# Florescence/UNet-Medical-Image-Contour-Segmentation

Measured on NVIDIA B200. Metric: unet512_train_images_per_sec, higher is better.
Workload: dtype bf16

## Files before the change

include/unetb200.h:

```cpp
#ifndef UNETB200_H_
#define UNETB200_H_

#include <stddef.h>
#include <stdint.h>

#ifdef __cplusplus
extern "C" {
#endif

#define UNETB200_F32 0
#define UNETB200_BF16 1

#define UNETB200_OK 0
#define UNETB200_E_INVALID (-1)
#define UNETB200_E_CUDA (-2)
#define UNETB200_E_NOMEM (-3)

#define UNETB200_ALGO_AUTO 0
#define UNETB200_ALGO_SIMT 1
#define UNETB200_ALGO_TC 2
#define UNETB200_ALGO_PREFER_TC 3

int unetb200_version(void);
const char* unetb200_last_error(void);
int unetb200_device_info(int* sm_count, int* cc_major, int* cc_minor);

typedef struct unetb200_gconv {
  int32_t dtype;
  int32_t algo;
  int32_t B, Hm, Wm;
  int32_t Cin;
  int32_t ntaps;
  int32_t tap_dy[9], tap_dx[9];
  int32_t in_scale;
  int32_t in_off_y, in_off_x;
  int32_t Hin, Win;
  int64_t ld_in;
  int32_t N;
  int32_t nquad;
  int32_t out_scale;
  int32_t out_off_y, out_off_x;
  int32_t Hout, Wout;
  int64_t ld_out;
} unetb200_gconv_t;

int64_t unetb200_gconv_stats_workspace(const unetb200_gconv_t* d);
int unetb200_gconv_fprop(const unetb200_gconv_t* d, const void* x, const void* wp,
                         const float* bias, void* y, double* stats, float* stats_ws, int* algo_used,
                         void* stream);

int unetb200_gconv_fprop_affine_relu_supported(const unetb200_gconv_t* d, const void* x, const void* wp,
                                               const void* z);
int unetb200_gconv_fprop_affine_relu(const unetb200_gconv_t* d, const void* x, const void* wp,
                                     const float* scale_shift, void* z, void* stream);

int unetb200_gconv_fprop_affine_relu_pool_supported(const unetb200_gconv_t* d, const void* x, const void* wp,
                                                    const void* z, const void* pooled, int64_t ld_pooled);
int unetb200_gconv_fprop_affine_relu_pool(const unetb200_gconv_t* d, const void* x, const void* wp,
                                          const float* scale_shift, void* z, void* pooled, int64_t ld_pooled,
                                          void* stream);

int unetb200_gconv_fprop_affine_relu_outconv_supported(const unetb200_gconv_t* d, const void* x, const void* wp,
                                                       int ncls);
int unetb200_gconv_fprop_affine_relu_outconv(const unetb200_gconv_t* d, const void* x, const void* wp,
                                             const float* scale_shift, const float* oc_w, const float* oc_b,
                                             void* logits, int ncls, void* stream);

int unetb200_gconv_dgrad_bnbwd_supported(const unetb200_gconv_t* d, const void* g, const void* wp, const void* gx);
int unetb200_gconv_dgrad_bnbwd(const unetb200_gconv_t* d, const void* g, const void* wp, void* gx, const void* yprev,
                               int64_t ld_yprev, const float* coefs, double* sums, float* ws, void* stream);

int unetb200_gconv_wgrad_plan(const unetb200_gconv_t* d, int* splits, int* algo_used);
int unetb200_gconv_wgrad(const unetb200_gconv_t* d, const void* x, const void* gy, float* partials,
                         int splits, void* stream);
int unetb200_wgrad_reduce(const float* partials, int splits, int ntaps, int Cin, int N, int Cq,
                          float* dst, int64_t st, int64_t sc, int64_t sq, int64_t sn, int accumulate,
                          void* stream);

typedef struct unetb200_reduce_job {
  const float* partials;
  float* dst;
  int64_t st, sc, sq, sn;
  int32_t splits, ntaps, Cin, N, Cq, accumulate;
} unetb200_reduce_job_t;
int unetb200_wgrad_reduce_multi(const unetb200_reduce_job_t* jobs, int njobs, void* stream);

int unetb200_pack_weights(const float* src, void* dst, int dst_dtype, int64_t n0, int64_t n1,
                          int64_t n2, int64_t s0, int64_t s1, int64_t s2, int64_t off, void* stream);
typedef struct unetb200_pack_job {
  const float* src;
  void* dst;
  int64_t n0, n1, n2;
  int64_t s0, s1, s2, off;
} unetb200_pack_job_t;
int unetb200_pack_weights_multi(const unetb200_pack_job_t* jobs, int njobs, int dst_dtype, void* stream);

int unetb200_split_tf32(const float* x, int64_t ld_x, float* out, int64_t npix, int C, int pattern,
                        void* stream);

int unetb200_bn_finalize(const double* stats, int64_t count, const float* gamma, const float* beta,
                         float eps, float momentum, float* running_mean, float* running_var,
                         float* save_mean, float* save_invstd, float* scale, float* shift, int C,
                         void* stream);
int unetb200_bn_finalize_track(const double* stats, int64_t count, const float* gamma, const float* beta,
                               float eps, float momentum, float* running_mean, float* running_var,
                               float* save_mean, float* save_invstd, float* scale, float* shift,
                               int64_t* num_batches_tracked, int C, void* stream);
int unetb200_bn_eval_coeffs(const float* gamma, const float* beta, const float* running_mean,
                            const float* running_var, float eps, float* scale, float* shift,
                            float* save_mean, float* save_invstd, int C, void* stream);
int unetb200_bn_relu_apply(const void* y, int64_t ld_y, const float* scale, const float* shift,
                           void* z, int64_t ld_z, void* pooled, int64_t ld_p, int dtype, int B,
                           int H, int W, int C, void* stream);
int unetb200_maxpool2_fwd(const void* x, int64_t ld_x, void* p, int64_t ld_p, int dtype, int B,
                          int H, int W, int C, void* stream);
int unetb200_maxpool2_bwd(const void* x, int64_t ld_x, const void* gp, int64_t ld_gp, void* gx,
                          int64_t ld_gx, int accumulate, int dtype, int B, int H, int W, int C,
                          void* stream);
int unetb200_maxpool2_bwd_bnreduce(const void* x, int64_t ld_x, const void* gp, int64_t ld_gp, void* gx,
                                   int64_t ld_gx, const void* y, int64_t ld_y, const float* scale,
                                   const float* shift, const float* mean, const float* invstd, double* sums,
                                   int dtype, int B, int H, int W, int C, void* stream);
int unetb200_bn_relu_bwd_reduce(const void* gz, int64_t ld_gz, const void* y, int64_t ld_y,
                                const float* scale, const float* shift, const float* mean,
                                const float* invstd, double* sums, int dtype, int B, int H, int W,
                                int C, void* stream);
int unetb200_bn_bwd_finalize(const double* sums, int64_t count, int training, float* dgamma,
                             float* dbeta, float* coef, int C, void* stream);
int unetb200_bn_relu_bwd_apply(const void* gz, int64_t ld_gz, const void* y, int64_t ld_y,
                               const float* scale, const float* shift, const float* mean,
                               const float* invstd, const float* coef, void* gy, int64_t ld_gy,
                               int dtype, int B, int H, int W, int C, void* stream);

#define UNETB200_IPC_HANDLE_BYTES 64
#define UNETB200_BUS_ID_BYTES 32
typedef struct unetb200_bn_peer_group_s unetb200_bn_peer_group_t;
int unetb200_bn_peer_group_create(int rank, int world, int max_channels, void* ipc_handle, char* bus_id,
                                  unetb200_bn_peer_group_t** out);
int unetb200_bn_peer_group_open(unetb200_bn_peer_group_t* g, const void* ipc_handles, const char* bus_ids);
int unetb200_bn_peer_group_destroy(unetb200_bn_peer_group_t* g);
int unetb200_bn_peer_group_status(const unetb200_bn_peer_group_t* g, int64_t* missing_rank, int64_t* epoch);
int unetb200_bn_sync_finalize(unetb200_bn_peer_group_t* g, const double* stats, int64_t count,
                              const float* gamma, const float* beta, float eps, float momentum,
                              float* running_mean, float* running_var, float* save_mean,
                              float* save_invstd, float* scale, float* shift,
                              int64_t* num_batches_tracked, int C, void* stream);
int unetb200_bn_sync_bwd_finalize(unetb200_bn_peer_group_t* g, const double* sums, int64_t count,
                                  float* dgamma, float* dbeta, float* coef, int C, void* stream);

int unetb200_upsample2x_fwd(const void* x, int64_t ld_x, void* y, int64_t ld_y, int dtype, int B,
                            int h, int w, int C, int Hout, int Wout, int off_y, int off_x,
                            void* stream);
int unetb200_upsample2x_bwd(const void* gy, int64_t ld_gy, void* gx, int64_t ld_gx, int dtype,
                            int B, int h, int w, int C, int Hout, int Wout, int off_y, int off_x,
                            void* stream);

int unetb200_gather_nhwc(const void* src, int src_dtype, int64_t sn, int64_t sc, int64_t sh,
                         int64_t sw, void* dst, int dst_dtype, int64_t ld_dst, int B, int C, int H,
                         int W, void* stream);
int unetb200_copy_channels(const void* src, int src_dtype, int64_t ld_src, void* dst, int dst_dtype,
                           int64_t ld_dst, int64_t npix, int C, void* stream);
int unetb200_zero_channels(void* dst, int dtype, int64_t ld_dst, int64_t npix, int C, void* stream);
int unetb200_channel_sum(const void* g, int dtype, int64_t ld, int64_t npix, int C, double* acc,
                         float* out, void* stream);
int unetb200_f64_to_f32(const double* src, float* dst, int n, void* stream);
int unetb200_add_channels(void* a, int64_t ld_a, const void* b, int64_t ld_b, int dtype,
                          int64_t npix, int C, void* stream);

int unetb200_outconv_fwd(const void* x, int64_t ld_x, const float* w, const float* bias,
                         void* logits, int dtype, int64_t npix, int C, int ncls, void* stream);
int64_t unetb200_outconv_bwd_workspace(int64_t npix, int C, int ncls);
int unetb200_outconv_bwd(const void* x, int64_t ld_x, const float* w, const void* glogits,
                         void* gx, int64_t ld_gx, float* dw, float* dbias, float* workspace,
                         int dtype, int64_t npix, int C, int ncls, void* stream);
int unetb200_outconv_bwd_bnbwd_supported(const void* x, int64_t ld_x, const void* gx, int64_t ld_gx,
                                         const void* yprev, int64_t ld_yprev, int dtype, int C, int ncls);
int unetb200_outconv_bwd_bnbwd(const void* x, int64_t ld_x, const float* w, const void* glogits, void* gx,
                               int64_t ld_gx, float* dw, float* dbias, float* workspace, const void* yprev,
                               int64_t ld_yprev, const float* coefs, double* sums, int dtype, int64_t npix, int C,
                               int ncls, void* stream);

int unetb200_sa_forward(const void* x, int64_t ld_x, const float* w, float* stats, float* gate, void* out,
                        int64_t ld_out, int dtype, int B, int H, int W, int C, void* stream);
int64_t unetb200_sa_backward_workspace(int B, int H, int W);
int unetb200_sa_backward(const void* g, int64_t ld_g, const void* x, int64_t ld_x, const float* w,
// ... 43 lines not shown
```

unet-medical-image-contour-segmentation_b200/csrc/common.cuh:

```cuda
#pragma once
#include <cuda_bf16.h>
#include <cuda_runtime.h>
#include <stdint.h>
#include <stdio.h>

#include <string>

#include "../../include/unetb200.h"

namespace ub {

void set_error(const char* fmt, ...);
int cuda_fail(cudaError_t e, const char* what);

#define UB_CHECK_ARG(cond, ...)                \
  do {                                         \
    if (!(cond)) {                             \
      ub::set_error(__VA_ARGS__);              \
      return UNETB200_E_INVALID;               \
    }                                          \
  } while (0)

#define UB_LAUNCH_CHECK(what)                              \
  do {                                                     \
// ... 13 lines not shown
  static __device__ __forceinline__ float round(float v) { return v; }
};
template <>
struct Elem<__nv_bfloat16> {
  static __device__ __forceinline__ float ld(const __nv_bfloat16* p) { return __bfloat162float(*p); }
  static __device__ __forceinline__ void st(__nv_bfloat16* p, float v) { *p = __float2bfloat16_rn(v); }
  static __device__ __forceinline__ float round(float v) { return __bfloat162float(__float2bfloat16_rn(v)); }
};

__device__ __forceinline__ void load8(const float* p, float v[8]) {
  float4 a = *reinterpret_cast<const float4*>(p);
  float4 b = *reinterpret_cast<const float4*>(p + 4);
  v[0] = a.x; v[1] = a.y; v[2] = a.z; v[3] = a.w; v[4] = b.x; v[5] = b.y; v[6] = b.z; v[7] = b.w;
}
__device__ __forceinline__ void load8(const __nv_bfloat16* p, float v[8]) {
  uint4 r = *reinterpret_cast<const uint4*>(p);
  const uint32_t w[4] = {r.x, r.y, r.z, r.w};
#pragma unroll
  for (int i = 0; i < 4; ++i) {
    v[2 * i] = __uint_as_float(w[i] << 16);
    v[2 * i + 1] = __uint_as_float(w[i] & 0xffff0000u);
  }
}
__device__ __forceinline__ uint32_t pack_bf16x2(float lo, float hi) {
  __nv_bfloat162 t = __floats2bfloat162_rn(lo, hi);
  return *reinterpret_cast<uint32_t*>(&t);
}
__device__ __forceinline__ void store8(float* p, const float v[8]) {
  *reinterpret_cast<float4*>(p) = make_float4(v[0], v[1], v[2], v[3]);
  *reinterpret_cast<float4*>(p + 4) = make_float4(v[4], v[5], v[6], v[7]);
}
__device__ __forceinline__ void store8(__nv_bfloat16* p, const float v[8]) {
  uint4 r;
  r.x = pack_bf16x2(v[0], v[1]);
  r.y = pack_bf16x2(v[2], v[3]);
  r.z = pack_bf16x2(v[4], v[5]);
  r.w = pack_bf16x2(v[6], v[7]);
  *reinterpret_cast<uint4*>(p) = r;
}

__device__ __forceinline__ float warp_sum(float v) {
#pragma unroll
  for (int o = 16; o > 0; o >>= 1) v += __shfl_xor_sync(0xffffffffu, v, o);
  return v;
}
__device__ __forceinline__ double warp_sum(double v) {
#pragma unroll
  for (int o = 16; o > 0; o >>= 1) v += __shfl_xor_sync(0xffffffffu, v, o);
  return v;
}

inline bool aligned16(const void* p) { return (reinterpret_cast<uintptr_t>(p) & 15) == 0; }

}
```

unet-medical-image-contour-segmentation_b200/csrc/conv_simt.cu:

```cuda
#include <cstdlib>

#include "gconv.cuh"

namespace ub {

constexpr int FBM = 128, FBN = 64, FBK = 16;
constexpr int WBK = 64, WBN = 64, WBM = 16;

int gconv_validate(const unetb200_gconv_t* d, GconvDev* o) {
  UB_CHECK_ARG(d != nullptr, "gconv: null descriptor");
  UB_CHECK_ARG(d->dtype == UNETB200_F32 || d->dtype == UNETB200_BF16, "gconv: dtype %d", d->dtype);
  UB_CHECK_ARG(d->B > 0 && d->Hm > 0 && d->Wm > 0 && d->Cin > 0, "gconv: bad M grid / Cin");
  UB_CHECK_ARG(d->ntaps >= 1 && d->ntaps <= 9, "gconv: ntaps %d", d->ntaps);
  UB_CHECK_ARG(d->in_scale == 1 || d->in_scale == 2, "gconv: in_scale %d", d->in_scale);
  UB_CHECK_ARG(d->out_scale == 1 || d->out_scale == 2, "gconv: out_scale %d", d->out_scale);
  UB_CHECK_ARG(d->nquad == 1 || d->nquad == 4, "gconv: nquad %d", d->nquad);
  UB_CHECK_ARG(d->N > 0 && d->N % d->nquad == 0, "gconv: N %d not divisible by nquad %d", d->N, d->nquad);
  UB_CHECK_ARG(d->nquad == 1 || d->out_scale == 2, "gconv: nquad 4 needs out_scale 2");
  UB_CHECK_ARG(d->Hin > 0 && d->Win > 0 && d->Hout > 0 && d->Wout > 0, "gconv: bad grids");
  UB_CHECK_ARG(d->ld_in >= d->Cin && d->ld_out >= d->N / d->nquad, "gconv: pixel stride smaller than channels");
  UB_CHECK_ARG(d->out_off_y >= 0 && d->out_off_x >= 0 &&
                   (d->Hm - 1) * d->out_scale + (d->nquad == 4 ? 1 : 0) + d->out_off_y < d->Hout &&
                   (d->Wm - 1) * d->out_scale + (d->nquad == 4 ? 1 : 0) + d->out_off_x < d->Wout,
               "gconv: output does not fit the destination grid");
// ... 587 lines not shown

static bool simt_vec_ok(const unetb200_gconv_t* d, const void* x, const void* wp, const void* y) {
  const size_t esz = d->dtype == UNETB200_BF16 ? 2 : 4;
  const int Cq = d->N / d->nquad;
  return d->Cin % 16 == 0 && Cq % 4 == 0 && d->ld_in % 8 == 0 && d->ld_out % 4 == 0 &&
         (reinterpret_cast<uintptr_t>(x) % (8 * esz)) == 0 && (!wp || (reinterpret_cast<uintptr_t>(wp) % 16) == 0) &&
         (reinterpret_cast<uintptr_t>(y) % (4 * esz)) == 0;
}

static int simt_fbn(int N) { return N <= 16 ? 16 : (N <= 32 ? 32 : 64); }
static int simt_fbm(int N) { return 8 * 256 / (simt_fbn(N) / 4); }
static int simt_wbk(int N) { return 4 * 256 / (simt_fbn(N) / 4); }

static int simt_wgrad_splits(const GconvDev& g) {
  const int wbn = simt_fbn(g.N), wbk = simt_wbk(g.N);
  long long tiles = (long long)((g.K + wbk - 1) / wbk) * ((g.N + wbn - 1) / wbn);
  long long want = ((long long)sm_count() * 6 + tiles - 1) / tiles;
  long long max_by_m = (g.M + 255) / 256;
  if (want > max_by_m) want = max_by_m;
  if (want > 1024) want = 1024;
  if (want < 1) want = 1;
  return (int)want;
}

}

using namespace ub;
typedef __nv_bfloat16 bf16;

extern "C" {

int64_t unetb200_gconv_stats_workspace(const unetb200_gconv_t* d) {
  GconvDev g;
  if (gconv_validate(d, &g)) return -1;
  long long simt_tiles = (g.M + FBM - 1) / FBM;
  long long tiles = simt_tiles;
  long long ft = first_fprop_tiles(d);
  if (ft > tiles) tiles = ft;
  long long n = tiles * 2 * g.N;
  long long n2 = tc2_stats_workspace(d);
  if (n2 > n) n = n2;
  long long n3 = tc3_stats_workspace(d);
  if (n3 > n) n = n3;
  const long long n4 = narrow_tc_stats_rows(d) * 2 * g.N;
  if (n4 > n) n = n4;
  const long long n5 = halo_stats_rows(d) * 2 * g.N;
  if (n5 > n) n = n5;
  const long long n6 = first_narrow_rows(d) * 2 * g.N;
  if (n6 > n) n = n6;
  const long long n7 = fprop_narrow_f32_rows(d) * 2 * g.N;
  return n > n7 ? n : n7;
}

int unetb200_gconv_fprop(const unetb200_gconv_t* d, const void* x, const void* wp, const float* bias, void* y,
                         double* stats, float* stats_ws, int* algo_used, void* stream) {
  GconvDev g;
  int rc = gconv_validate(d, &g);
  if (rc) return rc;
  UB_CHECK_ARG(x && wp && y, "gconv_fprop: null pointer");
  UB_CHECK_ARG(!stats || (stats_ws && d->nquad == 1), "gconv_fprop: stats need a workspace and nquad == 1");
  if (!stats) stats_ws = nullptr;
  cudaStream_t s = (cudaStream_t)stream;
  int algo = d->algo;
  if (algo != UNETB200_ALGO_SIMT && !stats && halo_t_fprop_supported(d, x, wp, y)) {
    if (algo_used) *algo_used = UNETB200_ALGO_TC;
    return halo_t_fprop(d, x, wp, bias, y, s);
  }
  if (algo != UNETB200_ALGO_SIMT && !stats && !bias && halo_t_dgrad_supported(d, x, wp, y)) {
    if (algo_used) *algo_used = UNETB200_ALGO_TC;
    return halo_t_dgrad(d, x, wp, y, s);
  }
  if (!bias && first_narrow_supported(d, y)) {
    if (algo_used) *algo_used = UNETB200_ALGO_SIMT;
    return first_narrow_fprop(d, x, wp, y, stats, stats_ws, nullptr, s);
  }
  if (algo != UNETB200_ALGO_SIMT && !bias && halo_fprop_supported(d, x, wp, y)) {
    if (algo_used) *algo_used = UNETB200_ALGO_TC;
    return halo_fprop(d, x, wp, y, stats, stats_ws, nullptr, s);
  }
  if (algo != UNETB200_ALGO_SIMT && !bias && narrow_tc_supported(d, x, wp, y)) {
    if (algo_used) *algo_used = UNETB200_ALGO_TC;
    return narrow_tc_fprop(d, x, wp, y, stats, stats_ws, nullptr, s);
  }
  if (algo == UNETB200_ALGO_AUTO || algo == UNETB200_ALGO_PREFER_TC) algo = tc_fprop_supported(d, x, wp, y) ? UNETB200_ALGO_TC : UNETB200_ALGO_SIMT;
  if (algo_used) *algo_used = algo;
  if (algo == UNETB200_ALGO_TC) {
    UB_CHECK_ARG(tc_fprop_supported(d, x, wp, y), "gconv_fprop: tcgen05 path requested but shape/alignment unsupported");
    if (tc3_fprop_supported(d, x, wp, bias, y)) return tc3_fprop(d, g, x, wp, y, stats, stats_ws, s);
    return tc2_fprop(d, g, x, wp, bias, y, stats, stats_ws, s);
  }
  UB_CHECK_ARG(algo == UNETB200_ALGO_SIMT, "gconv_fprop: unknown algo %d", algo);
  if (!bias && first_fprop_supported(d, y)) return first_fprop(d, g, x, wp, y, stats, stats_ws, s);
  if (!bias && fprop_narrow_f32_supported(d, x, wp, y)) return fprop_narrow_f32(d, x, wp, y, stats, stats_ws, s);
  const int fbn = simt_fbn(g.N), fbm = simt_fbm(g.N);
  dim3 grid((unsigned)((g.M + fbm - 1) / fbm), (unsigned)((g.N + fbn - 1) / fbn));
  const bool vec = simt_vec_ok(d, x, wp, y) && (g.K % 4 == 0);
#define UB_SIMT_F(T, V, BN) gconv_fprop_simt_kernel<T, V, BN><<<grid, 256, 0, s>>>(g, (const T*)x, (const T*)wp, bias, (T*)y, stats_ws)
#define UB_SIMT_FN(T, V) do { if (fbn == 16) UB_SIMT_F(T, V, 16); else if (fbn == 32) UB_SIMT_F(T, V, 32); else UB_SIMT_F(T, V, 64); } while (0)
  if (d->dtype == UNETB200_BF16) {
    if (vec) UB_SIMT_FN(bf16, true); else UB_SIMT_FN(bf16, false);
  } else {
    if (vec) UB_SIMT_FN(float, true); else UB_SIMT_FN(float, false);
  }
#undef UB_SIMT_FN
#undef UB_SIMT_F
  UB_LAUNCH_CHECK("gconv_fprop_simt");
  if (stats) return launch_stats_reduce(stats_ws, (g.M + fbm - 1) / fbm, 2 * g.N, stats, s);
  return 0;
}

int unetb200_gconv_fprop_affine_relu_supported(const unetb200_gconv_t* d, const void* x, const void* wp, const void* z) {
  GconvDev g;
  if (gconv_validate(d, &g)) return 0;
  static const bool off = getenv("UNETB200_NO_BN_FOLD") != nullptr;
  static const bool wide = getenv("UNETB200_TC3_MAXBN") && atoi(getenv("UNETB200_TC3_MAXBN")) >= 256;
  if (off || d->algo == UNETB200_ALGO_SIMT) return 0;
  if (first_tc_supported(d, z) && aligned16(wp)) return 1;
  if (first_narrow_supported(d, z)) return 1;
  if (halo_fprop_supported(d, x, wp, z)) return 1;
  if (narrow_tc_supported(d, x, wp, z)) return 1;
  if (d->N % 128 != 0 && d->N % 64 != 0) return 0;
  if (d->dtype == UNETB200_BF16 && d->N % 256 == 0 && wide) return 0;
  return tc_fprop_supported(d, x, wp, z) && tc3_fprop_supported(d, x, wp, nullptr, z);
}

int unetb200_gconv_fprop_affine_relu(const unetb200_gconv_t* d, const void* x, const void* wp, const float* scale_shift,
                                     void* z, void* stream) {
  GconvDev g;
  int rc = gconv_validate(d, &g);
  if (rc) return rc;
  UB_CHECK_ARG(x && wp && z && scale_shift, "gconv_fprop_affine_relu: null pointer");
  UB_CHECK_ARG(unetb200_gconv_fprop_affine_relu_supported(d, x, wp, z),
               "gconv_fprop_affine_relu: shape not covered by the fused kernel (query _supported first and run "
               "gconv_fprop + bn_relu_apply instead)");
  if (first_tc_supported(d, z) && aligned16(wp))
    return first_tc_fprop(d, x, wp, z, nullptr, nullptr, scale_shift, (cudaStream_t)stream);
  if (first_narrow_supported(d, z))
    return first_narrow_fprop(d, x, wp, z, nullptr, nullptr, scale_shift, (cudaStream_t)stream);
  if (halo_fprop_supported(d, x, wp, z))
    return halo_fprop(d, x, wp, z, nullptr, nullptr, scale_shift, (cudaStream_t)stream);
  if (narrow_tc_supported(d, x, wp, z))
    return narrow_tc_fprop(d, x, wp, z, nullptr, nullptr, scale_shift, (cudaStream_t)stream);
  return tc3_fprop(d, g, x, wp, z, nullptr, nullptr, (cudaStream_t)stream, scale_shift);
}

int unetb200_gconv_fprop_affine_relu_pool_supported(const unetb200_gconv_t* d, const void* x, const void* wp, const void* z,
                                                    const void* pooled, int64_t ld_pooled) {
  GconvDev g;
  if (gconv_validate(d, &g)) return 0;
  static const bool off = getenv("UNETB200_NO_POOL_FOLD") != nullptr;
  if (off || d->dtype != UNETB200_BF16 || !pooled || (ld_pooled & 1) || (reinterpret_cast<uintptr_t>(pooled) & 3)) return 0;
  if (!unetb200_gconv_fprop_affine_relu_supported(d, x, wp, z)) return 0;
  if ((first_tc_supported(d, z) && aligned16(wp)) || first_narrow_supported(d, z)) return 0;
  if (!halo_fprop_supported(d, x, wp, z) && narrow_tc_supported(d, x, wp, z)) return 0;
  return d->Hm >= 2 && d->Wm >= 2;
}

int unetb200_gconv_fprop_affine_relu_pool(const unetb200_gconv_t* d, const void* x, const void* wp, const float* scale_shift,
                                          void* z, void* pooled, int64_t ld_pooled, void* stream) {
  GconvDev g;
  int rc = gconv_validate(d, &g);
  if (rc) return rc;
  UB_CHECK_ARG(x && wp && z && scale_shift && pooled, "gconv_fprop_affine_relu_pool: null pointer");
  UB_CHECK_ARG(unetb200_gconv_fprop_affine_relu_pool_supported(d, x, wp, z, pooled, ld_pooled),
               "gconv_fprop_affine_relu_pool: shape not covered (query _supported first and run gconv_fprop_affine_relu + "
               "maxpool2_fwd instead)");
  if (halo_fprop_supported(d, x, wp, z))
    return halo_fprop(d, x, wp, z, nullptr, nullptr, scale_shift, (cudaStream_t)stream, nullptr, 0, nullptr, pooled,
                      (long long)ld_pooled);
  return tc3_fprop(d, g, x, wp, z, nullptr, nullptr, (cudaStream_t)stream, scale_shift, nullptr, 0, nullptr, nullptr, pooled,
                   (long long)ld_pooled);
}

int unetb200_gconv_dgrad_bnbwd_supported(const unetb200_gconv_t* d, const void* g, const void* wp, const void* gx) {
  GconvDev gd;
  if (gconv_validate(d, &gd)) return 0;
  static const bool off = getenv("UNETB200_NO_BNBWD_FUSE") != nullptr;
  if (off || d->algo == UNETB200_ALGO_SIMT) return 0;
  if (halo_bnbwd_supported(d, g, wp, gx)) return 1;
  return tc_fprop_supported(d, g, wp, gx) && tc3_fprop_supported(d, g, wp, nullptr, gx) && tc3_bnbwd_supported(d);
}

int unetb200_gconv_dgrad_bnbwd(const unetb200_gconv_t* d, const void* g, const void* wp, void* gx, const void* yprev,
                               int64_t ld_yprev, const float* coefs, double* sums, float* ws, void* stream) {
  GconvDev gd;
  int rc = gconv_validate(d, &gd);
  if (rc) return rc;
  UB_CHECK_ARG(g && wp && gx && yprev && coefs && sums && ws, "gconv_dgrad_bnbwd: null pointer");
  UB_CHECK_ARG(ld_yprev >= d->N, "gconv_dgrad_bnbwd: ld_yprev < N");
  UB_CHECK_ARG(unetb200_gconv_dgrad_bnbwd_supported(d, g, wp, gx),
               "gconv_dgrad_bnbwd: shape not covered by the fused kernel (query _supported first and run gconv_fprop + "
               "bn_relu_bwd_reduce instead)");
  if (halo_bnbwd_supported(d, g, wp, gx))
    return halo_fprop(d, g, wp, gx, sums, ws, nullptr, (cudaStream_t)stream, yprev, (long long)ld_yprev, coefs);
  return tc3_fprop(d, gd, g, wp, gx, sums, ws, (cudaStream_t)stream, nullptr, yprev, (long long)ld_yprev, coefs);
}

int unetb200_gconv_fprop_affine_relu_outconv_supported(const unetb200_gconv_t* d, const void* x, const void* wp,
                                                       int ncls) {
  GconvDev g;
  if (gconv_validate(d, &g)) return 0;
  static const bool off = getenv("UNETB200_NO_BN_FOLD") != nullptr || getenv("UNETB200_NO_OUTCONV_FOLD") != nullptr;
  if (off || d->algo == UNETB200_ALGO_SIMT || !aligned16(x) || !aligned16(wp)) return 0;
  return tc3_affine_outconv_supported(d, ncls);
}

int unetb200_gconv_fprop_affine_relu_outconv(const unetb200_gconv_t* d, const void* x, const void* wp,
                                             const float* scale_shift, const float* oc_w, const float* oc_b,
                                             void* logits, int ncls, void* stream) {
  GconvDev g;
  int rc = gconv_validate(d, &g);
  if (rc) return rc;
  UB_CHECK_ARG(x && wp && scale_shift && oc_w && logits, "gconv_fprop_affine_relu_outconv: null pointer");
  UB_CHECK_ARG(unetb200_gconv_fprop_affine_relu_outconv_supported(d, x, wp, ncls),
               "gconv_fprop_affine_relu_outconv: shape not covered (query _supported first)");
  Tc3OutConv oc = {oc_w, oc_b, logits, ncls};
  return tc3_fprop(d, g, x, wp, logits, nullptr, nullptr, (cudaStream_t)stream, scale_shift, nullptr, 0, nullptr, &oc);
}

int unetb200_gconv_wgrad_plan(const unetb200_gconv_t* d, int* splits, int* algo_used) {
  GconvDev g;
  int rc = gconv_validate(d, &g);
  if (rc) return rc;
  int algo = d->algo;
  if (first_narrow_supported(d, nullptr)) {
    if (algo_used) *algo_used = UNETB200_ALGO_SIMT;
    if (splits) *splits = first_narrow_wgrad_splits(d);
    return 0;
  }
  if (algo != UNETB200_ALGO_SIMT && halo_wgrad_supported(d, nullptr, nullptr)) {
    if (algo_used) *algo_used = UNETB200_ALGO_TC;
    if (splits) *splits = halo_wgrad_splits(d);
    return 0;
  }
  if (algo != UNETB200_ALGO_SIMT && halo_t_wgrad_supported(d, nullptr, nullptr)) {
    if (algo_used) *algo_used = UNETB200_ALGO_TC;
    if (splits) *splits = halo_t_wgrad_splits(d);
    return 0;
  }
  if (algo != UNETB200_ALGO_SIMT && narrow_wgrad_supported(d, nullptr, nullptr)) {
    if (algo_used) *algo_used = UNETB200_ALGO_TC;
    if (splits) *splits = narrow_wgrad_splits(d);
    return 0;
  }
  if (algo == UNETB200_ALGO_AUTO || algo == UNETB200_ALGO_PREFER_TC) algo = tc_wgrad_supported(d, nullptr, nullptr) ? UNETB200_ALGO_TC : UNETB200_ALGO_SIMT;
  if (algo == UNETB200_ALGO_TC)
    UB_CHECK_ARG(tc_wgrad_supported(d, nullptr, nullptr), "gconv_wgrad: tcgen05 path requested but shape unsupported");
// ... 191 lines not shown
```

unet-medical-image-contour-segmentation_b200/csrc/conv_tc3.cu:

```cuda
#include <cstring>

#include "tc_common.cuh"

namespace ub {

__device__ __forceinline__ uint32_t cluster_ctarank() {
  uint32_t r;
  asm volatile("mov.u32 %0, %%cluster_ctarank;" : "=r"(r));
  return r;
}
__device__ __forceinline__ void cluster_sync_all() {
  asm volatile("barrier.cluster.arrive.release.aligned;\n\tbarrier.cluster.wait.acquire.aligned;" ::: "memory");
}
__device__ __forceinline__ uint32_t mapa_u32(uint32_t saddr, uint32_t rank) {
  uint32_t r;
  asm volatile("mapa.shared::cluster.u32 %0, %1, %2;" : "=r"(r) : "r"(saddr), "r"(rank));
  return r;
}
__device__ __forceinline__ void mbar_arrive_cluster(uint32_t cluster_addr) {
  asm volatile("mbarrier.arrive.release.cluster.shared::cluster.b64 _, [%0];" ::"r"(cluster_addr) : "memory");
}
__device__ __forceinline__ void mbar_arrive_local(uint64_t* bar) {
  asm volatile("mbarrier.arrive.shared::cta.b64 _, [%0];" ::"r"(smem_u32(bar)) : "memory");
}
// ... 123 lines not shown
  long long ld_pool;
};

constexpr uint32_t kA3Stage = 44032;
constexpr int kEpi3Stage = 4096;
constexpr int kEpi3Warps = 8;
constexpr int kTc3Threads = 64 + 32 * kEpi3Warps;

constexpr int EPI_PLAIN = 0, EPI_AFFINE = 1, EPI_BNBWD = 2, EPI_AFFINE_OUT = 3;
template <typename T, int BLOCK_N, int SA, int SB, int ACC, int CG, int TPS, int EPI = EPI_PLAIN>
__global__ void __launch_bounds__(kTc3Threads, 1) tc3_conv_kernel(const __grid_constant__ Tc3Params p) {
  constexpr bool OUTC = EPI == EPI_AFFINE_OUT, AFFINE = EPI == EPI_AFFINE || OUTC, BNBWD = EPI == EPI_BNBWD;
  static_assert(!OUTC || (BLOCK_N == 64 && sizeof(T) == 2), "the OutConv epilogue is the bf16 N = 64 kernel");
  constexpr bool TF32 = sizeof(T) == 4;
  constexpr int EPR = 128 / sizeof(T);
  constexpr uint32_t kBTap = (BLOCK_N / CG) * 128;
  constexpr uint32_t kBStage = TPS * kBTap;
  static_assert(9 % TPS == 0, "taps per stage");
  constexpr int NCB = BLOCK_N / EPR;
  static_assert(2 * BLOCK_N * ACC <= 512, "TMEM columns");
  extern __shared__ uint8_t smem_raw[];
  uint8_t* smem = reinterpret_cast<uint8_t*>((reinterpret_cast<uintptr_t>(smem_raw) + 1023) & ~(uintptr_t)1023);
  uint8_t* a_ring = smem;
  uint8_t* b_ring = a_ring + SA * kA3Stage;
  uint8_t* epi = b_ring + SB * kBStage;
  uint8_t* yst = epi + kEpi3Warps * kEpi3Stage;
  uint64_t* bars = reinterpret_cast<uint64_t*>(yst + (BNBWD ? kEpi3Warps * kEpi3Stage : 0));
  uint64_t* a_full = bars;
  uint64_t* a_empty = a_full + SA;
  uint64_t* b_full = a_empty + SA;
  uint64_t* b_empty = b_full + SB;
  uint64_t* t_full = b_empty + SB;
  uint64_t* t_empty = t_full + ACC;
  uint64_t* y_full = t_empty + ACC;
  uint32_t* tmem_slot = reinterpret_cast<uint32_t*>(y_full + kEpi3Warps);

  const int warp = threadIdx.x >> 5, lane = threadIdx.x & 31;
  const uint32_t rank = CG == 2 ? cluster_ctarank() : 0u;
  const int group0 = blockIdx.x / CG, ngroups = gridDim.x / CG;
  if (warp == 0 && lane == 0) {
    tma_prefetch_desc(&p.a_map);
    tma_prefetch_desc(&p.b_map);
    tma_prefetch_desc(&p.o_map);
    for (int s = 0; s < SA; ++s) { mbar_init(&a_full[s], 1); mbar_init(&a_empty[s], 1); }
    for (int s = 0; s < SB; ++s) { mbar_init(&b_full[s], 1); mbar_init(&b_empty[s], 1); }
    for (int s = 0; s < ACC; ++s) { mbar_init(&t_full[s], 1); mbar_init(&t_empty[s], kEpi3Warps * CG); }
    if constexpr (BNBWD) {
      tma_prefetch_desc(&p.y_map);
      for (int s = 0; s < kEpi3Warps; ++s) mbar_init(&y_full[s], 1);
    }
    fence_barrier_init();
  }
  if (warp == 1) tmem_alloc_cg<CG>(tmem_slot, 512);
  if constexpr (OUTC) {
    float* ocs = reinterpret_cast<float*>(epi);
    for (int i = threadIdx.x; i < 64 * 8 + 8; i += blockDim.x) {
      const int c = i >> 3, k = i & 7;
      float v = 0.f;
      if (k < p.ncls) v = c < 64 ? __ldg(p.oc_w + k * 64 + c) : (p.oc_b ? __ldg(p.oc_b + k) : 0.f);
      ocs[i] = __bfloat162float(__float2bfloat16_rn(v));
    }
  }
  tc_fence_before();
  __syncthreads();
  if constexpr (CG == 2) cluster_sync_all();
  tc_fence_after();
  const uint32_t tmem_base = *tmem_slot;

  if (warp == 0) {
    uint32_t sa = 0, pa = 1, sb = 0, pb = 1;
    for (int gt = group0; gt < p.total_groups; gt += ngroups) {
      const int nb = gt / p.m_groups;
      int mt = (gt - nb * p.m_groups) * CG + (int)rank;
      const bool valid = mt < p.m_tiles;
      const int tj = mt % p.tiles_w;
      mt /= p.tiles_w;
      const int ti = mt % p.tiles_h;
      const int b = valid ? mt / p.tiles_h : p.B;
      const int i0 = ti * p.tile_h - 1, j0 = tj * p.tile_w - 1;
      const int n0 = nb * BLOCK_N + (int)rank * (BLOCK_N / CG);
      for (int c = 0; c < p.cchunks; ++c) {
        mbar_wait(&a_empty[sa], pa);
        if (elect_one()) {
          if (rank == 0) mbar_expect_tx(&a_full[sa], CG * p.a_box_bytes);
          tma_load_4d_cg<CG>(a_ring + sa * kA3Stage, &p.a_map, mapa_u32(smem_u32(&a_full[sa]), 0), c * EPR, j0, i0, b);
        }
        if (++sa == SA) { sa = 0; pa ^= 1; }
        for (int t = 0; t < 9; t += TPS) {
          mbar_wait(&b_empty[sb], pb);
          if (elect_one()) {
            if (rank == 0) mbar_expect_tx(&b_full[sb], CG * kBStage);
            const uint32_t bar = mapa_u32(smem_u32(&b_full[sb]), 0);
#pragma unroll
            for (int j = 0; j < TPS; ++j)
              tma_load_2d_cg<CG>(b_ring + sb * kBStage + j * kBTap, &p.b_map, bar, (t + j) * p.Cin + c * EPR, n0);
          }
          if (++sb == SB) { sb = 0; pb ^= 1; }
        }
      }
    }
  } else if (warp == 1) {
    if (rank == 0) {
      constexpr uint32_t idesc = make_idesc(TF32, false, false, 128 * CG, BLOCK_N);
      const uint64_t a_desc_t = make_desc(smem_u32(a_ring), 16, p.row_bytes);
      const uint64_t b_desc_t = make_desc(smem_u32(b_ring), 16, 1024);
      const uint32_t sub1 = p.sub1_off;
      uint32_t sa = 0, pa = 0, sb = 0, pb = 0, acc = 0, pacc = 1;
      for (int gt = group0; gt < p.total_groups; gt += ngroups) {
        mbar_wait(&t_empty[acc], pacc);
        tc_fence_after();
        const uint32_t d_tmem = tmem_base + acc * 2 * BLOCK_N;
        uint32_t accum = 0;
        for (int c = 0; c < p.cchunks; ++c) {
          mbar_wait(&a_full[sa], pa);
          const uint64_t a_desc0 = a_desc_t + sa * (kA3Stage >> 4);
          for (int t = 0; t < 9; t += TPS) {
            mbar_wait(&b_full[sb], pb);
            tc_fence_after();
            const uint64_t b_desc0 = b_desc_t + sb * (kBStage >> 4);
            if (elect_one()) {
#pragma unroll
              for (int j = 0; j < TPS; ++j) {
                const uint64_t a_desc1 = a_desc0 + p.tap_aoff[t + j];
                const uint64_t b_desc1 = b_desc0 + j * (kBTap >> 4);
#pragma unroll
                for (int kk = 0; kk < 4; ++kk) {
                  const uint32_t on = accum | (uint32_t)(j | kk);
                  umma_cg<CG, TF32>(d_tmem, a_desc1 + 2 * kk, b_desc1 + 2 * kk, idesc, on);
                  umma_cg<CG, TF32>(d_tmem + BLOCK_N, a_desc1 + sub1 + 2 * kk, b_desc1 + 2 * kk, idesc, on);
                }
              }
              umma_commit_cg<CG>(&b_empty[sb]);
              if (t + TPS == 9) umma_commit_cg<CG>(&a_empty[sa]);
            }
            __syncwarp();
            accum = 1;
            if (++sb == SB) { sb = 0; pb ^= 1; }
          }
          if (++sa == SA) { sa = 0; pa ^= 1; }
        }
        if (elect_one()) umma_commit_cg<CG>(&t_full[acc]);
        __syncwarp();
        if (++acc == ACC) { acc = 0; pacc ^= 1; }
      }
    }
  } else {
    const int quad = warp & 3;
    const int s = (warp - 2) >> 2;
    const int ew = s * 4 + quad;
    uint8_t* buf = epi + ew * kEpi3Stage;
    const uint32_t buf_s = smem_u32(buf);
    uint32_t acc = 0, pacc = 0;
    int cur_nb = -1;
    float st[NCB][TF32 ? 2 : 4];
#pragma unroll
    for (int i = 0; i < NCB; ++i)
#pragma unroll
      for (int j = 0; j < (TF32 ? 2 : 4); ++j) st[i][j] = 0.f;
    auto flush = [&](int nb) {
      if (!p.stats_ws || nb < 0) return;
      float* dst = p.stats_ws + (((long long)nb * gridDim.x + blockIdx.x) * kEpi3Warps + ew) * 2 * BLOCK_N;
#pragma unroll
      for (int cb = 0; cb < NCB; ++cb) {
        if constexpr (TF32) {
          dst[cb * 32 + lane] = st[cb][0];
          dst[BLOCK_N + cb * 32 + lane] = st[cb][1];
          st[cb][0] = st[cb][1] = 0.f;
        } else {
          dst[cb * 64 + 2 * lane] = st[cb][0];
          dst[BLOCK_N + cb * 64 + 2 * lane] = st[cb][1];
          dst[cb * 64 + 2 * lane + 1] = st[cb][2];
          dst[BLOCK_N + cb * 64 + 2 * lane + 1] = st[cb][3];
          st[cb][0] = st[cb][1] = st[cb][2] = st[cb][3] = 0.f;
        }
      }
    };
    const uint32_t t_empty_leader0 = mapa_u32(smem_u32(&t_empty[0]), 0);
    constexpr int CPL = TF32 ? 1 : 2;
    float bmu[BNBWD ? NCB : 1][CPL], bis[BNBWD ? NCB : 1][CPL], bsc[BNBWD ? NCB : 1][CPL], bsh[BNBWD ? NCB : 1][CPL];
    uint8_t* ybuf = yst + ew * kEpi3Stage;
    const uint32_t ybuf_s = smem_u32(ybuf);
    uint32_t yph = 0;
    auto y_fetch = [&](int gt2, int cb2) {
      const int nb2 = gt2 / p.m_groups;
      int mt2 = (gt2 - nb2 * p.m_groups) * CG + (int)rank;
      const bool valid2 = mt2 < p.m_tiles;
      const int tj2 = mt2 % p.tiles_w;
      mt2 /= p.tiles_w;
      const int ti2 = mt2 % p.tiles_h;
      const int b2 = valid2 ? mt2 / p.tiles_h : p.B;
      mbar_expect_tx(&y_full[ew], kEpi3Stage);
      tma_load_4d(ybuf, &p.y_map, &y_full[ew], nb2 * BLOCK_N + cb2 * EPR, tj2 * p.tile_w + s * p.sub1_dj,
                  ti2 * p.tile_h + s * p.sub1_di + 4 * quad, b2);
    };
    if constexpr (BNBWD) {
      if (lane == 0 && group0 < p.total_groups) y_fetch(group0, 0);
    }
    for (int gt = group0; gt < p.total_groups; gt += ngroups) {
      const int nb = gt / p.m_groups;
      int mt = (gt - nb * p.m_groups) * CG + (int)rank;
      const bool valid = mt < p.m_tiles;
      const int tj = mt % p.tiles_w;
      mt /= p.tiles_w;
      const int ti = mt % p.tiles_h;
      const int b = mt / p.tiles_h;
      const int n0 = nb * BLOCK_N;
      if (nb != cur_nb) {
        flush(cur_nb);
        cur_nb = nb;
        if constexpr (BNBWD) {
#pragma unroll
          for (int cb = 0; cb < NCB; ++cb)
#pragma unroll
            for (int k = 0; k < CPL; ++k) {
              const int ch = n0 + cb * EPR + CPL * lane + k;
              bmu[cb][k] = __ldg(p.bnc + ch);
              bis[cb][k] = __ldg(p.bnc + p.N + ch);
              bsc[cb][k] = __ldg(p.bnc + 2 * p.N + ch);
              bsh[cb][k] = __ldg(p.bnc + 3 * p.N + ch);
            }
        }
      }
      const int pi0 = ti * p.tile_h + s * p.sub1_di + 4 * quad;
      const int pj0 = tj * p.tile_w + s * p.sub1_dj;
      const uint32_t valid_rows =
          __ballot_sync(0xffffffffu, valid && (pi0 + (lane >> 3) < p.Hm) && (pj0 + (lane & 7) < p.Wm));
      mbar_wait(&t_full[acc], pacc);
      tc_fence_after();
      if (valid_rows != 0u) {
#pragma unroll
        for (int cb = 0; cb < NCB; ++cb) {
          const uint32_t taddr = tmem_base + ((uint32_t)(quad * 32) << 16) + acc * 2 * BLOCK_N + s * BLOCK_N + cb * EPR;
          uint32_t v[EPR];
#pragma unroll
          for (int h = 0; h < EPR / 32; ++h) tmem_ld32_issue(taddr + h * 32, v + h * 32);
          if (lane == 0) tma_store_wait_read_all();
          tmem_ld_fence();
          __syncwarp();
          if constexpr (AFFINE) {
            const float4* sc4 = reinterpret_cast<const float4*>(p.affine + n0 + cb * EPR);
            const float4* sh4 = reinterpret_cast<const float4*>(p.affine + p.N + n0 + cb * EPR);
#pragma unroll
            for (int k4 = 0; k4 < EPR / 4; ++k4) {
              const float4 a = __ldg(sc4 + k4), c = __ldg(sh4 + k4);
              v[4 * k4 + 0] = __float_as_uint(fmaxf(fmaf(__uint_as_float(v[4 * k4 + 0]), a.x, c.x), 0.f));
              v[4 * k4 + 1] = __float_as_uint(fmaxf(fmaf(__uint_as_float(v[4 * k4 + 1]), a.y, c.y), 0.f));
              v[4 * k4 + 2] = __float_as_uint(fmaxf(fmaf(__uint_as_float(v[4 * k4 + 2]), a.z, c.z), 0.f));
              v[4 * k4 + 3] = __float_as_uint(fmaxf(fmaf(__uint_as_float(v[4 * k4 + 3]), a.w, c.w), 0.f));
            }
          }
          if constexpr (OUTC) {
            const float* ocs = reinterpret_cast<const float*>(epi);
            float lg[8];
#pragma unroll
            for (int k = 0; k < 8; ++k) lg[k] = 0.f;
#pragma unroll
            for (int c = 0; c < 64; ++c) {
              const float z = __bfloat162float(__float2bfloat16_rn(__uint_as_float(v[c])));
              const float4 w0 = *reinterpret_cast<const float4*>(ocs + c * 8);
              lg[0] = fmaf(z, w0.x, lg[0]); lg[1] = fmaf(z, w0.y, lg[1]);
              lg[2] = fmaf(z, w0.z, lg[2]); lg[3] = fmaf(z, w0.w, lg[3]);
// ... 98 lines not shown
            for (int r = 0; r < 32; ++r)
              u[r] = lds_u32(buf_s + r * 128 + ((((lane >> 2) ^ (r & 7)) << 4) | ((lane & 3) << 2)));
            if (valid_rows == 0xffffffffu) {
#pragma unroll
              for (int r = 0; r < 32; ++r) {
                if constexpr (TF32) {
                  const float a = __uint_as_float(u[r]);
                  s0 += a; q0 = fmaf(a, a, q0);
                } else {
                  const float a = __uint_as_float(u[r] << 16), c2 = __uint_as_float(u[r] & 0xffff0000u);
                  s0 += a; q0 = fmaf(a, a, q0); s1 += c2; q1 = fmaf(c2, c2, q1);
                }
              }
            } else {
#pragma unroll
              for (int r = 0; r < 32; ++r) {
                const float m = ((valid_rows >> r) & 1u) ? 1.f : 0.f;
                if constexpr (TF32) {
                  const float a = __uint_as_float(u[r]) * m;
                  s0 += a; q0 = fmaf(a, a, q0);
                } else {
                  const float a = __uint_as_float(u[r] << 16) * m, c2 = __uint_as_float(u[r] & 0xffff0000u) * m;
                  s0 += a; q0 = fmaf(a, a, q0); s1 += c2; q1 = fmaf(c2, c2, q1);
                }
              }
            }
            st[cb][0] += s0; st[cb][1] += q0;
            if constexpr (!TF32) { st[cb][2] += s1; st[cb][3] += q1; }
          }
        }
      }
      if constexpr (BNBWD) {
        if (valid_rows == 0u) {
#pragma unroll 1
          for (int cb = 0; cb < NCB; ++cb) {
            mbar_wait(&y_full[ew], yph);
            yph ^= 1;
            __syncwarp();
            if (lane == 0) {
              if (cb + 1 < NCB) y_fetch(gt, cb + 1);
              else if (gt + ngroups < p.total_groups) y_fetch(gt + ngroups, 0);
            }
          }
        }
      }
      tc_fence_before();
      __syncwarp();
      if (lane == 0) {
        if constexpr (CG == 2) mbar_arrive_cluster(t_empty_leader0 + acc * 8);
        else mbar_arrive_local(&t_empty[acc]);
      }
      if (++acc == ACC) { acc = 0; pacc ^= 1; }
    }
    flush(cur_nb);
    if (lane == 0) tma_store_wait_all();
  }
  tc_fence_before();
  __syncthreads();
  if constexpr (CG == 2) cluster_sync_all();
  if (warp == 1) {
    __syncwarp();
    tmem_dealloc_cg<CG>(tmem_base, 512);
  }
}

struct Tc3Plan {
  int BN, CG, tile_w, tile_h, box_w, box_h;
  int m_tiles, m_groups, n_blocks, grid;
};

static int tc3_cluster_size() {
  static const int cg = getenv("UNETB200_TC3_CG1") ? 1 : 2;
  return cg;
}

static bool tc3_plan(const unetb200_gconv_t* d, Tc3Plan* pl) {
  const int esz = d->dtype == UNETB200_BF16 ? 2 : 4;
  const int epr = 128 / esz;
  if (d->dtype != UNETB200_BF16 && d->dtype != UNETB200_F32) return false;
  if (d->nquad != 1 || d->in_scale != 1 || d->out_scale != 1 || d->ntaps != 9) return false;
  if (d->in_off_y || d->in_off_x) return false;
  if (d->Cin % epr || d->N % 64) return false;
  if ((d->ld_in * esz) % 16 || (d->ld_out * esz) % 16) return false;
  bool seen[9] = {false};
  for (int t = 0; t < 9; ++t) {
    const int dy = d->tap_dy[t], dx = d->tap_dx[t];
    if (dy < -1 || dy > 1 || dx < -1 || dx > 1) return false;
    if (seen[(dy + 1) * 3 + dx + 1]) return false;
    seen[(dy + 1) * 3 + dx + 1] = true;
  }
  pl->CG = tc3_cluster_size();
  static const int max_bn = getenv("UNETB200_TC3_MAXBN") ? atoi(getenv("UNETB200_TC3_MAXBN")) : 128;
  pl->BN = (d->dtype == UNETB200_BF16 && d->N % 256 == 0 && max_bn >= 256) ? 256 : (d->N % 128 == 0 ? 128 : 64);
  if (d->Wm > 8) { pl->tile_w = 16; pl->tile_h = 16; }
  else { pl->tile_w = 8; pl->tile_h = 32; }
  pl->box_w = pl->tile_w + 2;
  pl->box_h = pl->tile_h + 2;
  const int tiles_w = (d->Wm + pl->tile_w - 1) / pl->tile_w, tiles_h = (d->Hm + pl->tile_h - 1) / pl->tile_h;
  pl->m_tiles = d->B * tiles_w * tiles_h;
  pl->m_groups = (pl->m_tiles + pl->CG - 1) / pl->CG;
  pl->n_blocks = d->N / pl->BN;
  const long long total = (long long)pl->m_groups * pl->n_blocks;
  const int slots = sm_count() / pl->CG;
  pl->grid = (int)(total < slots ? total : slots) * pl->CG;
  return true;
}

int tc3_fprop_supported(const unetb200_gconv_t* d, const void* x, const void* wp, const float* bias, const void* y) {
  static const bool off = getenv("UNETB200_NO_TC3") != nullptr;
  if (off || bias) return 0;
  if (d->dtype == UNETB200_F32 && d->algo != UNETB200_ALGO_TC && d->algo != UNETB200_ALGO_PREFER_TC) return 0;
  Tc3Plan pl;
  if (!tc3_plan(d, &pl)) return 0;
  if (!aligned16(x) || !aligned16(wp) || !aligned16(y)) return 0;
  return 1;
}

long long tc3_stats_workspace(const unetb200_gconv_t* d) {
  Tc3Plan pl;
  if (!tc3_plan(d, &pl)) return 0;
  return (long long)pl.n_blocks * pl.grid * kEpi3Warps * 2 * pl.BN;
}

template <typename T, int BN, int SA, int SB, int ACC, int CG, int TPS, int EPI = EPI_PLAIN>
static int tc3_launch(const Tc3Params& P, int grid, cudaStream_t s) {
  constexpr int smem = SA * kA3Stage + SB * TPS * (BN / CG) * 128 + (EPI == EPI_BNBWD ? 2 : 1) * kEpi3Warps * kEpi3Stage + 1024 + 256;
  static_assert(smem <= 227 * 1024, "shared memory budget");
  if (int rc = set_max_dynamic_smem(reinterpret_cast<const void*>(&tc3_conv_kernel<T, BN, SA, SB, ACC, CG, TPS, EPI>), smem,
                                    "tc3_conv smem attribute"))
    return rc;
  cudaLaunchConfig_t cfg = {};
  cfg.gridDim = dim3((unsigned)grid);
  cfg.blockDim = dim3(kTc3Threads);
  cfg.dynamicSmemBytes = smem;
  cfg.stream = s;
  cudaLaunchAttribute at[1];
  at[0].id = cudaLaunchAttributeClusterDimension;
  at[0].val.clusterDim.x = CG;
  at[0].val.clusterDim.y = 1;
  at[0].val.clusterDim.z = 1;
  cfg.attrs = at;
  cfg.numAttrs = 1;
  cudaError_t e = cudaLaunchKernelEx(&cfg, tc3_conv_kernel<T, BN, SA, SB, ACC, CG, TPS, EPI>, P);
  if (e != cudaSuccess) return cuda_fail(e, "tc3_conv launch");
  return 0;
}

__global__ void __launch_bounds__(1024) tc3_stats_reduce_kernel(const float* __restrict__ ws, int rows, int BN, int N, double* __restrict__ stats) {
  __shared__ double red[32][33];
  const int lane = threadIdx.x & 31, ry = threadIdx.x >> 5;
  const int nb = blockIdx.y;
  const int col = blockIdx.x * 32 + lane;
  double acc = 0.0;
  if (col < 2 * BN) {
    const float* base = ws + (long long)nb * rows * 2 * BN + col;
    int r = ry;
    for (; r + 96 < rows; r += 128) {
      const float a = base[(long long)r * 2 * BN], b = base[(long long)(r + 32) * 2 * BN],
                  c = base[(long long)(r + 64) * 2 * BN], d = base[(long long)(r + 96) * 2 * BN];
      acc += (double)a; acc += (double)b; acc += (double)c; acc += (double)d;
    }
    for (; r < rows; r += 32) acc += (double)base[(long long)r * 2 * BN];
  }
  red[ry][lane] = acc;
  __syncthreads();
  if (ry == 0 && col < 2 * BN) {
    double s = 0.0;
#pragma unroll
    for (int i = 0; i < 32; ++i) s += red[i][lane];
    const int which = col / BN, c = col - which * BN;
    stats[which * N + nb * BN + c] += s;
  }
}

int tc3_bnbwd_supported(const unetb200_gconv_t* d) {
  Tc3Plan pl;
  if (!tc3_plan(d, &pl)) return 0;
  return pl.CG == 2 && pl.BN != 256;
}

int tc3_affine_outconv_supported(const unetb200_gconv_t* d, int ncls) {
  Tc3Plan pl;
  if (!tc3_plan(d, &pl)) return 0;
  return d->dtype == UNETB200_BF16 && pl.CG == 2 && pl.BN == 64 && d->N == 64 && ncls >= 1 && ncls <= 8;
}

int tc3_fprop(const unetb200_gconv_t* d, const GconvDev& g, const void* x, const void* wp, void* y, double* stats,
              float* stats_ws, cudaStream_t stream, const float* affine, const void* yprev, long long ld_yprev,
              const float* bnc, const Tc3OutConv* oc, void* pooled, long long ld_pool) {
  Tc3Plan pl;
  if (pooled && (!affine || oc || d->dtype != UNETB200_BF16 || (ld_pool & 1) || (reinterpret_cast<uintptr_t>(pooled) & 3))) {
    set_error("tc3_fprop: the pooled second output needs the bf16 affine epilogue and 4-byte aligned rows");
    return UNETB200_E_INVALID;
  }
  if (yprev && (affine || !stats || !stats_ws || !bnc || !aligned16(yprev) ||
                (ld_yprev * (d->dtype == UNETB200_BF16 ? 2 : 4)) % 16)) {
    set_error("tc3_fprop: the BatchNorm-backward epilogue needs sums, a workspace, coefficients and 16-byte aligned yprev rows");
    return UNETB200_E_INVALID;
  }
  if (affine && (stats || (reinterpret_cast<uintptr_t>(affine) & 15))) {
    set_error("tc3_fprop: the affine epilogue takes no statistics and needs 16-byte aligned coefficients");
    return UNETB200_E_INVALID;
  }
  if (!tc3_plan(d, &pl)) { set_error("tc3_fprop: unsupported shape"); return UNETB200_E_INVALID; }
  const int esz = d->dtype == UNETB200_BF16 ? 2 : 4;
  Tc3Params P;
  memset(&P, 0, sizeof(P));
  int rc = encode_act_box(&P.a_map, d->dtype, x, d->Cin, d->Win, d->Hin, d->B, d->ld_in, (long long)d->Win * d->ld_in,
                          (long long)d->Hin * d->Win * d->ld_in, pl.box_w, pl.box_h, false);
  if (rc) return rc;
  const char* obase = (const char*)y + ((long long)d->out_off_y * d->Wout + d->out_off_x) * d->ld_out * (long long)esz;
  rc = encode_act_box(&P.o_map, d->dtype, obase, d->N, d->Wm, d->Hm, d->B, d->ld_out, (long long)d->Wout * d->ld_out,
                      (long long)d->Hout * d->Wout * d->ld_out, 8, 4, false);
  if (rc) return rc;
  rc = encode_weights(&P.b_map, d->dtype, wp, g.K, d->N, pl.BN / pl.CG);
  if (rc) return rc;
  for (int t = 0; t < 9; ++t)
    P.tap_aoff[t] = (uint32_t)(((d->tap_dy[t] + 1) * pl.box_w + (d->tap_dx[t] + 1)) * 128) >> 4;
  P.a_box_bytes = (uint32_t)(pl.box_w * pl.box_h * 128);
  P.row_bytes = (uint32_t)pl.box_w * 128;
  if (pl.tile_w == 16) { P.sub1_di = 0; P.sub1_dj = 8; P.sub1_off = (8 * 128) >> 4; }
  else { P.sub1_di = 16; P.sub1_dj = 0; P.sub1_off = (uint32_t)(16 * pl.box_w * 128) >> 4; }
  P.cchunks = d->Cin / (128 / esz);
  P.Cin = d->Cin;
  P.tile_w = pl.tile_w; P.tile_h = pl.tile_h;
  P.tiles_w = (d->Wm + pl.tile_w - 1) / pl.tile_w;
  P.tiles_h = (d->Hm + pl.tile_h - 1) / pl.tile_h;
  P.m_tiles = pl.m_tiles; P.m_groups = pl.m_groups;
  P.total_groups = pl.m_groups * pl.n_blocks;
  P.Hm = d->Hm; P.Wm = d->Wm; P.B = d->B;
  P.stats_ws = stats ? stats_ws : nullptr;
  P.affine = affine;
  P.N = d->N;
  P.bnc = bnc;
  P.pooled = pooled; P.ld_pool = ld_pool;
  if (yprev) {
    rc = encode_act_box(&P.y_map, d->dtype, yprev, d->N, d->Wm, d->Hm, d->B, ld_yprev, (long long)d->Wm * ld_yprev,
                        (long long)d->Hm * d->Wm * ld_yprev, 8, 4, false);
    if (rc) return rc;
  }
  if (oc) {
    if (!affine || !tc3_affine_outconv_supported(d, oc->ncls) || !oc->w || !oc->logits) {
      set_error("tc3_fprop: the OutConv epilogue needs the folded BatchNorm coefficients, bf16, N = 64 and n_classes <= 8");
      return UNETB200_E_INVALID;
    }
    P.oc_w = oc->w; P.oc_b = oc->b; P.logits = oc->logits; P.ncls = oc->ncls;
    return tc3_launch<__nv_bfloat16, 64, 3, 3, 2, 2, 3, EPI_AFFINE_OUT>(P, pl.grid, stream);
  }
  if (affine) {
    if (pl.BN == 256) { set_error("tc3_fprop: affine epilogue supports N blocks of 64 / 128"); return UNETB200_E_INVALID; }
    if (d->dtype == UNETB200_BF16) {
      if (pl.CG == 2) return pl.BN == 128 ? tc3_launch<__nv_bfloat16, 128, 2, 3, 2, 2, 3, EPI_AFFINE>(P, pl.grid, stream)
                                          : tc3_launch<__nv_bfloat16, 64, 3, 3, 2, 2, 3, EPI_AFFINE>(P, pl.grid, stream);
      return pl.BN == 128 ? tc3_launch<__nv_bfloat16, 128, 2, 6, 2, 1, 1, EPI_AFFINE>(P, pl.grid, stream)
                          : tc3_launch<__nv_bfloat16, 64, 3, 6, 2, 1, 1, EPI_AFFINE>(P, pl.grid, stream);
    }
    if (pl.CG == 2) return pl.BN == 128 ? tc3_launch<float, 128, 2, 3, 2, 2, 3, EPI_AFFINE>(P, pl.grid, stream)
                                        : tc3_launch<float, 64, 3, 3, 2, 2, 3, EPI_AFFINE>(P, pl.grid, stream);
    return pl.BN == 128 ? tc3_launch<float, 128, 2, 6, 2, 1, 1, EPI_AFFINE>(P, pl.grid, stream)
                        : tc3_launch<float, 64, 3, 6, 2, 1, 1, EPI_AFFINE>(P, pl.grid, stream);
  }
  if (stats) {
    cudaError_t e = cudaMemsetAsync(stats_ws, 0, sizeof(float) * (size_t)tc3_stats_workspace(d), stream);
    if (e != cudaSuccess) return cuda_fail(e, "tc3 stats workspace memset");
  }
  if (yprev) {
    if (pl.CG != 2 || pl.BN == 256) { set_error("tc3_fprop: BatchNorm-backward epilogue: CTA pairs, N blocks of 64 / 128"); return UNETB200_E_INVALID; }
    static const int cfg64 = getenv("UNETB200_BNBWD64_CFG") ? atoi(getenv("UNETB200_BNBWD64_CFG")) : 1;
    if (d->dtype == UNETB200_BF16)
      rc = pl.BN == 128 ? tc3_launch<__nv_bfloat16, 128, 2, 3, 2, 2, 3, EPI_BNBWD>(P, pl.grid, stream)
           : cfg64 == 1 ? tc3_launch<__nv_bfloat16, 64, 3, 2, 2, 2, 3, EPI_BNBWD>(P, pl.grid, stream)
                        : tc3_launch<__nv_bfloat16, 64, 2, 3, 2, 2, 3, EPI_BNBWD>(P, pl.grid, stream);
    else
      rc = pl.BN == 128 ? tc3_launch<float, 128, 2, 3, 2, 2, 3, EPI_BNBWD>(P, pl.grid, stream)
                        : tc3_launch<float, 64, 3, 2, 2, 2, 3, EPI_BNBWD>(P, pl.grid, stream);
  } else if (d->dtype == UNETB200_BF16) {
    if (pl.CG == 2) {
      if (pl.BN == 256) rc = tc3_launch<__nv_bfloat16, 256, 2, 2, 1, 2, 3>(P, pl.grid, stream);
      else if (pl.BN == 128) rc = tc3_launch<__nv_bfloat16, 128, 2, 3, 2, 2, 3>(P, pl.grid, stream);
      else rc = tc3_launch<__nv_bfloat16, 64, 3, 3, 2, 2, 3>(P, pl.grid, stream);
    } else {
      if (pl.BN == 256) rc = tc3_launch<__nv_bfloat16, 256, 2, 3, 1, 1, 1>(P, pl.grid, stream);
      else if (pl.BN == 128) rc = tc3_launch<__nv_bfloat16, 128, 2, 6, 2, 1, 1>(P, pl.grid, stream);
      else rc = tc3_launch<__nv_bfloat16, 64, 3, 6, 2, 1, 1>(P, pl.grid, stream);
    }
  } else {
    if (pl.CG == 2) {
      if (pl.BN == 128) rc = tc3_launch<float, 128, 2, 3, 2, 2, 3>(P, pl.grid, stream);
      else rc = tc3_launch<float, 64, 3, 3, 2, 2, 3>(P, pl.grid, stream);
    } else {
      if (pl.BN == 128) rc = tc3_launch<float, 128, 2, 6, 2, 1, 1>(P, pl.grid, stream);
      else rc = tc3_launch<float, 64, 3, 6, 2, 1, 1>(P, pl.grid, stream);
    }
  }
  if (rc) return rc;
  if (stats) {
    const int rows = pl.grid * kEpi3Warps;
    tc3_stats_reduce_kernel<<<dim3((2 * pl.BN + 31) / 32, pl.n_blocks), 1024, 0, stream>>>(stats_ws, rows, pl.BN, d->N, stats);
    cudaError_t e = cudaGetLastError();
    if (e != cudaSuccess) return cuda_fail(e, "tc3_stats_reduce");
  }
  return 0;
}


struct alignas(64) Tc3WParams {
  CUtensorMap a_map;
  CUtensorMap o_map;
  int g_dx[3], g_dy0, g_tap[3][3];
  int Cin, nunits;
  int tiles_w, tiles_h;
  int ptiles, ptiles_per_split;
  int N, K;
  float* partials;
};

template <int STAGES>
__global__ void __launch_bounds__(192, 1) tc3_wgrad_kernel(const __grid_constant__ Tc3WParams p) {
  constexpr int EPR = 64, BLOCK_N = 128;
  constexpr uint32_t kGSub = 64 * 128;
  constexpr uint32_t kABox = 10 * 8 * 128;
  constexpr uint32_t kStage = 2 * kABox + kGSub;
  constexpr int UMMA_K = 16, MMAS = 64 / UMMA_K;
  extern __shared__ uint8_t smem_raw[];
  uint8_t* smem = reinterpret_cast<uint8_t*>((reinterpret_cast<uintptr_t>(smem_raw) + 1023) & ~(uintptr_t)1023);
  uint64_t* full_bar = reinterpret_cast<uint64_t*>(smem + STAGES * kStage);
  uint64_t* empty_bar = full_bar + STAGES;
  uint64_t* tmem_full = empty_bar + STAGES;
  uint32_t* tmem_slot = reinterpret_cast<uint32_t*>(tmem_full + 1);

  const int warp = threadIdx.x >> 5, lane = threadIdx.x & 31;
  const uint32_t rank = cluster_ctarank();
  const int mt = blockIdx.x >> 1;
  const int n0 = blockIdx.y * BLOCK_N;
  const int split = blockIdx.z;
  const int pt_begin = split * p.ptiles_per_split;
  int pt_end = pt_begin + p.ptiles_per_split;
  if (pt_end > p.ptiles) pt_end = p.ptiles;
  const int num_k = pt_end - pt_begin;

  if (warp == 0 && lane == 0) {
    tma_prefetch_desc(&p.a_map);
    tma_prefetch_desc(&p.o_map);
    for (int s = 0; s < STAGES; ++s) { mbar_init(&full_bar[s], 1); mbar_init(&empty_bar[s], 1); }
    mbar_init(tmem_full, 1);
    fence_barrier_init();
  }
  if (warp == 1) tmem_alloc_cg<2>(tmem_slot, 512);
  tc_fence_before();
  __syncthreads();
  cluster_sync_all();
  tc_fence_after();
  const uint32_t tmem_base = *tmem_slot;

  if (warp == 0) {
    int pt = pt_begin;
    int tj = pt % p.tiles_w;
    int rest = pt / p.tiles_w;
    int ti = rest % p.tiles_h;
    int b = rest / p.tiles_h;
    int uc[2], ug[2];
#pragma unroll
    for (int h = 0; h < 2; ++h) {
      const int u = mt * 4 + (int)rank * 2 + h;
      uc[h] = u / 3;
      ug[h] = u - uc[h] * 3;
    }
    uint32_t s = 0, ph = 1;
    for (int kb = 0; kb < num_k; ++kb) {
      mbar_wait(&empty_bar[s], ph);
      if (elect_one()) {
        if (rank == 0) mbar_expect_tx(&full_bar[s], 2 * kStage);
        const uint32_t bar = mapa_u32(smem_u32(&full_bar[s]), 0);
        const int i0 = ti * 8, j0 = tj * 8;
        uint8_t* sa = smem + s * kStage;
#pragma unroll
        for (int h = 0; h < 2; ++h)
          tma_load_4d_cg<2>(sa + h * kABox, &p.a_map, bar, uc[h] * EPR, j0 + p.g_dx[ug[h]], i0 + p.g_dy0, b);
        tma_load_4d_cg<2>(sa + 2 * kABox, &p.o_map, bar, n0 + (int)rank * 64, j0, i0, b);
      }
      if (++s == STAGES) { s = 0; ph ^= 1; }
      if (++tj == p.tiles_w) { tj = 0; if (++ti == p.tiles_h) { ti = 0; ++b; } }
    }
  } else if (warp == 1) {
    if (rank == 0) {
      constexpr uint32_t idesc = make_idesc(false, true, true, 256, BLOCK_N);
      const uint64_t da_t = make_desc(smem_u32(smem), kABox, 1024, kLayoutSW128);
      const uint64_t db_t = make_desc(smem_u32(smem) + 2 * kABox, kGSub, 1024, kLayoutSW128);
      uint32_t s = 0, ph = 0;
      for (int kb = 0; kb < num_k; ++kb) {
        mbar_wait(&full_bar[s], ph);
        tc_fence_after();
        const uint64_t da0 = da_t + s * (kStage >> 4), db0 = db_t + s * (kStage >> 4);
        if (elect_one()) {
#pragma unroll
          for (int a = 0; a < 3; ++a) {
#pragma unroll
            for (int k = 0; k < MMAS; ++k)
              umma_cg<2, false>(tmem_base + a * BLOCK_N, da0 + ((a * 1024 + k * UMMA_K * 128) >> 4),
                                db0 + ((k * UMMA_K * 128) >> 4), idesc, (kb > 0 || k > 0) ? 1u : 0u);
          }
// ... 68 lines not shown
  w->mpairs = w->nunits / 4;
  w->ntiles = d->N / 128;
  w->tiles_w = (d->Wm + 7) / 8;
  w->tiles_h = (d->Hm + 7) / 8;
  w->ptiles = d->B * w->tiles_w * w->tiles_h;
  return true;
}

int tc3_wgrad_supported(const unetb200_gconv_t* d, const void* x, const void* gy) {
  Tc3WPlan w;
  if (!tc3_wgrad_plan(d, &w)) return 0;
  if ((x && !aligned16(x)) || (gy && !aligned16(gy))) return 0;
  return 1;
}

int tc3_wgrad_splits(const unetb200_gconv_t* d) {
  Tc3WPlan w;
  if (!tc3_wgrad_plan(d, &w)) return 1;
  const long long pairs = (long long)w.mpairs * w.ntiles;
  const long long max_by_k = (w.ptiles + 15) / 16;
  return pick_splits(pairs, sm_count() / 2, max_by_k);
}

int tc3_wgrad(const unetb200_gconv_t* d, const GconvDev& g, const void* x, const void* gy, float* partials, int splits,
              cudaStream_t stream) {
  Tc3WPlan w;
  if (!tc3_wgrad_plan(d, &w)) { set_error("tc3_wgrad: unsupported shape"); return UNETB200_E_INVALID; }
  Tc3WParams P;
  memset(&P, 0, sizeof(P));
  int rc = encode_act_box(&P.a_map, d->dtype, x, d->Cin, d->Win, d->Hin, d->B, d->ld_in, (long long)d->Win * d->ld_in,
                          (long long)d->Hin * d->Win * d->ld_in, 8, 10, true);
  if (rc) return rc;
  const char* obase = (const char*)gy + ((long long)d->out_off_y * d->Wout + d->out_off_x) * d->ld_out * 2LL;
  rc = encode_act_box(&P.o_map, d->dtype, obase, d->N, d->Wm, d->Hm, d->B, d->ld_out, (long long)d->Wout * d->ld_out,
                      (long long)d->Hout * d->Wout * d->ld_out, 8, 8, true);
  if (rc) return rc;
  for (int gi = 0; gi < 3; ++gi) {
    P.g_dx[gi] = w.g_dx[gi];
    for (int a = 0; a < 3; ++a) P.g_tap[gi][a] = w.g_tap[gi][a];
  }
  P.g_dy0 = w.g_dy0;
  P.Cin = d->Cin; P.nunits = w.nunits;
  P.tiles_w = w.tiles_w; P.tiles_h = w.tiles_h;
  P.ptiles = w.ptiles;
  P.ptiles_per_split = (w.ptiles + splits - 1) / splits;
  P.N = d->N; P.K = g.K;
  P.partials = partials;
  static const int st_env = getenv("UNETB200_TC3W_STAGES") ? atoi(getenv("UNETB200_TC3W_STAGES")) : 7;
  const bool deep = st_env >= 7;
  const int smem = (deep ? 7 : 5) * (2 * 10240 + 8192) + 1024 + 256;
  if (int rc = deep ? set_max_dynamic_smem(reinterpret_cast<const void*>(&tc3_wgrad_kernel<7>), smem, "tc3_wgrad smem attribute")
                    : set_max_dynamic_smem(reinterpret_cast<const void*>(&tc3_wgrad_kernel<5>), smem, "tc3_wgrad smem attribute"))
    return rc;
  cudaLaunchConfig_t cfg = {};
  cfg.gridDim = dim3((unsigned)w.mpairs * 2, (unsigned)w.ntiles, (unsigned)splits);
  cfg.blockDim = dim3(192);
  cfg.dynamicSmemBytes = smem;
  cfg.stream = stream;
  cudaLaunchAttribute at[1];
  at[0].id = cudaLaunchAttributeClusterDimension;
  at[0].val.clusterDim.x = 2;
  at[0].val.clusterDim.y = 1;
  at[0].val.clusterDim.z = 1;
  cfg.attrs = at;
  cfg.numAttrs = 1;
  cudaError_t e = deep ? cudaLaunchKernelEx(&cfg, tc3_wgrad_kernel<7>, P) : cudaLaunchKernelEx(&cfg, tc3_wgrad_kernel<5>, P);
  if (e != cudaSuccess) return cuda_fail(e, "tc3_wgrad launch");
  return 0;
}

}
```

unet-medical-image-contour-segmentation_b200/csrc/conv_tc4.cu:

```cuda
#include <cstring>

#include "tc_common.cuh"

namespace ub {

struct alignas(64) Tc4WParams {
  CUtensorMap a_map;
  CUtensorMap o_map;
  int tap[3][3];
  int Cin, N, K;
  int cchunks;
  int tiles_w, tiles_h;
  int ptiles, ptiles_per_split;
  float* partials;
};

constexpr uint32_t kT4Box = 10240;
constexpr uint32_t kT4Stage = 2 * kT4Box;
constexpr int kT4AccCols = 192;

template <int STAGES>
__global__ void __launch_bounds__(192, 1) tc4_wgrad_kernel(const __grid_constant__ Tc4WParams p) {
  constexpr int UMMA_K = 16, MMAS = 64 / UMMA_K;
  extern __shared__ uint8_t smem_raw[];
  uint8_t* smem = reinterpret_cast<uint8_t*>((reinterpret_cast<uintptr_t>(smem_raw) + 1023) & ~(uintptr_t)1023);
  uint64_t* full_bar = reinterpret_cast<uint64_t*>(smem + STAGES * kT4Stage);
  uint64_t* empty_bar = full_bar + STAGES;
  uint64_t* tmem_full = empty_bar + STAGES;
  uint32_t* tmem_slot = reinterpret_cast<uint32_t*>(tmem_full + 1);

  const int warp = threadIdx.x >> 5, lane = threadIdx.x & 31;
  const int c = blockIdx.x % p.cchunks;
  const int g = blockIdx.x / p.cchunks;
  const int split = blockIdx.z;
  const int pt_begin = split * p.ptiles_per_split;
  int pt_end = pt_begin + p.ptiles_per_split;
  if (pt_end > p.ptiles) pt_end = p.ptiles;
  const int num_k = pt_end - pt_begin;

  if (warp == 0 && lane == 0) {
    tma_prefetch_desc(&p.a_map);
    tma_prefetch_desc(&p.o_map);
    for (int s = 0; s < STAGES; ++s) { mbar_init(&full_bar[s], 1); mbar_init(&empty_bar[s], 1); }
    mbar_init(tmem_full, 1);
    fence_barrier_init();
  }
  if (warp == 1) tmem_alloc(tmem_slot, 512);
  tc_fence_before();
  __syncthreads();
  tc_fence_after();
  const uint32_t tmem_base = *tmem_slot;

  if (warp == 0) {
    int pt = pt_begin;
    int tj = pt % p.tiles_w;
    int rest = pt / p.tiles_w;
    int ti = rest % p.tiles_h;
    int b = rest / p.tiles_h;
    uint32_t s = 0, ph = 1;
    for (int kb = 0; kb < num_k; ++kb) {
      mbar_wait(&empty_bar[s], ph);
      if (elect_one()) {
        mbar_expect_tx(&full_bar[s], kT4Stage);
        const int i0 = ti * 8, j0 = tj * 8;
        uint8_t* sa = smem + s * kT4Stage;
        tma_load_4d(sa, &p.a_map, &full_bar[s], c * 64, j0, i0 - 1, b);
        tma_load_4d(sa + kT4Box, &p.o_map, &full_bar[s], g * 64, j0 - 1, i0, b);
      }
      if (++s == STAGES) { s = 0; ph ^= 1; }
      if (++tj == p.tiles_w) { tj = 0; if (++ti == p.tiles_h) { ti = 0; ++b; } }
    }
  } else if (warp == 1) {
    constexpr uint32_t idesc = make_idesc(false, true, true, 128, kT4AccCols);
    const uint64_t da_t = make_desc(smem_u32(smem), 1024, 1024, kLayoutSW128);
    const uint64_t db_t = make_desc(smem_u32(smem) + kT4Box, 128, 1280, kLayoutSW128);
    uint32_t s = 0, ph = 0;
    for (int kb = 0; kb < num_k; ++kb) {
      mbar_wait(&full_bar[s], ph);
      tc_fence_after();
      const uint64_t da0 = da_t + s * (kT4Stage >> 4), db0 = db_t + s * (kT4Stage >> 4);
      if (elect_one()) {
#pragma unroll
        for (int a = 0; a < 2; ++a) {
#pragma unroll
          for (int k = 0; k < MMAS; ++k)
            umma<false>(tmem_base + a * kT4AccCols, da0 + ((a * 2048 + k * 2 * 1024) >> 4), db0 + ((k * 2 * 1280) >> 4),
                        idesc, (kb > 0 || k > 0) ? 1u : 0u);
        }
        umma_commit(&empty_bar[s]);
      }
      __syncwarp();
      if (++s == STAGES) { s = 0; ph ^= 1; }
    }
    if (elect_one()) umma_commit(tmem_full);
    __syncwarp();
  } else {
    const int quad = warp & 3;
    const int row = quad * 32 + lane;
    mbar_wait(tmem_full, 0);
    tc_fence_after();
// ... 66 lines not shown
  w->tiles_w = (d->Wm + 7) / 8;
  w->tiles_h = (d->Hm + 7) / 8;
  w->ptiles = d->B * w->tiles_w * w->tiles_h;
  return true;
}

int tc4_wgrad_supported(const unetb200_gconv_t* d, const void* x, const void* gy) {
  Tc4WPlan w;
  if (!tc4_wgrad_plan(d, &w)) return 0;
  if ((x && !aligned16(x)) || (gy && !aligned16(gy))) return 0;
  return 1;
}

int tc4_wgrad_preferred(const unetb200_gconv_t* d) {
  if (!tc4_wgrad_supported(d, nullptr, nullptr)) return 0;
  if (tc4_mode() == 2) return 1;
  return tc3_wgrad_supported(d, nullptr, nullptr) ? 0 : 1;
}

int tc4_wgrad_splits(const unetb200_gconv_t* d) {
  Tc4WPlan w;
  if (!tc4_wgrad_plan(d, &w)) return 1;
  const long long tiles = (long long)w.cchunks * w.ngroups;
  const long long max_by_k = (w.ptiles + 15) / 16;
  return pick_splits(tiles, sm_count(), max_by_k);
}

int tc4_wgrad(const unetb200_gconv_t* d, const GconvDev& g, const void* x, const void* gy, float* partials, int splits,
              cudaStream_t stream) {
  Tc4WPlan w;
  if (!tc4_wgrad_plan(d, &w)) { set_error("tc4_wgrad: unsupported shape"); return UNETB200_E_INVALID; }
  Tc4WParams P;
  memset(&P, 0, sizeof(P));
  int rc = encode_act_box(&P.a_map, d->dtype, x, d->Cin, d->Win, d->Hin, d->B, d->ld_in, (long long)d->Win * d->ld_in,
                          (long long)d->Hin * d->Win * d->ld_in, 8, 10, true);
  if (rc) return rc;
  const char* obase = (const char*)gy + ((long long)d->out_off_y * d->Wout + d->out_off_x) * d->ld_out * 2LL;
  rc = encode_act_box(&P.o_map, d->dtype, obase, d->N, d->Wm, d->Hm, d->B, d->ld_out, (long long)d->Wout * d->ld_out,
                      (long long)d->Hout * d->Wout * d->ld_out, 10, 8, true);
  if (rc) return rc;
  for (int a = 0; a < 3; ++a)
    for (int b = 0; b < 3; ++b) P.tap[a][b] = w.tap[a][b];
  P.Cin = d->Cin; P.N = d->N; P.K = g.K;
  P.cchunks = w.cchunks;
  P.tiles_w = w.tiles_w; P.tiles_h = w.tiles_h;
  P.ptiles = w.ptiles;
  P.ptiles_per_split = (w.ptiles + splits - 1) / splits;
  P.partials = partials;
  constexpr int ST = 10;
  constexpr int smem = ST * (int)kT4Stage + 1024 + 256;
  static_assert(smem <= 227 * 1024, "shared memory budget");
  if (int e = set_max_dynamic_smem(reinterpret_cast<const void*>(&tc4_wgrad_kernel<ST>), smem, "tc4_wgrad")) return e;
  dim3 grid((unsigned)(w.cchunks * w.ngroups), 1, (unsigned)splits);
  tc4_wgrad_kernel<ST><<<grid, 192, smem, stream>>>(P);
  cudaError_t e = cudaGetLastError();
  if (e != cudaSuccess) return cuda_fail(e, "tc4_wgrad launch");
  return 0;
}

}
```

unet-medical-image-contour-segmentation_b200/csrc/core.cu:

```cuda
#include <stdarg.h>

#include <mutex>
#include <set>
#include <utility>

#include "common.cuh"

namespace ub {

static thread_local char g_err[1024] = "";

void set_error(const char* fmt, ...) {
  va_list ap;
  va_start(ap, fmt);
  vsnprintf(g_err, sizeof(g_err), fmt, ap);
  va_end(ap);
}

int cuda_fail(cudaError_t e, const char* what) {
  set_error("%s: %s (%s)", what, cudaGetErrorString(e), cudaGetErrorName(e));
  return e == cudaErrorMemoryAllocation ? UNETB200_E_NOMEM : UNETB200_E_CUDA;
}

int sm_count() {
  static int cached[64] = {0};
  int dev = 0;
  if (cudaGetDevice(&dev) != cudaSuccess || dev < 0 || dev >= 64) return 148;
  if (cached[dev] == 0) {
    int n = 0;
    if (cudaDeviceGetAttribute(&n, cudaDevAttrMultiProcessorCount, dev) != cudaSuccess || n <= 0) n = 148;
    cached[dev] = n;
  }
  return cached[dev];
}

int set_max_dynamic_smem(const void* func, int bytes, const char* what) {
  static std::mutex mu;
  static std::set<std::pair<int, const void*>> done;
  int dev = 0;
  cudaError_t e = cudaGetDevice(&dev);
  if (e != cudaSuccess) return cuda_fail(e, "cudaGetDevice");
  std::lock_guard<std::mutex> lock(mu);
  if (done.count({dev, func})) return 0;
  e = cudaFuncSetAttribute(func, cudaFuncAttributeMaxDynamicSharedMemorySize, bytes);
  if (e != cudaSuccess) return cuda_fail(e, what);
  done.insert({dev, func});
  return 0;
}

}

extern "C" {

int unetb200_version(void) { return 100; }

const char* unetb200_last_error(void) { return ub::g_err; }

int unetb200_device_info(int* sm_count, int* cc_major, int* cc_minor) {
  int dev = 0;
  cudaError_t e = cudaGetDevice(&dev);
  if (e != cudaSuccess) return ub::cuda_fail(e, "cudaGetDevice");
  cudaDeviceProp p;
  e = cudaGetDeviceProperties(&p, dev);
  if (e != cudaSuccess) return ub::cuda_fail(e, "cudaGetDeviceProperties");
  if (sm_count) *sm_count = p.multiProcessorCount;
  if (cc_major) *cc_major = p.major;
  if (cc_minor) *cc_minor = p.minor;
  return UNETB200_OK;
}
}
```

unet-medical-image-contour-segmentation_b200/csrc/elementwise.cu:

```cuda
#include "common.cuh"

namespace ub {

template <typename T, int V>
__device__ __forceinline__ void ldv(const T* p, float v[V]) {
  if constexpr (V == 8) {
    load8(p, v);
  } else {
#pragma unroll
    for (int i = 0; i < V; ++i) v[i] = Elem<T>::ld(p + i);
  }
}
template <typename T, int V>
__device__ __forceinline__ void stv(T* p, const float v[V]) {
  if constexpr (V == 8) {
    store8(p, v);
  } else {
#pragma unroll
    for (int i = 0; i < V; ++i) Elem<T>::st(p + i, v[i]);
  }
}
template <int V>
__device__ __forceinline__ void ldf(const float* p, float v[V]) {
#pragma unroll
  for (int i = 0; i < V; ++i) v[i] = __ldg(p + i);
}

static inline int grid_for(int64_t work, int threads, int per_sm = 8) {
  int64_t b = (work + threads - 1) / threads;
  int64_t cap = (int64_t)sm_count() * per_sm;
  if (b > cap) b = cap;
  if (b < 1) b = 1;
  return (int)b;
}

struct CsGeom {
  int CVB, gy;
  unsigned gx;
};
static CsGeom cs_geom(int CV, int64_t items, int per_thread, int max_cvb = 256) {
  CsGeom g;
  g.CVB = CV < max_cvb ? CV : max_cvb;
  const int lanes = 256 / g.CVB;
  g.gy = (CV + g.CVB - 1) / g.CVB;
  int64_t gx = (items + (int64_t)lanes * per_thread - 1) / ((int64_t)lanes * per_thread);
  int64_t cap = (int64_t)sm_count() * 8 / g.gy;
  if (cap < 1) cap = 1;
  if (gx > cap) gx = cap;
  if (gx < 1) gx = 1;
  g.gx = (unsigned)gx;
  return g;
}

template <typename T>
static bool vec_ok(int C, std::initializer_list<int64_t> lds, std::initializer_list<const void*> ptrs) {
  if (C % 8) return false;
  for (int64_t l : lds)
    if (l % 8) return false;
  for (const void* p : ptrs)
    if (p && (reinterpret_cast<uintptr_t>(p) % (8 * sizeof(T)))) return false;
  return true;
}

__global__ void bn_finalize_kernel(const double* __restrict__ stats, double inv_count, double unbias,
                                   const float* __restrict__ gamma, const float* __restrict__ beta,
                                   float eps, float momentum, float* running_mean, float* running_var,
                                   float* save_mean, float* save_invstd, float* scale, float* shift, int C,
                                   long long* num_batches_tracked) {
  int c = blockIdx.x * blockDim.x + threadIdx.x;
  if (c == 0 && num_batches_tracked) *num_batches_tracked += 1;
  if (c >= C) return;
  double mean = stats[c] * inv_count;
  double var = stats[C + c] * inv_count - mean * mean;
  if (var < 0) var = 0;
  float invstd = (float)(1.0 / sqrt(var + (double)eps));
  float g = gamma ? gamma[c] : 1.f, b = beta ? beta[c] : 0.f;
  float sc = g * invstd;
  save_mean[c] = (float)mean;
  save_invstd[c] = invstd;
  scale[c] = sc;
  shift[c] = b - (float)mean * sc;
  if (running_mean) running_mean[c] = (1.f - momentum) * running_mean[c] + momentum * (float)mean;
  if (running_var) running_var[c] = (1.f - momentum) * running_var[c] + momentum * (float)(var * unbias);
}

__global__ void bn_eval_coeffs_kernel(const float* __restrict__ gamma, const float* __restrict__ beta,
                                      const float* __restrict__ rm, const float* __restrict__ rv, float eps,
                                      float* scale, float* shift, float* save_mean, float* save_invstd, int C) {
  int c = blockIdx.x * blockDim.x + threadIdx.x;
  if (c >= C) return;
  float invstd = 1.0f / sqrtf(rv[c] + eps);
  float g = gamma ? gamma[c] : 1.f, b = beta ? beta[c] : 0.f;
  float sc = g * invstd;
  scale[c] = sc;
  shift[c] = b - rm[c] * sc;
  if (save_mean) save_mean[c] = rm[c];
  if (save_invstd) save_invstd[c] = invstd;
}

struct CsThread {
  int cv, lane, lanes;
  bool active;
};
__device__ __forceinline__ CsThread cs_thread(int CV, int CVB) {
  CsThread t;
  t.lanes = blockDim.x / CVB;
  t.lane = threadIdx.x / CVB;
  t.cv = blockIdx.y * CVB + threadIdx.x % CVB;
  t.active = t.cv < CV && t.lane < t.lanes;
  return t;
}

template <typename T, int V>
__global__ void __launch_bounds__(256)
bn_relu_apply_kernel(const T* __restrict__ y, int64_t ld_y, const float* __restrict__ scale,
                     const float* __restrict__ shift, T* __restrict__ z, int64_t ld_z, int64_t npix, int CV,
                     int CVB) {
  const CsThread t = cs_thread(CV, CVB);
  if (!t.active) return;
  const int c = t.cv * V;
  float sc[V], sh[V];
  ldf<V>(scale + c, sc);
  ldf<V>(shift + c, sh);
  const int64_t stride = (int64_t)gridDim.x * t.lanes;
  int64_t p = (int64_t)blockIdx.x * t.lanes + t.lane;
  for (; p + 3 * stride < npix; p += 4 * stride) {
    float v[4][V];
#pragma unroll
    for (int u = 0; u < 4; ++u) ldv<T, V>(y + (p + u * stride) * ld_y + c, v[u]);
#pragma unroll
    for (int u = 0; u < 4; ++u) {
#pragma unroll
      for (int i = 0; i < V; ++i) v[u][i] = fmaxf(fmaf(v[u][i], sc[i], sh[i]), 0.f);
      stv<T, V>(z + (p + u * stride) * ld_z + c, v[u]);
    }
  }
  for (; p < npix; p += stride) {
    float v[V];
    ldv<T, V>(y + p * ld_y + c, v);
#pragma unroll
    for (int i = 0; i < V; ++i) v[i] = fmaxf(fmaf(v[i], sc[i], sh[i]), 0.f);
    stv<T, V>(z + p * ld_z + c, v);
  }
}

__device__ __forceinline__ float pool_max(float m, float v) { return (v > m || v != v) ? v : m; }

template <typename T, int V>
__global__ void __launch_bounds__(256)
bn_relu_apply_pool_kernel(const T* __restrict__ y, int64_t ld_y, const float* __restrict__ scale,
                          const float* __restrict__ shift, T* __restrict__ z, int64_t ld_z, T* __restrict__ pooled,
                          int64_t ld_p, int B, int H, int W, int CV, int CVB) {
  const CsThread t = cs_thread(CV, CVB);
  if (!t.active) return;
  const int c = t.cv * V;
  float sc[V], sh[V];
  ldf<V>(scale + c, sc);
  ldf<V>(shift + c, sh);
  const int Hc = (H + 1) >> 1, Wc = (W + 1) >> 1, Hp = H >> 1, Wp = W >> 1;
  const int64_t nwin = (int64_t)B * Hc * Wc;
  const int64_t stride = (int64_t)gridDim.x * t.lanes;
  for (int64_t wdx = (int64_t)blockIdx.x * t.lanes + t.lane; wdx < nwin; wdx += stride) {
    const int j = (int)(wdx % Wc);
    int64_t r = wdx / Wc;
    const int i = (int)(r % Hc);
    const int n = (int)(r / Hc);
    const bool full = (2 * i + 1 < H) && (2 * j + 1 < W);
    float v[4][V], m[V];
    if (full) {
      const int64_t p00 = ((int64_t)n * H + 2 * i) * W + 2 * j;
      ldv<T, V>(y + p00 * ld_y + c, v[0]);
      ldv<T, V>(y + (p00 + 1) * ld_y + c, v[1]);
      ldv<T, V>(y + (p00 + W) * ld_y + c, v[2]);
      ldv<T, V>(y + (p00 + W + 1) * ld_y + c, v[3]);
#pragma unroll
      for (int k = 0; k < V; ++k) m[k] = -INFINITY;
#pragma unroll
      for (int q = 0; q < 4; ++q)
#pragma unroll
        for (int k = 0; k < V; ++k) {
          v[q][k] = Elem<T>::round(fmaxf(fmaf(v[q][k], sc[k], sh[k]), 0.f));
          m[k] = pool_max(m[k], v[q][k]);
        }
      stv<T, V>(z + p00 * ld_z + c, v[0]);
      stv<T, V>(z + (p00 + 1) * ld_z + c, v[1]);
      stv<T, V>(z + (p00 + W) * ld_z + c, v[2]);
      stv<T, V>(z + (p00 + W + 1) * ld_z + c, v[3]);
      stv<T, V>(pooled + (((int64_t)n * Hp + i) * Wp + j) * ld_p + c, m);
    } else {
      for (int q = 0; q < 4; ++q) {
        const int h = 2 * i + (q >> 1), w = 2 * j + (q & 1);
        if (h < H && w < W) {
          const int64_t p = ((int64_t)n * H + h) * W + w;
          ldv<T, V>(y + p * ld_y + c, v[0]);
#pragma unroll
          for (int k = 0; k < V; ++k) v[0][k] = fmaxf(fmaf(v[0][k], sc[k], sh[k]), 0.f);
          stv<T, V>(z + p * ld_z + c, v[0]);
        }
      }
    }
  }
}

template <typename T, int V>
__global__ void maxpool2_fwd_kernel(const T* __restrict__ x, int64_t ld_x, T* __restrict__ p, int64_t ld_p, int B,
                                    int H, int W, int CV) {
  const int Hp = H >> 1, Wp = W >> 1;
  const int64_t total = (int64_t)B * Hp * Wp * CV;
  for (int64_t idx = blockIdx.x * (int64_t)blockDim.x + threadIdx.x; idx < total;
       idx += (int64_t)gridDim.x * blockDim.x) {
    int cv = (int)(idx % CV);
    int64_t r = idx / CV;
    int j = (int)(r % Wp);
    r /= Wp;
    int i = (int)(r % Hp);
    int n = (int)(r / Hp);
    int c = cv * V;
    float m[V];
#pragma unroll
    for (int k = 0; k < V; ++k) m[k] = -INFINITY;
#pragma unroll
    for (int a = 0; a < 2; ++a)
#pragma unroll
      for (int b = 0; b < 2; ++b) {
        float v[V];
        ldv<T, V>(x + (((int64_t)n * H + 2 * i + a) * W + 2 * j + b) * ld_x + c, v);
#pragma unroll
        for (int k = 0; k < V; ++k) m[k] = pool_max(m[k], v[k]);
      }
    stv<T, V>(p + (((int64_t)n * Hp + i) * Wp + j) * ld_p + c, m);
  }
}

template <typename T, int V, bool ACC>
__global__ void maxpool2_bwd_kernel(const T* __restrict__ x, int64_t ld_x, const T* __restrict__ gp, int64_t ld_gp,
                                    T* __restrict__ gx, int64_t ld_gx, int B, int H, int W, int CV) {
  const int Hc = (H + 1) >> 1, Wc = (W + 1) >> 1, Hp = H >> 1, Wp = W >> 1;
  const int64_t total = (int64_t)B * Hc * Wc * CV;
  for (int64_t idx = blockIdx.x * (int64_t)blockDim.x + threadIdx.x; idx < total;
       idx += (int64_t)gridDim.x * blockDim.x) {
    int cv = (int)(idx % CV);
    int64_t r = idx / CV;
    int j = (int)(r % Wc);
    r /= Wc;
    int i = (int)(r % Hc);
    int n = (int)(r / Hc);
    int c = cv * V;
    const bool full = (i < Hp && j < Wp);
    float g[V], m[V];
    int arg[V];
#pragma unroll
    for (int k = 0; k < V; ++k) { m[k] = -INFINITY; arg[k] = 0; g[k] = 0.f; }
    if (full) {
      ldv<T, V>(gp + (((int64_t)n * Hp + i) * Wp + j) * ld_gp + c, g);
#pragma unroll
      for (int q = 0; q < 4; ++q) {
        float v[V];
        ldv<T, V>(x + (((int64_t)n * H + 2 * i + (q >> 1)) * W + 2 * j + (q & 1)) * ld_x + c, v);
#pragma unroll
        for (int k = 0; k < V; ++k)
          if (v[k] > m[k] || v[k] != v[k]) { m[k] = v[k]; arg[k] = q; }
      }
    }
#pragma unroll
    for (int q = 0; q < 4; ++q) {
      int h = 2 * i + (q >> 1), w = 2 * j + (q & 1);
      if (h < H && w < W) {
        T* dst = gx + (((int64_t)n * H + h) * W + w) * ld_gx + c;
        float o[V];
        if (ACC) ldv<T, V>(dst, o);
#pragma unroll
        for (int k = 0; k < V; ++k) {
          float t = (full && arg[k] == q) ? g[k] : 0.f;
          o[k] = ACC ? o[k] + t : t;
        }
        stv<T, V>(dst, o);
      }
    }
  }
}

template <typename T, int V>
__global__ void __launch_bounds__(256)
bn_relu_bwd_reduce_kernel(const T* __restrict__ gz, int64_t ld_gz, const T* __restrict__ y, int64_t ld_y,
                          const float* __restrict__ scale, const float* __restrict__ shift,
                          const float* __restrict__ mean, const float* __restrict__ invstd,
                          double* __restrict__ sums, int64_t npix, int C, int CV, int CVB) {
  constexpr int RED = (V == 8) ? 512 : 256;
  __shared__ float red[2][RED];
  const CsThread t = cs_thread(CV, CVB);
  const int cvl = threadIdx.x % CVB;
  float s0[V], s1[V];
#pragma unroll
  for (int k = 0; k < V; ++k) s0[k] = s1[k] = 0.f;
  if (t.active) {
    const int c = t.cv * V;
    float sc[V], sh[V], mu[V], is[V];
    ldf<V>(scale + c, sc);
    ldf<V>(shift + c, sh);
    ldf<V>(mean + c, mu);
    ldf<V>(invstd + c, is);
    const int64_t stride = (int64_t)gridDim.x * t.lanes;
    int64_t p = (int64_t)blockIdx.x * t.lanes + t.lane;
    for (; p + stride < npix; p += 2 * stride) {
      float g[2][V], v[2][V];
#pragma unroll
      for (int u = 0; u < 2; ++u) {
        ldv<T, V>(gz + (p + u * stride) * ld_gz + c, g[u]);
        ldv<T, V>(y + (p + u * stride) * ld_y + c, v[u]);
      }
#pragma unroll
      for (int u = 0; u < 2; ++u)
#pragma unroll
        for (int k = 0; k < V; ++k) {
          float gg = (fmaf(v[u][k], sc[k], sh[k]) > 0.f) ? g[u][k] : 0.f;
          s0[k] += gg;
          s1[k] += gg * ((v[u][k] - mu[k]) * is[k]);
        }
    }
    for (; p < npix; p += stride) {
      float g[V], v[V];
      ldv<T, V>(gz + p * ld_gz + c, g);
      ldv<T, V>(y + p * ld_y + c, v);
#pragma unroll
      for (int k = 0; k < V; ++k) {
        float gg = (fmaf(v[k], sc[k], sh[k]) > 0.f) ? g[k] : 0.f;
        s0[k] += gg;
        s1[k] += gg * ((v[k] - mu[k]) * is[k]);
      }
    }
  }
  const int lanes = t.lanes, lane = t.lane;
  const int row = CVB * V;
  const int chunk = RED / row;
  float fa[2] = {0.f, 0.f}, fb[2] = {0.f, 0.f};
  for (int base = 0; base < lanes; base += chunk) {
    __syncthreads();
    if (t.active && lane >= base && lane < base + chunk) {
#pragma unroll
      for (int k = 0; k < V; ++k) {
        red[0][(lane - base) * row + cvl * V + k] = s0[k];
        red[1][(lane - base) * row + cvl * V + k] = s1[k];
      }
    }
    __syncthreads();
    const int nl = lanes - base < chunk ? lanes - base : chunk;
#pragma unroll
    for (int u = 0; u < 2; ++u) {
      const int e = threadIdx.x + u * blockDim.x;
      if (e < row)
        for (int l = 0; l < nl; ++l) { fa[u] += red[0][l * row + e]; fb[u] += red[1][l * row + e]; }
    }
  }
#pragma unroll
  for (int u = 0; u < 2; ++u) {
    const int e = threadIdx.x + u * blockDim.x;
    const int ch = blockIdx.y * CVB * V + e;
    if (e < row && ch < C) {
      atomicAdd(sums + ch, (double)fa[u]);
      atomicAdd(sums + C + ch, (double)fb[u]);
    }
  }
}

__global__ void bn_bwd_finalize_kernel(const double* __restrict__ sums, double inv_count, int training,
                                       float* dgamma, float* dbeta, float* coef, int C) {
  int c = blockIdx.x * blockDim.x + threadIdx.x;
  if (c >= C) return;
  double sg = sums[c], sgx = sums[C + c];
  if (dbeta) dbeta[c] = (float)sg;
  if (dgamma) dgamma[c] = (float)sgx;
  coef[c] = training ? (float)(sg * inv_count) : 0.f;
  coef[C + c] = training ? (float)(sgx * inv_count) : 0.f;
}


template <typename T, int V>
__global__ void __launch_bounds__(256)
maxpool2_bwd_bnreduce_kernel(const T* __restrict__ x, int64_t ld_x, const T* __restrict__ gp, int64_t ld_gp,
                             T* __restrict__ gx, int64_t ld_gx, const T* __restrict__ y, int64_t ld_y,
                             const float* __restrict__ scale, const float* __restrict__ shift,
                             const float* __restrict__ mean, const float* __restrict__ invstd,
                             double* __restrict__ sums, int B, int H, int W, int C, int CV, int CVB) {
  constexpr int RED = (V == 8) ? 512 : 256;
  __shared__ float red[2][RED];
  const CsThread t = cs_thread(CV, CVB);
  const int cvl = threadIdx.x % CVB;
  float s0[V], s1[V];
#pragma unroll
  for (int k = 0; k < V; ++k) s0[k] = s1[k] = 0.f;
  if (t.active) {
    const int c = t.cv * V;
    float sc[V], sh[V], mu[V], is[V];
    ldf<V>(scale + c, sc);
    ldf<V>(shift + c, sh);
    ldf<V>(mean + c, mu);
    ldf<V>(invstd + c, is);
    const int Hc = (H + 1) >> 1, Wc = (W + 1) >> 1, Hp = H >> 1, Wp = W >> 1;
    const int64_t nwin = (int64_t)B * Hc * Wc;
    const int64_t stride = (int64_t)gridDim.x * t.lanes;
    for (int64_t wdx = (int64_t)blockIdx.x * t.lanes + t.lane; wdx < nwin; wdx += stride) {
      const int j = (int)(wdx % Wc);
      int64_t r = wdx / Wc;
      const int i = (int)(r % Hc);
      const int n = (int)(r / Hc);
      const bool full = (i < Hp && j < Wp);
      float g[V], m[V];
      int arg[V];
#pragma unroll
      for (int k = 0; k < V; ++k) { m[k] = -INFINITY; arg[k] = 0; g[k] = 0.f; }
      if (full) {
        ldv<T, V>(gp + (((int64_t)n * Hp + i) * Wp + j) * ld_gp + c, g);
#pragma unroll
        for (int q = 0; q < 4; ++q) {
          float v[V];
          ldv<T, V>(x + (((int64_t)n * H + 2 * i + (q >> 1)) * W + 2 * j + (q & 1)) * ld_x + c, v);
#pragma unroll
          for (int k = 0; k < V; ++k)
            if (v[k] > m[k] || v[k] != v[k]) { m[k] = v[k]; arg[k] = q; }
        }
      }
#pragma unroll
      for (int q = 0; q < 4; ++q) {
        const int h = 2 * i + (q >> 1), w = 2 * j + (q & 1);
        if (h < H && w < W) {
          const int64_t pix = ((int64_t)n * H + h) * W + w;
          float o[V], yv[V];
          ldv<T, V>(gx + pix * ld_gx + c, o);
          ldv<T, V>(y + pix * ld_y + c, yv);
#pragma unroll
          for (int k = 0; k < V; ++k) o[k] += (full && arg[k] == q) ? g[k] : 0.f;
          stv<T, V>(gx + pix * ld_gx + c, o);
#pragma unroll
          for (int k = 0; k < V; ++k) {
            const float gg = (fmaf(yv[k], sc[k], sh[k]) > 0.f) ? Elem<T>::round(o[k]) : 0.f;
            s0[k] += gg;
            s1[k] += gg * ((yv[k] - mu[k]) * is[k]);
          }
        }
      }
    }
  }
  const int lanes = t.lanes, lane = t.lane;
  const int row = CVB * V;
  const int chunk = RED / row;
  float fa[2] = {0.f, 0.f}, fb[2] = {0.f, 0.f};
  for (int base = 0; base < lanes; base += chunk) {
    __syncthreads();
    if (t.active && lane >= base && lane < base + chunk) {
#pragma unroll
      for (int k = 0; k < V; ++k) {
        red[0][(lane - base) * row + cvl * V + k] = s0[k];
        red[1][(lane - base) * row + cvl * V + k] = s1[k];
      }
    }
    __syncthreads();
    const int nl = lanes - base < chunk ? lanes - base : chunk;
#pragma unroll
    for (int u = 0; u < 2; ++u) {
      const int e = threadIdx.x + u * blockDim.x;
      if (e < row)
        for (int l = 0; l < nl; ++l) { fa[u] += red[0][l * row + e]; fb[u] += red[1][l * row + e]; }
    }
  }
#pragma unroll
  for (int u = 0; u < 2; ++u) {
    const int e = threadIdx.x + u * blockDim.x;
    const int ch = blockIdx.y * CVB * V + e;
    if (e < row && ch < C) {
      atomicAdd(sums + ch, (double)fa[u]);
      atomicAdd(sums + C + ch, (double)fb[u]);
    }
  }
}

template <typename T, int V>
__global__ void __launch_bounds__(256)
bn_relu_bwd_apply_kernel(const T* __restrict__ gz, int64_t ld_gz, const T* __restrict__ y, int64_t ld_y,
                         const float* __restrict__ scale, const float* __restrict__ shift,
                         const float* __restrict__ mean, const float* __restrict__ invstd,
                         const float* __restrict__ coef, T* __restrict__ gy, int64_t ld_gy, int64_t npix, int C,
                         int CV, int CVB) {
  const CsThread t = cs_thread(CV, CVB);
  if (!t.active) return;
  const int c = t.cv * V;
  float sc[V], sh[V], mu[V], A[V], B0[V];
  {
    float is[V], c0[V], c1[V];
    ldf<V>(scale + c, sc);
    ldf<V>(shift + c, sh);
    ldf<V>(mean + c, mu);
    ldf<V>(invstd + c, is);
    ldf<V>(coef + c, c0);
    ldf<V>(coef + C + c, c1);
#pragma unroll
    for (int k = 0; k < V; ++k) { A[k] = -sc[k] * c1[k] * is[k]; B0[k] = -sc[k] * c0[k]; }
  }
  const int64_t stride = (int64_t)gridDim.x * t.lanes;
  int64_t p = (int64_t)blockIdx.x * t.lanes + t.lane;
  for (; p + stride < npix; p += 2 * stride) {
    float g[2][V], v[2][V];
#pragma unroll
    for (int u = 0; u < 2; ++u) {
      ldv<T, V>(gz + (p + u * stride) * ld_gz + c, g[u]);
      ldv<T, V>(y + (p + u * stride) * ld_y + c, v[u]);
    }
#pragma unroll
    for (int u = 0; u < 2; ++u) {
#pragma unroll
      for (int k = 0; k < V; ++k) {
        float gg = (fmaf(v[u][k], sc[k], sh[k]) > 0.f) ? g[u][k] : 0.f;
        g[u][k] = fmaf(sc[k], gg, fmaf(A[k], v[u][k] - mu[k], B0[k]));
      }
      stv<T, V>(gy + (p + u * stride) * ld_gy + c, g[u]);
    }
  }
  for (; p < npix; p += stride) {
    float g[V], v[V];
    ldv<T, V>(gz + p * ld_gz + c, g);
    ldv<T, V>(y + p * ld_y + c, v);
#pragma unroll
    for (int k = 0; k < V; ++k) {
      float gg = (fmaf(v[k], sc[k], sh[k]) > 0.f) ? g[k] : 0.f;
      g[k] = fmaf(sc[k], gg, fmaf(A[k], v[k] - mu[k], B0[k]));
    }
    stv<T, V>(gy + p * ld_gy + c, g);
  }
}

struct Lerp { int i0, i1; float w0, w1; };
__device__ __forceinline__ Lerp lerp_coords(int o, int in_size, float s) {
  float src = s * (float)o;
  int i0 = (int)src;
  if (i0 > in_size - 1) i0 = in_size - 1;
  int i1 = i0 + (i0 < in_size - 1 ? 1 : 0);
  float l1 = src - (float)i0;
  return {i0, i1, 1.f - l1, l1};
}

template <typename T, int V>
__global__ void upsample2x_fwd_kernel(const T* __restrict__ x, int64_t ld_x, T* __restrict__ y, int64_t ld_y, int B,
                                      int h, int w, int CV, int Hout, int Wout, int off_y, int off_x, float sy,
                                      float sx) {
  const int H2 = 2 * h, W2 = 2 * w;
  const int64_t total = (int64_t)B * H2 * W2 * CV;
  for (int64_t idx = blockIdx.x * (int64_t)blockDim.x + threadIdx.x; idx < total;
       idx += (int64_t)gridDim.x * blockDim.x) {
// ... 202 lines not shown
  int i = blockIdx.x * blockDim.x + threadIdx.x;
  if (i < n) o[i] = (float)a[i];
}

}

using namespace ub;
typedef __nv_bfloat16 bf16;

#define UB_DTYPE_OK(dt) UB_CHECK_ARG((dt) == UNETB200_F32 || (dt) == UNETB200_BF16, "unsupported dtype %d", (int)(dt))

__device__ __forceinline__ float tf32_hi(float x) {
  const uint32_t u = __float_as_uint(x);
  return __uint_as_float((u + 0x1000u) & 0xffffe000u);
}

template <int V>
__global__ void __launch_bounds__(256) split_tf32_kernel(const float* __restrict__ x, int64_t ld_x, float* __restrict__ out,
                                                         int64_t npix, int CV, int pattern) {
  const int64_t total = npix * CV;
  const int C = CV * V;
  for (int64_t i = blockIdx.x * (int64_t)blockDim.x + threadIdx.x; i < total; i += (int64_t)gridDim.x * blockDim.x) {
    const int64_t p = i / CV;
    const int c = (int)(i - p * CV) * V;
    float v[V], hi[V], lo[V];
    if (V == 4) {
      const float4 t = *reinterpret_cast<const float4*>(x + p * ld_x + c);
      v[0] = t.x; v[1 % V] = t.y; v[2 % V] = t.z; v[3 % V] = t.w;
    } else {
      v[0] = x[p * ld_x + c];
    }
#pragma unroll
    for (int k = 0; k < V; ++k) { hi[k] = tf32_hi(v[k]); lo[k] = v[k] - hi[k]; }
    float* o = out + p * 3 * C + c;
    const float* g1 = pattern == 0 ? lo : hi;
    const float* g2 = pattern == 0 ? hi : lo;
    if (V == 4) {
      *reinterpret_cast<float4*>(o) = make_float4(hi[0], hi[1 % V], hi[2 % V], hi[3 % V]);
      *reinterpret_cast<float4*>(o + C) = make_float4(g1[0], g1[1 % V], g1[2 % V], g1[3 % V]);
      *reinterpret_cast<float4*>(o + 2 * C) = make_float4(g2[0], g2[1 % V], g2[2 % V], g2[3 % V]);
    } else {
      o[0] = hi[0]; o[C] = g1[0]; o[2 * C] = g2[0];
    }
  }
}

extern "C" {

int unetb200_bn_finalize_track(const double* stats, int64_t count, const float* gamma, const float* beta, float eps,
                               float momentum, float* running_mean, float* running_var, float* save_mean,
                               float* save_invstd, float* scale, float* shift, int64_t* num_batches_tracked, int C,
                               void* stream) {
  UB_CHECK_ARG(C > 0 && count > 0, "bn_finalize: C=%d count=%lld", C, (long long)count);
  double unbias = count > 1 ? (double)count / (double)(count - 1) : 1.0;
  bn_finalize_kernel<<<(C + 127) / 128, 128, 0, (cudaStream_t)stream>>>(
      stats, 1.0 / (double)count, unbias, gamma, beta, eps, momentum, running_mean, running_var, save_mean,
      save_invstd, scale, shift, C, reinterpret_cast<long long*>(num_batches_tracked));
  UB_LAUNCH_CHECK("bn_finalize");
  return 0;
}

int unetb200_bn_finalize(const double* stats, int64_t count, const float* gamma, const float* beta, float eps,
                         float momentum, float* running_mean, float* running_var, float* save_mean,
                         float* save_invstd, float* scale, float* shift, int C, void* stream) {
  return unetb200_bn_finalize_track(stats, count, gamma, beta, eps, momentum, running_mean, running_var, save_mean,
                                    save_invstd, scale, shift, nullptr, C, stream);
}

int unetb200_bn_eval_coeffs(const float* gamma, const float* beta, const float* running_mean,
                            const float* running_var, float eps, float* scale, float* shift, float* save_mean,
                            float* save_invstd, int C, void* stream) {
  UB_CHECK_ARG(C > 0, "bn_eval_coeffs: C=%d", C);
  bn_eval_coeffs_kernel<<<(C + 127) / 128, 128, 0, (cudaStream_t)stream>>>(gamma, beta, running_mean, running_var,
                                                                          eps, scale, shift, save_mean,
                                                                          save_invstd, C);
  UB_LAUNCH_CHECK("bn_eval_coeffs");
  return 0;
}

int unetb200_bn_relu_apply(const void* y, int64_t ld_y, const float* scale, const float* shift, void* z,
                           int64_t ld_z, void* pooled, int64_t ld_p, int dtype, int B, int H, int W, int C,
                           void* stream) {
  UB_DTYPE_OK(dtype);
  UB_CHECK_ARG(B > 0 && H > 0 && W > 0 && C > 0 && ld_y >= C && ld_z >= C, "bn_relu_apply: bad shape");
  cudaStream_t s = (cudaStream_t)stream;
  const int64_t npix = (int64_t)B * H * W;
#define GO(T, V)                                                                                              \
  do {                                                                                                        \
    int CV = C / V;                                                                                           \
    if (pooled) {                                                                                             \
      CsGeom g_ = cs_geom(CV, (int64_t)B * ((H + 1) / 2) * ((W + 1) / 2), 2);                                 \
      bn_relu_apply_pool_kernel<T, V><<<dim3(g_.gx, g_.gy), 256, 0, s>>>(                                     \
          (const T*)y, ld_y, scale, shift, (T*)z, ld_z, (T*)pooled, ld_p, B, H, W, CV, g_.CVB);               \
    } else {                                                                                                  \
      CsGeom g_ = cs_geom(CV, npix, 8);                                                                       \
      bn_relu_apply_kernel<T, V><<<dim3(g_.gx, g_.gy), 256, 0, s>>>((const T*)y, ld_y, scale, shift, (T*)z,   \
                                                                   ld_z, npix, CV, g_.CVB);                   \
    }                                                                                                         \
  } while (0)
  if (dtype == UNETB200_BF16) {
    if (vec_ok<bf16>(C, {ld_y, ld_z, pooled ? ld_p : 0}, {y, z, pooled})) GO(bf16, 8); else GO(bf16, 1);
  } else {
    if (vec_ok<float>(C, {ld_y, ld_z, pooled ? ld_p : 0}, {y, z, pooled})) GO(float, 8); else GO(float, 1);
  }
#undef GO
  UB_LAUNCH_CHECK("bn_relu_apply");
  return 0;
}

int unetb200_maxpool2_fwd(const void* x, int64_t ld_x, void* p, int64_t ld_p, int dtype, int B, int H, int W,
                          int C, void* stream) {
  UB_DTYPE_OK(dtype);
  UB_CHECK_ARG(B > 0 && H >= 2 && W >= 2 && C > 0, "maxpool2_fwd: bad shape %d %d %d %d", B, H, W, C);
  cudaStream_t s = (cudaStream_t)stream;
#define GO(T, V)                                                                                         \
  do {                                                                                                   \
    int CV = C / V;                                                                                      \
    int64_t work = (int64_t)B * (H / 2) * (W / 2) * CV;                                                  \
    maxpool2_fwd_kernel<T, V><<<grid_for(work, 256, 16), 256, 0, s>>>((const T*)x, ld_x, (T*)p, ld_p, B, \
                                                                      H, W, CV);                         \
  } while (0)
  if (dtype == UNETB200_BF16) {
    if (vec_ok<bf16>(C, {ld_x, ld_p}, {x, p})) GO(bf16, 8); else GO(bf16, 1);
  } else {
    if (vec_ok<float>(C, {ld_x, ld_p}, {x, p})) GO(float, 8); else GO(float, 1);
  }
#undef GO
  UB_LAUNCH_CHECK("maxpool2_fwd");
  return 0;
}

int unetb200_maxpool2_bwd(const void* x, int64_t ld_x, const void* gp, int64_t ld_gp, void* gx, int64_t ld_gx,
                          int accumulate, int dtype, int B, int H, int W, int C, void* stream) {
  UB_DTYPE_OK(dtype);
  UB_CHECK_ARG(B > 0 && H >= 2 && W >= 2 && C > 0, "maxpool2_bwd: bad shape");
  cudaStream_t s = (cudaStream_t)stream;
#define GO(T, V)                                                                                              \
  do {                                                                                                        \
    int CV = C / V;                                                                                           \
    int64_t work = (int64_t)B * ((H + 1) / 2) * ((W + 1) / 2) * CV;                                           \
    if (accumulate)                                                                                           \
      maxpool2_bwd_kernel<T, V, true><<<grid_for(work, 256, 16), 256, 0, s>>>(                                \
          (const T*)x, ld_x, (const T*)gp, ld_gp, (T*)gx, ld_gx, B, H, W, CV);                                \
    else                                                                                                      \
      maxpool2_bwd_kernel<T, V, false><<<grid_for(work, 256, 16), 256, 0, s>>>(                               \
          (const T*)x, ld_x, (const T*)gp, ld_gp, (T*)gx, ld_gx, B, H, W, CV);                                \
  } while (0)
  if (dtype == UNETB200_BF16) {
    if (vec_ok<bf16>(C, {ld_x, ld_gp, ld_gx}, {x, gp, gx})) GO(bf16, 8); else GO(bf16, 1);
  } else {
    if (vec_ok<float>(C, {ld_x, ld_gp, ld_gx}, {x, gp, gx})) GO(float, 8); else GO(float, 1);
  }
#undef GO
  UB_LAUNCH_CHECK("maxpool2_bwd");
  return 0;
}

int unetb200_maxpool2_bwd_bnreduce(const void* x, int64_t ld_x, const void* gp, int64_t ld_gp, void* gx, int64_t ld_gx,
                                   const void* y, int64_t ld_y, const float* scale, const float* shift, const float* mean,
                                   const float* invstd, double* sums, int dtype, int B, int H, int W, int C, void* stream) {
  UB_DTYPE_OK(dtype);
  UB_CHECK_ARG(B > 0 && H >= 2 && W >= 2 && C > 0 && x && gp && gx && y && scale && shift && mean && invstd && sums,
               "maxpool2_bwd_bnreduce: bad args");
  cudaStream_t s = (cudaStream_t)stream;
  const int64_t nwin = (int64_t)B * ((H + 1) / 2) * ((W + 1) / 2);
#define GO(T, V)                                                                                              \
  do {                                                                                                        \
    const int CV = (C + V - 1) / V;                                                                           \
    CsGeom g_ = cs_geom(CV, nwin, 2, V == 8 ? 64 : 256);                                                      \
    maxpool2_bwd_bnreduce_kernel<T, V><<<dim3(g_.gx, g_.gy), 256, 0, s>>>(                                    \
        (const T*)x, ld_x, (const T*)gp, ld_gp, (T*)gx, ld_gx, (const T*)y, ld_y, scale, shift, mean, invstd, \
        sums, B, H, W, C, CV, g_.CVB);                                                                        \
  } while (0)
  if (dtype == UNETB200_BF16) {
    if (vec_ok<bf16>(C, {ld_x, ld_gp, ld_gx, ld_y}, {x, gp, gx, y})) GO(bf16, 8); else GO(bf16, 1);
  } else {
    if (vec_ok<float>(C, {ld_x, ld_gp, ld_gx, ld_y}, {x, gp, gx, y})) GO(float, 8); else GO(float, 1);
  }
#undef GO
  UB_LAUNCH_CHECK("maxpool2_bwd_bnreduce");
  return 0;
}

int unetb200_bn_relu_bwd_reduce(const void* gz, int64_t ld_gz, const void* y, int64_t ld_y, const float* scale,
                                const float* shift, const float* mean, const float* invstd, double* sums,
                                int dtype, int B, int H, int W, int C, void* stream) {
  UB_DTYPE_OK(dtype);
  UB_CHECK_ARG(B > 0 && H > 0 && W > 0 && C > 0, "bn_relu_bwd_reduce: bad shape");
  cudaStream_t s = (cudaStream_t)stream;
  const int64_t npix = (int64_t)B * H * W;
#define GO(T, V)                                                                                              \
  do {                                                                                                        \
    int CV = C / V;                                                                                           \
    CsGeom g_ = cs_geom(CV, npix, 8, V == 8 ? 64 : 256);      \
    bn_relu_bwd_reduce_kernel<T, V><<<dim3(g_.gx, g_.gy), 256, 0, s>>>(                                       \
        (const T*)gz, ld_gz, (const T*)y, ld_y, scale, shift, mean, invstd, sums, npix, C, CV, g_.CVB);       \
  } while (0)
  if (dtype == UNETB200_BF16) {
    if (vec_ok<bf16>(C, {ld_gz, ld_y}, {gz, y})) GO(bf16, 8); else GO(bf16, 1);
  } else {
    if (vec_ok<float>(C, {ld_gz, ld_y}, {gz, y})) GO(float, 8); else GO(float, 1);
  }
#undef GO
  UB_LAUNCH_CHECK("bn_relu_bwd_reduce");
  return 0;
}

int unetb200_bn_bwd_finalize(const double* sums, int64_t count, int training, float* dgamma, float* dbeta,
                             float* coef, int C, void* stream) {
  UB_CHECK_ARG(C > 0 && count > 0, "bn_bwd_finalize: bad shape");
  bn_bwd_finalize_kernel<<<(C + 127) / 128, 128, 0, (cudaStream_t)stream>>>(sums, 1.0 / (double)count, training,
                                                                            dgamma, dbeta, coef, C);
  UB_LAUNCH_CHECK("bn_bwd_finalize");
  return 0;
}

int unetb200_bn_relu_bwd_apply(const void* gz, int64_t ld_gz, const void* y, int64_t ld_y, const float* scale,
                               const float* shift, const float* mean, const float* invstd, const float* coef,
                               void* gy, int64_t ld_gy, int dtype, int B, int H, int W, int C, void* stream) {
  UB_DTYPE_OK(dtype);
  UB_CHECK_ARG(B > 0 && H > 0 && W > 0 && C > 0, "bn_relu_bwd_apply: bad shape");
  cudaStream_t s = (cudaStream_t)stream;
  const int64_t npix = (int64_t)B * H * W;
#define GO(T, V)                                                                                             \
  do {                                                                                                       \
    int CV = C / V;                                                                                          \
    CsGeom g_ = cs_geom(CV, npix, 8);                                                                        \
    bn_relu_bwd_apply_kernel<T, V><<<dim3(g_.gx, g_.gy), 256, 0, s>>>(                                       \
        (const T*)gz, ld_gz, (const T*)y, ld_y, scale, shift, mean, invstd, coef, (T*)gy, ld_gy, npix, C, CV,  \
        g_.CVB);                                                                                             \
  } while (0)
  if (dtype == UNETB200_BF16) {
    if (vec_ok<bf16>(C, {ld_gz, ld_y, ld_gy}, {gz, y, gy})) GO(bf16, 8); else GO(bf16, 1);
  } else {
    if (vec_ok<float>(C, {ld_gz, ld_y, ld_gy}, {gz, y, gy})) GO(float, 8); else GO(float, 1);
  }
#undef GO
  UB_LAUNCH_CHECK("bn_relu_bwd_apply");
  return 0;
}

static inline float ac_scale(int in, int out) { return out > 1 ? (float)(in - 1) / (float)(out - 1) : 0.f; }

int unetb200_upsample2x_fwd(const void* x, int64_t ld_x, void* y, int64_t ld_y, int dtype, int B, int h, int w,
                            int C, int Hout, int Wout, int off_y, int off_x, void* stream) {
  UB_DTYPE_OK(dtype);
  UB_CHECK_ARG(B > 0 && h > 0 && w > 0 && C > 0 && off_y >= 0 && off_x >= 0 && 2 * h + off_y <= Hout &&
                   2 * w + off_x <= Wout,
               "upsample2x_fwd: bad shape");
  cudaStream_t s = (cudaStream_t)stream;
  float sy = ac_scale(h, 2 * h), sx = ac_scale(w, 2 * w);
#define GO(T, V)                                                                                           \
  do {                                                                                                     \
    int CV = C / V;                                                                                        \
    int64_t work = (int64_t)B * 4 * h * w * CV;                                                            \
    upsample2x_fwd_kernel<T, V><<<grid_for(work, 256, 16), 256, 0, s>>>(                                   \
        (const T*)x, ld_x, (T*)y, ld_y, B, h, w, CV, Hout, Wout, off_y, off_x, sy, sx);                    \
  } while (0)
  if (dtype == UNETB200_BF16) {
    if (vec_ok<bf16>(C, {ld_x, ld_y}, {x, y})) GO(bf16, 8); else GO(bf16, 1);
  } else {
    if (vec_ok<float>(C, {ld_x, ld_y}, {x, y})) GO(float, 8); else GO(float, 1);
  }
#undef GO
  UB_LAUNCH_CHECK("upsample2x_fwd");
  return 0;
}

int unetb200_upsample2x_bwd(const void* gy, int64_t ld_gy, void* gx, int64_t ld_gx, int dtype, int B, int h,
                            int w, int C, int Hout, int Wout, int off_y, int off_x, void* stream) {
  UB_DTYPE_OK(dtype);
  UB_CHECK_ARG(B > 0 && h > 0 && w > 0 && C > 0 && off_y >= 0 && off_x >= 0 && 2 * h + off_y <= Hout &&
                   2 * w + off_x <= Wout,
               "upsample2x_bwd: bad shape");
  cudaStream_t s = (cudaStream_t)stream;
  float sy = ac_scale(h, 2 * h), sx = ac_scale(w, 2 * w);
#define GO(T, V)                                                                                           \
  do {                                                                                                     \
    int CV = C / V;                                                                                        \
    int64_t work = (int64_t)B * h * w * CV;                                                                \
    upsample2x_bwd_kernel<T, V><<<grid_for(work, 128, 16), 128, 0, s>>>(                                   \
        (const T*)gy, ld_gy, (T*)gx, ld_gx, B, h, w, CV, Hout, Wout, off_y, off_x, sy, sx);                \
  } while (0)
  if (dtype == UNETB200_BF16) {
    if (vec_ok<bf16>(C, {ld_gy, ld_gx}, {gy, gx})) GO(bf16, 8); else GO(bf16, 1);
  } else {
    if (vec_ok<float>(C, {ld_gy, ld_gx}, {gy, gx})) GO(float, 8); else GO(float, 1);
  }
#undef GO
  UB_LAUNCH_CHECK("upsample2x_bwd");
  return 0;
}
// ... 152 lines not shown
```

unet-medical-image-contour-segmentation_b200/csrc/gconv.cuh:

```cuda
#pragma once
#include "common.cuh"

namespace ub {

struct GconvDev {
  int B, Hm, Wm, Cin, ntaps;
  int tap_dy[9], tap_dx[9];
  int in_scale, in_off_y, in_off_x, Hin, Win;
  long long ld_in;
  int N, nquad, Cq, out_scale, out_off_y, out_off_x, Hout, Wout;
  long long ld_out;
  long long M;
  int K;
};

int gconv_validate(const unetb200_gconv_t* d, GconvDev* out);

inline int pick_splits(long long tiles, int slots, long long smax) {
  if (tiles < 1) tiles = 1;
  if (smax < 1) smax = 1;
  long long lim = (4LL * slots + tiles - 1) / tiles;
  if (lim > smax) lim = smax;
  if (lim > 512) lim = 512;
  if (lim < 1) lim = 1;
  double best = -1.0;
  long long pick = 1;
  for (long long s = 1; s <= lim; ++s) {
    const long long ctas = tiles * s;
    const long long waves = (ctas + slots - 1) / slots;
    const double eff = (double)ctas / (double)(waves * slots);
    if (eff > best + 1e-9 || (eff > best - 0.005 && ctas <= 2LL * slots)) { best = eff > best ? eff : best; pick = s; }
  }
  return (int)pick;
}

int tc_fprop_supported(const unetb200_gconv_t* d, const void* x, const void* wp, const void* y);
int tc_wgrad_supported(const unetb200_gconv_t* d, const void* x, const void* gy);
int launch_stats_reduce(const float* ws, long long ntiles, int C2, double* stats, cudaStream_t s);

int tc2_fprop_supported(const unetb200_gconv_t* d, const void* x, const void* wp, const void* y);
long long tc2_stats_workspace(const unetb200_gconv_t* d);
int tc2_fprop(const unetb200_gconv_t* d, const GconvDev& g, const void* x, const void* wp, const float* bias, void* y,
              double* stats, float* stats_ws, cudaStream_t stream);

int tc2_wgrad_supported(const unetb200_gconv_t* d, const void* x, const void* gy);
int tc2_wgrad_splits(const unetb200_gconv_t* d);
int tc2_wgrad(const unetb200_gconv_t* d, const GconvDev& g, const void* x, const void* gy, float* partials, int splits,
              cudaStream_t stream);

int tc3_fprop_supported(const unetb200_gconv_t* d, const void* x, const void* wp, const float* bias, const void* y);
long long tc3_stats_workspace(const unetb200_gconv_t* d);
struct Tc3OutConv {
  const float* w;
  const float* b;
  void* logits;
  int ncls;
};
int tc3_affine_outconv_supported(const unetb200_gconv_t* d, int ncls);
int tc3_fprop(const unetb200_gconv_t* d, const GconvDev& g, const void* x, const void* wp, void* y, double* stats,
              float* stats_ws, cudaStream_t stream, const float* affine = nullptr, const void* yprev = nullptr,
              long long ld_yprev = 0, const float* bnc = nullptr, const Tc3OutConv* oc = nullptr, void* pooled = nullptr,
              long long ld_pool = 0);
int tc3_bnbwd_supported(const unetb200_gconv_t* d);

int tc3_wgrad_supported(const unetb200_gconv_t* d, const void* x, const void* gy);
int tc3_wgrad_splits(const unetb200_gconv_t* d);
int tc3_wgrad(const unetb200_gconv_t* d, const GconvDev& g, const void* x, const void* gy, float* partials, int splits,
              cudaStream_t stream);

int tc4_wgrad_supported(const unetb200_gconv_t* d, const void* x, const void* gy);
int tc4_wgrad_preferred(const unetb200_gconv_t* d);
int tc4_wgrad_splits(const unetb200_gconv_t* d);
int tc4_wgrad(const unetb200_gconv_t* d, const GconvDev& g, const void* x, const void* gy, float* partials, int splits,
              cudaStream_t stream);

int first_tc_supported(const unetb200_gconv_t* d, const void* y);
long long first_tc_stats_rows(const unetb200_gconv_t* d);
int first_tc_fprop(const unetb200_gconv_t* d, const void* x, const void* wp, void* y, double* stats, float* stats_ws,
                   const float* affine, cudaStream_t s);

int narrow_tc_supported(const unetb200_gconv_t* d, const void* x, const void* wp, const void* y);
long long narrow_tc_stats_rows(const unetb200_gconv_t* d);
int narrow_tc_fprop(const unetb200_gconv_t* d, const void* x, const void* wp, void* y, double* stats, float* stats_ws,
                    const float* affine, cudaStream_t s);

int halo_fprop_supported(const unetb200_gconv_t* d, const void* x, const void* wp, const void* y);
long long halo_stats_rows(const unetb200_gconv_t* d);
int halo_fprop(const unetb200_gconv_t* d, const void* x, const void* wp, void* y, double* stats, float* stats_ws,
               const float* affine, cudaStream_t s, const void* yprev = nullptr, long long ld_yprev = 0,
               const float* bnc = nullptr, void* pooled = nullptr, long long ld_pool = 0);
int halo_bnbwd_supported(const unetb200_gconv_t* d, const void* g, const void* wp, const void* gx);
int halo_wgrad_supported(const unetb200_gconv_t* d, const void* x, const void* gy);
int halo_wgrad_splits(const unetb200_gconv_t* d);
int halo_wgrad(const unetb200_gconv_t* d, const void* x, const void* gy, float* partials, int splits, cudaStream_t s);
int first_narrow_supported(const unetb200_gconv_t* d, const void* y);
long long first_narrow_rows(const unetb200_gconv_t* d);
int first_narrow_fprop(const unetb200_gconv_t* d, const void* x, const void* wp, void* y, double* stats, float* stats_ws,
                       const float* affine, cudaStream_t s);
int first_narrow_wgrad_splits(const unetb200_gconv_t* d);
int first_narrow_wgrad(const unetb200_gconv_t* d, const void* x, const void* gy, float* partials, int splits, cudaStream_t s);
int fprop_narrow_f32_supported(const unetb200_gconv_t* d, const void* x, const void* wp, const void* y);
long long fprop_narrow_f32_rows(const unetb200_gconv_t* d);
int fprop_narrow_f32(const unetb200_gconv_t* d, const void* x, const void* wp, void* y, double* stats, float* stats_ws,
                     cudaStream_t s);
int wgrad_narrow_f32_supported(const unetb200_gconv_t* d, const void* x, const void* gy);
int wgrad_narrow_f32_splits(const unetb200_gconv_t* d);
int wgrad_narrow_f32(const unetb200_gconv_t* d, const void* x, const void* gy, float* partials, int splits, cudaStream_t s);
int halo_t_fprop_supported(const unetb200_gconv_t* d, const void* x, const void* wp, const void* y);
int halo_t_fprop(const unetb200_gconv_t* d, const void* x, const void* wp, const float* bias, void* y, cudaStream_t s);
int halo_t_dgrad_supported(const unetb200_gconv_t* d, const void* g, const void* wp, const void* gx);
int halo_t_dgrad(const unetb200_gconv_t* d, const void* g, const void* wp, void* gx, cudaStream_t s);
int halo_t_wgrad_supported(const unetb200_gconv_t* d, const void* x, const void* gy);
int halo_t_wgrad_splits(const unetb200_gconv_t* d);
int halo_t_wgrad(const unetb200_gconv_t* d, const void* x, const void* gy, float* partials, int splits, cudaStream_t s);
int narrow_wgrad_supported(const unetb200_gconv_t* d, const void* x, const void* gy);
// ... 14 lines not shown
```

unet-medical-image-contour-segmentation_b200/unetb200/_lib.py:

```python
from __future__ import annotations

import ctypes as C
import os

_HERE = os.path.dirname(os.path.abspath(__file__))
LIB_PATH = os.path.join(_HERE, "libunetb200.so")

F32, BF16, I64, U8 = 0, 1, 2, 3
ALGO_AUTO, ALGO_SIMT, ALGO_TC, ALGO_PREFER_TC = 0, 1, 2, 3
E_INVALID, E_CUDA, E_NOMEM = -1, -2, -3

c_i64 = C.c_int64
c_p = C.c_void_p


class GConv(C.Structure):
    _fields_ = [
        ("dtype", C.c_int32), ("algo", C.c_int32),
        ("B", C.c_int32), ("Hm", C.c_int32), ("Wm", C.c_int32),
        ("Cin", C.c_int32), ("ntaps", C.c_int32),
        ("tap_dy", C.c_int32 * 9), ("tap_dx", C.c_int32 * 9),
        ("in_scale", C.c_int32), ("in_off_y", C.c_int32), ("in_off_x", C.c_int32),
        ("Hin", C.c_int32), ("Win", C.c_int32), ("ld_in", c_i64),
        ("N", C.c_int32), ("nquad", C.c_int32), ("out_scale", C.c_int32),
        ("out_off_y", C.c_int32), ("out_off_x", C.c_int32),
        ("Hout", C.c_int32), ("Wout", C.c_int32), ("ld_out", c_i64),
    ]


class PackJob(C.Structure):
    _fields_ = [("src", c_p), ("dst", c_p), ("n0", c_i64), ("n1", c_i64), ("n2", c_i64),
                ("s0", c_i64), ("s1", c_i64), ("s2", c_i64), ("off", c_i64)]


class ReduceJob(C.Structure):
    _fields_ = [("partials", c_p), ("dst", c_p), ("st", c_i64), ("sc", c_i64), ("sq", c_i64), ("sn", c_i64),
                ("splits", C.c_int32), ("ntaps", C.c_int32), ("Cin", C.c_int32), ("N", C.c_int32), ("Cq", C.c_int32),
                ("accumulate", C.c_int32)]


PROTOTYPES = {
    "unetb200_version": (C.c_int, []),
    "unetb200_last_error": (C.c_char_p, []),
    "unetb200_device_info": (C.c_int, [C.POINTER(C.c_int)] * 3),
    "unetb200_gconv_stats_workspace": (c_i64, [C.POINTER(GConv)]),
    "unetb200_gconv_fprop": (C.c_int, [C.POINTER(GConv), c_p, c_p, c_p, c_p, c_p, c_p, C.POINTER(C.c_int), c_p]),
    "unetb200_gconv_fprop_affine_relu_supported": (C.c_int, [C.POINTER(GConv), c_p, c_p, c_p]),
    "unetb200_gconv_fprop_affine_relu": (C.c_int, [C.POINTER(GConv), c_p, c_p, c_p, c_p, c_p]),
    "unetb200_gconv_fprop_affine_relu_pool_supported": (C.c_int, [C.POINTER(GConv), c_p, c_p, c_p, c_p, C.c_int64]),
    "unetb200_gconv_fprop_affine_relu_pool": (C.c_int, [C.POINTER(GConv), c_p, c_p, c_p, c_p, c_p, C.c_int64, c_p]),
    "unetb200_gconv_fprop_affine_relu_outconv_supported": (C.c_int, [C.POINTER(GConv), c_p, c_p, C.c_int]),
    "unetb200_gconv_fprop_affine_relu_outconv": (C.c_int, [C.POINTER(GConv), c_p, c_p, c_p, c_p, c_p, c_p, C.c_int, c_p]),
    "unetb200_wgrad_reduce_multi": (C.c_int, [C.POINTER(ReduceJob), C.c_int, c_p]),
    "unetb200_gconv_dgrad_bnbwd_supported": (C.c_int, [C.POINTER(GConv), c_p, c_p, c_p]),
    "unetb200_gconv_dgrad_bnbwd": (C.c_int, [C.POINTER(GConv), c_p, c_p, c_p, c_p, C.c_int64, c_p, c_p, c_p, c_p]),
    "unetb200_gconv_wgrad_plan": (C.c_int, [C.POINTER(GConv), C.POINTER(C.c_int), C.POINTER(C.c_int)]),
    "unetb200_gconv_wgrad": (C.c_int, [C.POINTER(GConv), c_p, c_p, c_p, C.c_int, c_p]),
    "unetb200_wgrad_reduce": (C.c_int, [c_p, C.c_int, C.c_int, C.c_int, C.c_int, C.c_int, c_p, c_i64, c_i64, c_i64, c_i64,
                                        C.c_int, c_p]),
    "unetb200_pack_weights": (C.c_int, [c_p, c_p, C.c_int, c_i64, c_i64, c_i64, c_i64, c_i64, c_i64, c_i64, c_p]),
    "unetb200_pack_weights_multi": (C.c_int, [C.POINTER(PackJob), C.c_int, C.c_int, c_p]),
    "unetb200_split_tf32": (C.c_int, [c_p, c_i64, c_p, c_i64, C.c_int, C.c_int, c_p]),
    "unetb200_bn_finalize": (C.c_int, [c_p, c_i64, c_p, c_p, C.c_float, C.c_float, c_p, c_p, c_p, c_p, c_p, c_p, C.c_int, c_p]),
    "unetb200_bn_finalize_track": (C.c_int, [c_p, c_i64, c_p, c_p, C.c_float, C.c_float, c_p, c_p, c_p, c_p, c_p, c_p, c_p,
                                             C.c_int, c_p]),
    "unetb200_bn_eval_coeffs": (C.c_int, [c_p, c_p, c_p, c_p, C.c_float, c_p, c_p, c_p, c_p, C.c_int, c_p]),
    "unetb200_bn_relu_apply": (C.c_int, [c_p, c_i64, c_p, c_p, c_p, c_i64, c_p, c_i64, C.c_int, C.c_int, C.c_int, C.c_int, C.c_int, c_p]),
    "unetb200_maxpool2_fwd": (C.c_int, [c_p, c_i64, c_p, c_i64, C.c_int, C.c_int, C.c_int, C.c_int, C.c_int, c_p]),
    "unetb200_maxpool2_bwd": (C.c_int, [c_p, c_i64, c_p, c_i64, c_p, c_i64, C.c_int, C.c_int, C.c_int, C.c_int, C.c_int, C.c_int, c_p]),
    "unetb200_bn_relu_bwd_reduce": (C.c_int, [c_p, c_i64, c_p, c_i64, c_p, c_p, c_p, c_p, c_p, C.c_int, C.c_int, C.c_int, C.c_int, C.c_int, c_p]),
    "unetb200_bn_bwd_finalize": (C.c_int, [c_p, c_i64, C.c_int, c_p, c_p, c_p, C.c_int, c_p]),
    "unetb200_bn_relu_bwd_apply": (C.c_int, [c_p, c_i64, c_p, c_i64, c_p, c_p, c_p, c_p, c_p, c_p, c_i64, C.c_int, C.c_int, C.c_int, C.c_int, C.c_int, c_p]),
    "unetb200_bn_peer_group_create": (C.c_int, [C.c_int, C.c_int, C.c_int, c_p, c_p, C.POINTER(c_p)]),
    "unetb200_bn_peer_group_open": (C.c_int, [c_p, c_p, c_p]),
    "unetb200_bn_peer_group_destroy": (C.c_int, [c_p]),
    "unetb200_bn_peer_group_status": (C.c_int, [c_p, C.POINTER(c_i64), C.POINTER(c_i64)]),
    "unetb200_bn_sync_finalize": (C.c_int, [c_p, c_p, c_i64, c_p, c_p, C.c_float, C.c_float, c_p, c_p, c_p, c_p, c_p, c_p,
                                            c_p, C.c_int, c_p]),
    "unetb200_bn_sync_bwd_finalize": (C.c_int, [c_p, c_p, c_i64, c_p, c_p, c_p, C.c_int, c_p]),
    "unetb200_upsample2x_fwd": (C.c_int, [c_p, c_i64, c_p, c_i64, C.c_int] + [C.c_int] * 8 + [c_p]),
    "unetb200_upsample2x_bwd": (C.c_int, [c_p, c_i64, c_p, c_i64, C.c_int] + [C.c_int] * 8 + [c_p]),
    "unetb200_gather_nhwc": (C.c_int, [c_p, C.c_int, c_i64, c_i64, c_i64, c_i64, c_p, C.c_int, c_i64, C.c_int, C.c_int, C.c_int, C.c_int, c_p]),
    "unetb200_copy_channels": (C.c_int, [c_p, C.c_int, c_i64, c_p, C.c_int, c_i64, c_i64, C.c_int, c_p]),
    "unetb200_zero_channels": (C.c_int, [c_p, C.c_int, c_i64, c_i64, C.c_int, c_p]),
    "unetb200_sa_forward": (C.c_int, [c_p, c_i64, c_p, c_p, c_p, c_p, c_i64, C.c_int, C.c_int, C.c_int, C.c_int, C.c_int, c_p]),
    "unetb200_sa_backward_workspace": (c_i64, [C.c_int, C.c_int, C.c_int]),
    "unetb200_sa_backward": (C.c_int, [c_p, c_i64, c_p, c_i64, c_p, c_p, c_p, c_p, c_i64, c_p, c_p, C.c_int, C.c_int, C.c_int,
                                       C.c_int, C.c_int, c_p]),
    "unetb200_maxpool2_bwd_bnreduce": (C.c_int, [c_p, c_i64, c_p, c_i64, c_p, c_i64, c_p, c_i64, c_p, c_p, c_p, c_p, c_p,
                                                 C.c_int, C.c_int, C.c_int, C.c_int, C.c_int, c_p]),
    "unetb200_f64_to_f32": (C.c_int, [c_p, c_p, C.c_int, c_p]),
    "unetb200_channel_sum": (C.c_int, [c_p, C.c_int, c_i64, c_i64, C.c_int, c_p, c_p, c_p]),
    "unetb200_add_channels": (C.c_int, [c_p, c_i64, c_p, c_i64, C.c_int, c_i64, C.c_int, c_p]),
    "unetb200_outconv_fwd": (C.c_int, [c_p, c_i64, c_p, c_p, c_p, C.c_int, c_i64, C.c_int, C.c_int, c_p]),
    "unetb200_outconv_bwd_workspace": (c_i64, [c_i64, C.c_int, C.c_int]),
    "unetb200_outconv_bwd": (C.c_int, [c_p, c_i64, c_p, c_p, c_p, c_i64, c_p, c_p, c_p, C.c_int, c_i64, C.c_int, C.c_int, c_p]),
    "unetb200_outconv_bwd_bnbwd_supported": (C.c_int, [c_p, c_i64, c_p, c_i64, c_p, c_i64, C.c_int, C.c_int, C.c_int]),
    "unetb200_outconv_bwd_bnbwd": (C.c_int, [c_p, c_i64, c_p, c_p, c_p, c_i64, c_p, c_p, c_p, c_p, c_i64, c_p, c_p, C.c_int,
                                             c_i64, C.c_int, C.c_int, c_p]),
    "unetb200_ce_dice_fwd": (C.c_int, [c_p, C.c_int, c_p, c_i64, C.c_int, C.c_float, c_p, c_p, c_p, c_p]),
    "unetb200_ce_dice_bwd": (C.c_int, [c_p, C.c_int, c_p, c_i64, C.c_int, c_p, c_p, c_p, c_p]),
    "unetb200_dice_fwd": (C.c_int, [c_p, c_p, c_i64, c_i64, C.c_float, c_p, c_p, c_p, c_p]),
    "unetb200_dice_bwd": (C.c_int, [c_p, c_p, c_i64, c_i64, C.c_float, c_p, c_p, c_p, c_p]),
    "unetb200_boundary_loss": (C.c_int, [c_p, C.c_int, c_i64, c_i64, c_i64, c_p, C.c_int, c_i64, c_i64, c_i64,
                                         C.c_int, C.c_int, C.c_int, C.c_int, C.c_float, C.c_float, c_p, c_p, c_p]),
    "unetb200_boundary_work_bytes": (c_i64, []),
    "unetb200_grad_sqnorm": (C.c_int, [c_p, c_p, C.c_int, c_p, c_p]),
    "unetb200_rmsprop_step": (C.c_int, [c_p, c_p, c_p, c_p, c_p, C.c_int, c_p, C.c_float, C.c_float, C.c_float, C.c_float,
                                        C.c_float, C.c_float, C.c_int, c_p]),
    "unetb200_eval_counts": (C.c_int, [c_p, C.c_int, c_i64, c_i64, c_i64, c_i64, c_p, C.c_int, C.c_int, C.c_int,
                                       C.c_int, C.c_int, C.c_int, C.c_int, c_p, C.c_int, c_p, C.c_float, c_p, c_p]),
    "unetb200_resize_argmax": (C.c_int, [c_p, C.c_int, c_i64, c_i64, c_i64, c_i64] + [C.c_int] * 6 + [c_p, C.c_int, c_p]),
    "unetb200_preprocess_image_u8": (C.c_int, [c_p, C.c_int, C.c_int, C.c_int, C.c_int, c_p, C.c_int, c_p, c_p, c_p]),
    "unetb200_preprocess_mask_u8": (C.c_int, [c_p, C.c_int, C.c_int, C.c_int, c_p, C.c_int, c_p, c_p, c_p]),
}

_lib = None


class UnetB200Error(RuntimeError):
    pass


def load():
    global _lib
# ... 28 lines not shown
```

unet-medical-image-contour-segmentation_b200/unetb200/functional.py:

```python
from __future__ import annotations

import os

import torch

from . import _lib, ops
from ._lib import ALGO_AUTO, ALGO_PREFER_TC, ALGO_SIMT


def compute_dtype(x):
    if torch.is_autocast_enabled("cuda") or x.dtype == torch.bfloat16:
        return torch.bfloat16
    return torch.float32


def conv_algo(dtype):
    if dtype == torch.bfloat16:
        return ALGO_AUTO
    mode = os.environ.get("UNET_B200_PRECISION", "").lower()
    if mode == "":
        mode = "tf32" if torch.backends.cudnn.allow_tf32 else "fp32"
    if mode in ("tf32", "tf32x3"):
        return ALGO_PREFER_TC
    if mode == "fp32":
# ... 269 lines not shown
    ent = _EVAL_COEFS.get(id(bn))
    if ent is not None and ent[0]() is bn and ent[1] == key and not torch.cuda.is_current_stream_capturing():
        return ent[2]
    gamma = _f32c(bn.weight) if bn.weight is not None else None
    beta = _f32c(bn.bias) if bn.bias is not None else None
    coefs = ops.bn_eval_coeffs(gamma, beta, bn.running_mean, bn.running_var, bn.eps, Cout)
    if len(_EVAL_COEFS) > 512:
        for k in [k for k, e in _EVAL_COEFS.items() if e[0]() is None]:
            del _EVAL_COEFS[k]
    if not torch.cuda.is_current_stream_capturing():
        _EVAL_COEFS[id(bn)] = (weakref.ref(bn), key, coefs)
    return coefs


def sync_peer(bn, training, device):
    if not training or not isinstance(bn, torch.nn.SyncBatchNorm):
        return None
    from . import ddp
    return ddp.bn_sync_group(bn, device)


def conv_bn_relu_fwd(x, w, bn, training, out=None, want_pool=False, fold=False, outconv=None, peer=None):
    B, Cin, H, W = x.shape
    Cout = w.shape[0]
    cd, dev = x.dtype, x.device
    wp = pack3x3_fprop(w, cd)
    if fold and not (training or bn.running_mean is None) and Cout % 2 == 0:
        if outconv is not None and out is None and not want_pool:
            ow, ob = outconv
            K = ow.shape[0]
            d = ops.make_gconv(ops._DT[cd], conv_algo(cd), B, H, W, Cin, ops.TAPS3, 1, (0, 0), H, W, ops.nhwc_ld(x),
                               Cout, 1, 1, (0, 0), H, W, Cout)
            if tuple(ow.shape[1:]) == (Cout, 1, 1) and ops.gconv_fprop_affine_relu_outconv_supported(d, x, wp, K):
                coefs = _eval_coefs(bn, Cout)
                logits = torch.empty((B, H, W, K), dtype=cd, device=dev)
                ops.gconv_fprop_affine_relu_outconv(d, x, wp, coefs, _f32c(ow).view(K, Cout),
                                                    _f32c(ob) if ob is not None else None, logits)
                return None, logits.permute(0, 3, 1, 2), None, coefs, True
        z = out if out is not None else ops.empty_nhwc(B, Cout, H, W, cd, dev)
        d = _gconv3x3(x, Cout, z, cd)
        if ops.gconv_fprop_affine_relu_supported(d, x, wp, z):
            coefs = _eval_coefs(bn, Cout)
            pooled = ops.empty_nhwc(B, Cout, H // 2, W // 2, cd, dev) if want_pool else None
            if pooled is not None and ops.gconv_fprop_affine_relu_pool_supported(d, x, wp, z, pooled):
                ops.gconv_fprop_affine_relu(d, x, wp, coefs, z, pooled)
            else:
                ops.gconv_fprop_affine_relu(d, x, wp, coefs, z)
                if pooled is not None:
                    ops.maxpool2_fwd(z, pooled)
            return None, z, pooled, coefs, False
    y = ops.empty_nhwc(B, Cout, H, W, cd, dev)
    use_batch = training or bn.running_mean is None
    stats = zeros_f64(2 * Cout, dev) if use_batch else None
    ops.gconv_fprop(_gconv3x3(x, Cout, y, cd), x, wp, None, y, stats)
    gamma = _f32c(bn.weight) if bn.weight is not None else None
    beta = _f32c(bn.bias) if bn.bias is not None else None
    if use_batch:
        if bn.momentum is None and bn.running_mean is not None and training:
            raise ValueError(f"unetb200: {type(bn).__name__}(momentum=None) (cumulative average) is not supported")
        update = training and bn.running_mean is not None and not _RECOMPUTE[0]
        args = (stats, B * H * W, gamma, beta, bn.eps, bn.momentum if update else 0.0,
                bn.running_mean if update else None, bn.running_var if update else None, Cout)
        nbt = bn.num_batches_tracked if update else None
        if peer is None:
            coefs = ops.bn_finalize(*args, num_batches_tracked=nbt)
        else:
            coefs = ops.bn_sync_finalize(peer, *args, num_batches_tracked=nbt)
        if update:
            torch._C._increment_version([bn.running_mean, bn.running_var])
    else:
        coefs = ops.bn_eval_coeffs(gamma, beta, bn.running_mean, bn.running_var, bn.eps, Cout)
    z = out if out is not None else ops.empty_nhwc(B, Cout, H, W, cd, dev)
    pooled = ops.empty_nhwc(B, Cout, H // 2, W // 2, cd, dev) if want_pool else None
    ops.bn_relu_apply(y, coefs, z, pooled)
    return y, z, pooled, coefs, False


def _grad_kept_as_is(param, dW):
    if getattr(param, "grad", None) is not None or torch.is_grad_enabled():
        return False
    if dW.stride() != param.stride() or param.dtype != torch.float32 or dW.dtype != torch.float32:
        return False
    if getattr(param, "_backward_hooks", None) or getattr(param, "_post_accumulate_grad_hooks", None):
        return False
    return True


def _sink_owns(param, dW):
    ent = _GRAD_SINK.get(id(param))
    return (ent is not None and ent[0]() is param and ent[2] and dW.data_ptr() == ent[1].data_ptr()
            and not torch.is_grad_enabled())


def _defer_mode(param, dW, kept, side):
    if side:
        return False
    if _sink_owns(param, dW):
        return "pass"
    return "call" if kept else False


def _vec_dst(param, Cc):
    if param is None:
        return None
    d = grad_dst(param)
    return d if d is not None and d.dim() == 1 and d.numel() == Cc and d.is_contiguous() else None


def conv_bn_relu_bwd(gz, x, y, w, coefs, batch_stats, need_gx, param=None, bn_params=(None, None), sums=None,
                     below=None, colsum=None, peer=None):
    param = w if param is None else param
    B, Cin, H, W = x.shape
    Cout = w.shape[0]
    cd = x.dtype
    gy, dgamma, dbeta = ops.bn_relu_bwd(gz, y, coefs, batch_stats, _vec_dst(bn_params[0], Cout),
                                        _vec_dst(bn_params[1], Cout), sums=sums, peer=peer)
    dW = grad_dst(param)
    if dW is None:
        dW = torch.empty_like(w, dtype=torch.float32)
    so, si, skh, skw = dW.stride()
    if skh != 3 * skw or dW.shape != (Cout, Cin, 3, 3):
        dW = torch.empty((Cout, Cin, 3, 3), dtype=torch.float32, device=x.device)
        so, si, skh, skw = dW.stride()
# ... 343 lines not shown
```

unet-medical-image-contour-segmentation_b200/unetb200/ops.py:

```python
from __future__ import annotations

import contextlib
import ctypes as C
import os

import torch

from . import _lib
from ._lib import ALGO_AUTO, ALGO_SIMT, ALGO_TC, BF16, F32, I64, GConv

_DT = {torch.float32: F32, torch.bfloat16: BF16}
_ESZ = {torch.float32: 4, torch.bfloat16: 2}

LAUNCHES = 0
_PROFILE = None


@contextlib.contextmanager
def profile():
    global _PROFILE
    prev, _PROFILE = _PROFILE, []
    try:
        yield _PROFILE
    finally:
# ... 268 lines not shown

def x3_active(d):
    return d.dtype == F32 and d.algo in (ALGO_TC, _lib.ALGO_PREFER_TC) and d.Cin >= 16 and x3_mode()


def x3_split(x):
    B, Cc, H, W = x.shape
    out = empty_nhwc(B, 3 * Cc, H, W, torch.float32, x.device)
    _run("split_tf32", lib().unetb200_split_tf32, _p(x), nhwc_ld(x), _p(out), B * H * W, Cc, 0, _stream(),
         nbytes=16.0 * x.numel())
    return out


def x3_split_rows(wp, rows, Cc):
    out = torch.empty((rows * 3 * Cc,), dtype=torch.float32, device=wp.device)
    _run("split_tf32_w", lib().unetb200_split_tf32, _p(wp), Cc, _p(out), rows, Cc, 1, _stream(), nbytes=16.0 * rows * Cc)
    return out


def _x3_desc(d, ld_in=None, ld_out=None, triple=True):
    d3 = GConv.from_buffer_copy(d)
    if triple:
        d3.Cin = 3 * d.Cin
    if ld_in is not None:
        d3.ld_in = ld_in
    if ld_out is not None:
        d3.ld_out = ld_out
    return d3


def gconv_fprop(d, x, wp, bias, y, stats, kind="fprop", x_split=None):
    used = C.c_int(0)
    ws = None
    flops, nbytes = gconv_flops(d), gconv_bytes(d, 2 if d.dtype == BF16 else 4)
    tag = _shape_tag(d)
    if x3_active(d):
        xs = x_split if x_split is not None else x3_split(x)
        wp = x3_split_rows(wp, d.N * d.ntaps, d.Cin)
        d = _x3_desc(d, ld_in=3 * d.Cin)
        x = xs
        kind = kind + "_x3"
    if stats is not None:
        n = lib().unetb200_gconv_stats_workspace(C.byref(d))
        if n < 0:
            _lib.check(-1, "gconv_stats_workspace")
        ws = torch.empty(n, dtype=torch.float32, device=x.device)
    _run(f"conv_{kind}", lib().unetb200_gconv_fprop, C.byref(d), _p(x), _p(wp), _p(bias), _p(y), _p(stats), _p(ws),
         C.byref(used), _stream(), kernels=2 if stats is not None else 1, flops=flops, nbytes=nbytes)
    if _PROFILE is not None:
        _PROFILE[-1][0] = f"conv_{kind}_{_ALGO_NAME.get(used.value, '?')}" + tag
    return used.value


def gconv_fprop_affine_relu_supported(d, x, wp, z):
    if x3_active(d):
        d = _x3_desc(d, ld_in=3 * d.Cin)
    return bool(lib().unetb200_gconv_fprop_affine_relu_supported(C.byref(d), _p(x), _p(wp), _p(z)))


def gconv_fprop_affine_relu_pool_supported(d, x, wp, z, pooled):
    return (not x3_active(d)) and bool(lib().unetb200_gconv_fprop_affine_relu_pool_supported(
        C.byref(d), _p(x), _p(wp), _p(z), _p(pooled), nhwc_ld(pooled)))


def gconv_fprop_affine_relu(d, x, wp, coefs, z, pooled=None):
    flops, nbytes = gconv_flops(d), gconv_bytes(d, 2 if d.dtype == BF16 else 4)
    tag = _shape_tag(d)
    if pooled is not None:
        _run("conv_fprop_bnfold", lib().unetb200_gconv_fprop_affine_relu_pool, C.byref(d), _p(x), _p(wp), _prow(coefs, 2),
             _p(z), _p(pooled), nhwc_ld(pooled), _stream(), flops=flops,
             nbytes=nbytes + float(pooled.numel()) * pooled.element_size())
        if _PROFILE is not None:
            _PROFILE[-1][0] = "conv_fprop_bnfold_tc" + tag
        return
    if x3_active(d):
        x = x3_split(x)
        wp = x3_split_rows(wp, d.N * d.ntaps, d.Cin)
        d = _x3_desc(d, ld_in=3 * d.Cin)
    _run("conv_fprop_bnfold", lib().unetb200_gconv_fprop_affine_relu, C.byref(d), _p(x), _p(wp), _prow(coefs, 2), _p(z),
         _stream(), flops=flops, nbytes=nbytes)
    if _PROFILE is not None:
        _PROFILE[-1][0] = "conv_fprop_bnfold_tc" + tag


def gconv_fprop_affine_relu_outconv_supported(d, x, wp, ncls):
    return (not x3_active(d)) and bool(lib().unetb200_gconv_fprop_affine_relu_outconv_supported(C.byref(d), _p(x), _p(wp), ncls))


def gconv_fprop_affine_relu_outconv(d, x, wp, coefs, oc_w, oc_b, logits):
    flops, tag = gconv_flops(d), _shape_tag(d)
    ncls = oc_w.shape[0]
    es = 2 if d.dtype == BF16 else 4
    _run("conv_fprop_bnfold", lib().unetb200_gconv_fprop_affine_relu_outconv, C.byref(d), _p(x), _p(wp), _prow(coefs, 2),
         _p(oc_w), _p(oc_b), _p(logits), ncls, _stream(), flops=flops,
         nbytes=float(es) * d.B * d.Hin * d.Win * d.Cin + float(es) * d.B * d.Hm * d.Wm * ncls)
    if _PROFILE is not None:
        _PROFILE[-1][0] = "conv_fprop_bnfold_tc" + tag


def gconv_dgrad_bnbwd_supported(d, g, wp, gx):
    return (not x3_active(d)) and bool(lib().unetb200_gconv_dgrad_bnbwd_supported(C.byref(d), _p(g), _p(wp), _p(gx)))


def gconv_dgrad_bnbwd(d, g, wp, gx, yprev, coefs_prev):
    flops, nbytes = gconv_flops(d), gconv_bytes(d, 2 if d.dtype == BF16 else 4)
    tag = _shape_tag(d)
    sums = torch.zeros((2, d.N), dtype=torch.float64, device=g.device)
    n = lib().unetb200_gconv_stats_workspace(C.byref(d))
    if n < 0:
        _lib.check(-1, "gconv_stats_workspace")
    ws = torch.empty(n, dtype=torch.float32, device=g.device)
    if not coefs_prev.is_contiguous():
        raise ValueError("unetb200: BatchNorm coefficients must be a contiguous [4, C] tensor")
    _run("conv_dgrad_tc" + tag, lib().unetb200_gconv_dgrad_bnbwd, C.byref(d), _p(g), _p(wp), _p(gx), _p(yprev),
         nhwc_ld(yprev), _p(coefs_prev), _p(sums), _p(ws), _stream(), kernels=2, flops=flops,
         nbytes=nbytes + float(yprev.numel()) * yprev.element_size())
    return sums


_REDUCE_JOBS = []
_REDUCE_PENDING = [None]
_CALL_JOBS = [None]
DEFER_REDUCE = _os.environ.get("UNETB200_DEFER_REDUCE", "1") != "0"


def graph_task():
    return torch._C._current_graph_task_id() if hasattr(torch._C, "_current_graph_task_id") else None


def _reduce_multi(jobs):
    if not jobs:
        return
    arr = (_lib.ReduceJob * len(jobs))()
    nbytes = 0.0
    for j, (partials, dst, st, sc, sq, sn, splits, ntaps, Cin, N, Cq) in enumerate(jobs):
        arr[j].partials, arr[j].dst = partials.data_ptr(), dst
        arr[j].st, arr[j].sc, arr[j].sq, arr[j].sn = st, sc, sq, sn
        arr[j].splits, arr[j].ntaps, arr[j].Cin, arr[j].N, arr[j].Cq, arr[j].accumulate = splits, ntaps, Cin, N, Cq, 0
        nbytes += 4.0 * ntaps * Cin * N * (splits + 1)
    n = len(jobs)
    _run("wgrad_reduce", lib().unetb200_wgrad_reduce_multi, arr, n, _stream(), nbytes=nbytes, kernels=(n + 31) // 32)


def flush_wgrad_reduce():
    _REDUCE_PENDING[0] = None
    try:
        _reduce_multi(_REDUCE_JOBS)
    finally:
        _REDUCE_JOBS.clear()


@contextlib.contextmanager
def reductions_at_return():
    prev, _CALL_JOBS[0] = _CALL_JOBS[0], []
    try:
        yield
        jobs = _CALL_JOBS[0]
    finally:
        _CALL_JOBS[0] = prev
    _reduce_multi(jobs)
# ... 108 lines not shown
    _run("bn_eval_coeffs", lib().unetb200_bn_eval_coeffs, _p(gamma), _p(beta), _p(running_mean), _p(running_var),
         eps, _prow(coefs, 2), _prow(coefs, 3), _prow(coefs, 0), _prow(coefs, 1), Cc, _stream())
    return coefs


def bn_relu_apply(y, coefs, z, pooled=None):
    B, Cc, H, W = y.shape
    es = y.element_size()
    _run("bn_relu_apply_pool" if pooled is not None else "bn_relu_apply", lib().unetb200_bn_relu_apply, _p(y),
         nhwc_ld(y), _prow(coefs, 2), _prow(coefs, 3), _p(z), nhwc_ld(z), _p(pooled),
         nhwc_ld(pooled) if pooled is not None else 0, dt(y), B, H, W, Cc, _stream(),
         nbytes=y.numel() * es * (2.25 if pooled is not None else 2.0))


def maxpool2_fwd(x, p):
    B, Cc, H, W = x.shape
    _run("maxpool2_fwd", lib().unetb200_maxpool2_fwd, _p(x), nhwc_ld(x), _p(p), nhwc_ld(p), dt(x), B, H, W, Cc,
         _stream(), nbytes=x.numel() * x.element_size() * 1.25)


def maxpool2_bwd(x, gp, gx, accumulate):
    B, Cc, H, W = x.shape
    _run("maxpool2_bwd", lib().unetb200_maxpool2_bwd, _p(x), nhwc_ld(x), _p(gp), nhwc_ld(gp), _p(gx), nhwc_ld(gx),
         1 if accumulate else 0, dt(x), B, H, W, Cc, _stream(),
         nbytes=x.numel() * x.element_size() * (3.25 if accumulate else 2.25))


POOL_BNBWD_FUSE = _os.environ.get("UNETB200_POOL_BNBWD_FUSE", "0") != "0" and _os.environ.get("UNETB200_NO_BNBWD_FUSE") is None


def maxpool2_bwd_bnreduce(x, gp, gx, y, coefs):
    B, Cc, H, W = x.shape
    sums = torch.zeros((2, Cc), dtype=torch.float64, device=x.device)
    _run("maxpool2_bwd", lib().unetb200_maxpool2_bwd_bnreduce, _p(x), nhwc_ld(x), _p(gp), nhwc_ld(gp), _p(gx), nhwc_ld(gx),
         _p(y), nhwc_ld(y), _prow(coefs, 2), _prow(coefs, 3), _prow(coefs, 0), _prow(coefs, 1), _p(sums), dt(x), B, H, W, Cc,
         _stream(), nbytes=x.numel() * x.element_size() * 4.25)
    return sums


def bn_relu_bwd(gz, y, coefs, training, dgamma=None, dbeta=None, sums=None, peer=None):
    B, Cc, H, W = y.shape
    dev = y.device
    es = y.element_size()
    L = lib()
    if sums is None:
        sums = torch.zeros((2, Cc), dtype=torch.float64, device=dev)
        _run("bn_relu_bwd_reduce", L.unetb200_bn_relu_bwd_reduce, _p(gz), nhwc_ld(gz), _p(y), nhwc_ld(y), _prow(coefs, 2),
             _prow(coefs, 3), _prow(coefs, 0), _prow(coefs, 1), _p(sums), dt(y), B, H, W, Cc, _stream(),
             nbytes=2.0 * y.numel() * es)
    if dgamma is None:
        dgamma = torch.empty(Cc, dtype=torch.float32, device=dev)
    if dbeta is None:
        dbeta = torch.empty(Cc, dtype=torch.float32, device=dev)
    coef = torch.empty((2, Cc), dtype=torch.float32, device=dev)
    if peer is not None:
        bn_sync_bwd_finalize(peer, sums, B * H * W, dgamma, dbeta, coef)
    else:
        _run("bn_bwd_finalize", L.unetb200_bn_bwd_finalize, _p(sums), B * H * W, 1 if training else 0, _p(dgamma),
             _p(dbeta), _p(coef), Cc, _stream())
    gy = empty_nhwc(B, Cc, H, W, y.dtype, dev)
    _run("bn_relu_bwd_apply", L.unetb200_bn_relu_bwd_apply, _p(gz), nhwc_ld(gz), _p(y), nhwc_ld(y), _prow(coefs, 2),
         _prow(coefs, 3), _prow(coefs, 0), _prow(coefs, 1), _p(coef), _p(gy), nhwc_ld(gy), dt(y), B, H, W, Cc, _stream(),
         nbytes=3.0 * y.numel() * es)
    return gy, dgamma, dbeta


def upsample2x_fwd(x, y, off):
    B, Cc, h, w = x.shape
    _run("upsample2x_fwd", lib().unetb200_upsample2x_fwd, _p(x), nhwc_ld(x), _p(y), nhwc_ld(y), dt(x), B, h, w, Cc,
         y.shape[2], y.shape[3], off[0], off[1], _stream(), nbytes=5.0 * x.numel() * x.element_size())


def upsample2x_bwd(gy, gx, off):
    B, Cc, h, w = gx.shape
    _run("upsample2x_bwd", lib().unetb200_upsample2x_bwd, _p(gy), nhwc_ld(gy), _p(gx), nhwc_ld(gx), dt(gx), B, h, w,
         Cc, gy.shape[2], gy.shape[3], off[0], off[1], _stream(), nbytes=5.0 * gx.numel() * gx.element_size())


def sa_forward(x, w, out):
    B, Cc, H, W = x.shape
    stats = torch.empty((B, H, W, 2), dtype=torch.float32, device=x.device)
    gate = torch.empty((B, H, W), dtype=torch.float32, device=x.device)
    _run("sa_forward", lib().unetb200_sa_forward, _p(x), nhwc_ld(x), _p(w), _p(stats), _p(gate), _p(out), nhwc_ld(out),
         dt(x), B, H, W, Cc, _stream(), kernels=3, nbytes=3.0 * x.numel() * x.element_size())
    return stats, gate


def sa_backward(g, x, w, stats, gate, dx, dw):
    B, Cc, H, W = x.shape
    ws = torch.empty(lib().unetb200_sa_backward_workspace(B, H, W), dtype=torch.float32, device=x.device)
    _run("sa_backward", lib().unetb200_sa_backward, _p(g), nhwc_ld(g), _p(x), nhwc_ld(x), _p(w), _p(stats), _p(gate),
         _p(dx), nhwc_ld(dx), _p(dw), _p(ws), dt(x), B, H, W, Cc, _stream(), kernels=5,
         nbytes=5.0 * x.numel() * x.element_size())


def outconv_fwd(x, w, bias, logits):
    B, Cc, H, W = x.shape
    K = w.shape[0]
    _run("outconv_fwd", lib().unetb200_outconv_fwd, _p(x), nhwc_ld(x), _p(w), _p(bias), _p(logits), dt(x), B * H * W,
         Cc, K, _stream(), nbytes=(x.numel() + logits.numel()) * x.element_size())


OUTCONV_FUSE = _os.environ.get("UNETB200_OUTCONV_FUSE", "0") != "0"


def outconv_bwd(x, w, glogits, gx, dw, dbias, below=None):
    B, Cc, H, W = x.shape
    K = w.shape[0]
    n = lib().unetb200_outconv_bwd_workspace(B * H * W, Cc, K)
    ws = torch.empty(n, dtype=torch.float32, device=x.device)
    if below is not None and gx is not None and OUTCONV_FUSE:
        yprev, coefs = below
        if coefs.is_contiguous() and lib().unetb200_outconv_bwd_bnbwd_supported(
# ... 11 lines not shown
```

Before: 707.8.

## Fold BatchNorm finalize into conv stats reduce and enable PDL launches

Folds the BatchNorm forward finalize (mean, invstd, scale/shift, running stats) into the tc3 stats-reduce kernel, so no separate finalize launch is needed. The conv epilogue now writes every stats workspace slot, which removes the workspace memset. The backward finalize is merged into the apply kernel. tc3 and reduce kernels launch with programmatic dependent launch (griddepcontrol) so consecutive kernels can overlap their prologues. Together these cut kernel launches and small serial gaps per BN layer, at the cost of more complex kernels and of correctness that depends on every workspace row being written.

```diff
diff --git a/include/unetb200.h b/include/unetb200.h
--- a/include/unetb200.h
+++ b/include/unetb200.h
@@ -48,6 +48,11 @@
 int unetb200_gconv_fprop(const unetb200_gconv_t* d, const void* x, const void* wp,
                          const float* bias, void* y, double* stats, float* stats_ws, int* algo_used,
                          void* stream);
+int unetb200_gconv_fprop_bn(const unetb200_gconv_t* d, const void* x, const void* wp, void* y, double* stats,
+                            float* stats_ws, int64_t count, const float* gamma, const float* beta, float eps,
+                            float momentum, float* running_mean, float* running_var, float* save_mean,
+                            float* save_invstd, float* scale, float* shift, int64_t* num_batches_tracked,
+                            int* algo_used, int* folded, void* stream);
 
 int unetb200_gconv_fprop_affine_relu_supported(const unetb200_gconv_t* d, const void* x, const void* wp,
                                                const void* z);
@@ -131,6 +136,11 @@
                                const float* scale, const float* shift, const float* mean,
                                const float* invstd, const float* coef, void* gy, int64_t ld_gy,
                                int dtype, int B, int H, int W, int C, void* stream);
+int unetb200_bn_relu_bwd_finalize_apply(const void* gz, int64_t ld_gz, const void* y, int64_t ld_y,
+                                        const float* scale, const float* shift, const float* mean,
+                                        const float* invstd, const double* sums, int training, float* dgamma,
+                                        float* dbeta, void* gy, int64_t ld_gy, int dtype, int B, int H, int W,
+                                        int C, void* stream);
 
 #define UNETB200_IPC_HANDLE_BYTES 64
 #define UNETB200_BUS_ID_BYTES 32
diff --git a/unet-medical-image-contour-segmentation_b200/csrc/common.cuh b/unet-medical-image-contour-segmentation_b200/csrc/common.cuh
--- a/unet-medical-image-contour-segmentation_b200/csrc/common.cuh
+++ b/unet-medical-image-contour-segmentation_b200/csrc/common.cuh
@@ -89,4 +89,78 @@
 
 inline bool aligned16(const void* p) { return (reinterpret_cast<uintptr_t>(p) & 15) == 0; }
 
+__device__ __forceinline__ void pdl_wait() { asm volatile("griddepcontrol.wait;" ::: "memory"); }
+__device__ __forceinline__ void pdl_launch_dependents() { asm volatile("griddepcontrol.launch_dependents;" ::: "memory"); }
+
+bool pdl_enabled();
+
+template <typename... P, typename... A>
+cudaError_t launch_pdl(void (*kernel)(P...), dim3 grid, dim3 block, size_t smem, cudaStream_t s, int cluster,
+                       A&&... args) {
+  cudaLaunchConfig_t cfg = {};
+  cfg.gridDim = grid;
+  cfg.blockDim = block;
+  cfg.dynamicSmemBytes = smem;
+  cfg.stream = s;
+  cudaLaunchAttribute at[2];
+  int n = 0;
+  at[n].id = cudaLaunchAttributeProgrammaticStreamSerialization;
+  at[n].val.programmaticStreamSerializationAllowed = pdl_enabled() ? 1 : 0;
+  ++n;
+  if (cluster > 1) {
+    at[n].id = cudaLaunchAttributeClusterDimension;
+    at[n].val.clusterDim.x = (unsigned)cluster;
+    at[n].val.clusterDim.y = 1;
+    at[n].val.clusterDim.z = 1;
+    ++n;
+  }
+  cfg.attrs = at;
+  cfg.numAttrs = n;
+  return cudaLaunchKernelEx(&cfg, kernel, static_cast<P>(args)...);
 }
+
+struct BnFinalize {
+  const float* gamma;
+  const float* beta;
+  float eps, momentum;
+  double inv_count, unbias;
+  float* running_mean;
+  float* running_var;
+  float* mean;
+  float* invstd;
+  float* scale;
+  float* shift;
+  long long* num_batches_tracked;
+  int C;
+};
+
+__device__ __forceinline__ void bn_finalize_channel(const BnFinalize& f, int c, double sum, double sumsq) {
+  double mean = sum * f.inv_count;
+  double var = sumsq * f.inv_count - mean * mean;
+  if (var < 0) var = 0;
+  float invstd = (float)(1.0 / sqrt(var + (double)f.eps));
+  float g = f.gamma ? f.gamma[c] : 1.f, b = f.beta ? f.beta[c] : 0.f;
+  float sc = g * invstd;
+  f.mean[c] = (float)mean;
+  f.invstd[c] = invstd;
+  f.scale[c] = sc;
+  f.shift[c] = b - (float)mean * sc;
+  if (f.running_mean) f.running_mean[c] = (1.f - f.momentum) * f.running_mean[c] + f.momentum * (float)mean;
+  if (f.running_var) f.running_var[c] = (1.f - f.momentum) * f.running_var[c] + f.momentum * (float)(var * f.unbias);
+}
+
+inline BnFinalize make_bn_finalize(int64_t count, const float* gamma, const float* beta, float eps, float momentum,
+                                   float* running_mean, float* running_var, float* mean, float* invstd, float* scale,
+                                   float* shift, int64_t* num_batches_tracked, int C) {
+  BnFinalize f;
+  f.gamma = gamma; f.beta = beta; f.eps = eps; f.momentum = momentum;
+  f.inv_count = 1.0 / (double)count;
+  f.unbias = count > 1 ? (double)count / (double)(count - 1) : 1.0;
+  f.running_mean = running_mean; f.running_var = running_var;
+  f.mean = mean; f.invstd = invstd; f.scale = scale; f.shift = shift;
+  f.num_batches_tracked = reinterpret_cast<long long*>(num_batches_tracked);
+  f.C = C;
+  return f;
+}
+
+}
diff --git a/unet-medical-image-contour-segmentation_b200/csrc/conv_simt.cu b/unet-medical-image-contour-segmentation_b200/csrc/conv_simt.cu
--- a/unet-medical-image-contour-segmentation_b200/csrc/conv_simt.cu
+++ b/unet-medical-image-contour-segmentation_b200/csrc/conv_simt.cu
@@ -663,8 +663,9 @@
   return n > n7 ? n : n7;
 }
 
-int unetb200_gconv_fprop(const unetb200_gconv_t* d, const void* x, const void* wp, const float* bias, void* y,
-                         double* stats, float* stats_ws, int* algo_used, void* stream) {
+static int gconv_fprop_impl(const unetb200_gconv_t* d, const void* x, const void* wp, const float* bias, void* y,
+                            double* stats, float* stats_ws, int* algo_used, void* stream, const BnFinalize* bnf,
+                            int* folded) {
   GconvDev g;
   int rc = gconv_validate(d, &g);
   if (rc) return rc;
@@ -697,7 +698,13 @@
   if (algo_used) *algo_used = algo;
   if (algo == UNETB200_ALGO_TC) {
     UB_CHECK_ARG(tc_fprop_supported(d, x, wp, y), "gconv_fprop: tcgen05 path requested but shape/alignment unsupported");
-    if (tc3_fprop_supported(d, x, wp, bias, y)) return tc3_fprop(d, g, x, wp, y, stats, stats_ws, s);
+    if (tc3_fprop_supported(d, x, wp, bias, y)) {
+      if (bnf && stats && bnf->C == d->N) {
+        *folded = 1;
+        return tc3_fprop(d, g, x, wp, y, stats, stats_ws, s, nullptr, nullptr, 0, nullptr, nullptr, nullptr, 0, bnf);
+      }
+      return tc3_fprop(d, g, x, wp, y, stats, stats_ws, s);
+    }
     return tc2_fprop(d, g, x, wp, bias, y, stats, stats_ws, s);
   }
   UB_CHECK_ARG(algo == UNETB200_ALGO_SIMT, "gconv_fprop: unknown algo %d", algo);
@@ -718,6 +725,28 @@
   UB_LAUNCH_CHECK("gconv_fprop_simt");
   if (stats) return launch_stats_reduce(stats_ws, (g.M + fbm - 1) / fbm, 2 * g.N, stats, s);
   return 0;
+}
+
+int unetb200_gconv_fprop(const unetb200_gconv_t* d, const void* x, const void* wp, const float* bias, void* y,
+                         double* stats, float* stats_ws, int* algo_used, void* stream) {
+  return gconv_fprop_impl(d, x, wp, bias, y, stats, stats_ws, algo_used, stream, nullptr, nullptr);
+}
+
+int unetb200_gconv_fprop_bn(const unetb200_gconv_t* d, const void* x, const void* wp, void* y, double* stats,
+                            float* stats_ws, int64_t count, const float* gamma, const float* beta, float eps,
+                            float momentum, float* running_mean, float* running_var, float* save_mean,
+                            float* save_invstd, float* scale, float* shift, int64_t* num_batches_tracked,
+                            int* algo_used, int* folded, void* stream) {
+  UB_CHECK_ARG(stats && count > 0 && save_mean && save_invstd && scale && shift,
+               "gconv_fprop_bn: needs statistics, a count and the coefficient rows");
+  int fold = 0;
+  const BnFinalize f = make_bn_finalize(count, gamma, beta, eps, momentum, running_mean, running_var, save_mean,
+                                        save_invstd, scale, shift, num_batches_tracked, d->N);
+  int rc = gconv_fprop_impl(d, x, wp, nullptr, y, stats, stats_ws, algo_used, stream, &f, &fold);
+  if (folded) *folded = fold;
+  if (rc || fold) return rc;
+  return unetb200_bn_finalize_track(stats, count, gamma, beta, eps, momentum, running_mean, running_var, save_mean,
+                                    save_invstd, scale, shift, num_batches_tracked, d->N, stream);
 }
 
 int unetb200_gconv_fprop_affine_relu_supported(const unetb200_gconv_t* d, const void* x, const void* wp, const void* z) {
@@ -802,8 +831,11 @@
   UB_CHECK_ARG(unetb200_gconv_dgrad_bnbwd_supported(d, g, wp, gx),
                "gconv_dgrad_bnbwd: shape not covered by the fused kernel (query _supported first and run gconv_fprop + "
                "bn_relu_bwd_reduce instead)");
-  if (halo_bnbwd_supported(d, g, wp, gx))
+  if (halo_bnbwd_supported(d, g, wp, gx)) {
+    cudaError_t e = cudaMemsetAsync(sums, 0, 2 * sizeof(double) * (size_t)d->N, (cudaStream_t)stream);
+    if (e != cudaSuccess) return cuda_fail(e, "gconv_dgrad_bnbwd sums memset");
     return halo_fprop(d, g, wp, gx, sums, ws, nullptr, (cudaStream_t)stream, yprev, (long long)ld_yprev, coefs);
+  }
   return tc3_fprop(d, gd, g, wp, gx, sums, ws, (cudaStream_t)stream, nullptr, yprev, (long long)ld_yprev, coefs);
 }
 
diff --git a/unet-medical-image-contour-segmentation_b200/csrc/conv_tc3.cu b/unet-medical-image-contour-segmentation_b200/csrc/conv_tc3.cu
--- a/unet-medical-image-contour-segmentation_b200/csrc/conv_tc3.cu
+++ b/unet-medical-image-contour-segmentation_b200/csrc/conv_tc3.cu
@@ -199,6 +199,8 @@
     fence_barrier_init();
   }
   if (warp == 1) tmem_alloc_cg<CG>(tmem_slot, 512);
+  pdl_wait();
+  pdl_launch_dependents();
   if constexpr (OUTC) {
     float* ocs = reinterpret_cast<float*>(epi);
     for (int i = threadIdx.x; i < 64 * 8 + 8; i += blockDim.x) {
@@ -304,21 +306,23 @@
     for (int i = 0; i < NCB; ++i)
 #pragma unroll
       for (int j = 0; j < (TF32 ? 2 : 4); ++j) st[i][j] = 0.f;
-    auto flush = [&](int nb) {
-      if (!p.stats_ws || nb < 0) return;
-      float* dst = p.stats_ws + (((long long)nb * gridDim.x + blockIdx.x) * kEpi3Warps + ew) * 2 * BLOCK_N;
-#pragma unroll
-      for (int cb = 0; cb < NCB; ++cb) {
-        if constexpr (TF32) {
-          dst[cb * 32 + lane] = st[cb][0];
-          dst[BLOCK_N + cb * 32 + lane] = st[cb][1];
-          st[cb][0] = st[cb][1] = 0.f;
-        } else {
-          dst[cb * 64 + 2 * lane] = st[cb][0];
-          dst[BLOCK_N + cb * 64 + 2 * lane] = st[cb][1];
-          dst[cb * 64 + 2 * lane + 1] = st[cb][2];
-          dst[BLOCK_N + cb * 64 + 2 * lane + 1] = st[cb][3];
-          st[cb][0] = st[cb][1] = st[cb][2] = st[cb][3] = 0.f;
+    auto flush = [&](int nb_end) {
+      if (!p.stats_ws) return;
+      for (int nb = cur_nb < 0 ? 0 : cur_nb; nb < nb_end; ++nb) {
+        float* dst = p.stats_ws + (((long long)nb * gridDim.x + blockIdx.x) * kEpi3Warps + ew) * 2 * BLOCK_N;
+#pragma unroll
+        for (int cb = 0; cb < NCB; ++cb) {
+          if constexpr (TF32) {
+            dst[cb * 32 + lane] = st[cb][0];
+            dst[BLOCK_N + cb * 32 + lane] = st[cb][1];
+            st[cb][0] = st[cb][1] = 0.f;
+          } else {
+            dst[cb * 64 + 2 * lane] = st[cb][0];
+            dst[BLOCK_N + cb * 64 + 2 * lane] = st[cb][1];
+            dst[cb * 64 + 2 * lane + 1] = st[cb][2];
+            dst[BLOCK_N + cb * 64 + 2 * lane + 1] = st[cb][3];
+            st[cb][0] = st[cb][1] = st[cb][2] = st[cb][3] = 0.f;
+          }
         }
       }
     };
@@ -353,7 +357,7 @@
       const int b = mt / p.tiles_h;
       const int n0 = nb * BLOCK_N;
       if (nb != cur_nb) {
-        flush(cur_nb);
+        flush(nb);
         cur_nb = nb;
         if constexpr (BNBWD) {
 #pragma unroll
@@ -558,7 +562,7 @@
       }
       if (++acc == ACC) { acc = 0; pacc ^= 1; }
     }
-    flush(cur_nb);
+    flush(p.total_groups / p.m_groups);
     if (lane == 0) tma_store_wait_all();
   }
   tc_fence_before();
@@ -635,47 +639,45 @@
   if (int rc = set_max_dynamic_smem(reinterpret_cast<const void*>(&tc3_conv_kernel<T, BN, SA, SB, ACC, CG, TPS, EPI>), smem,
                                     "tc3_conv smem attribute"))
     return rc;
-  cudaLaunchConfig_t cfg = {};
-  cfg.gridDim = dim3((unsigned)grid);
-  cfg.blockDim = dim3(kTc3Threads);
-  cfg.dynamicSmemBytes = smem;
-  cfg.stream = s;
-  cudaLaunchAttribute at[1];
-  at[0].id = cudaLaunchAttributeClusterDimension;
-  at[0].val.clusterDim.x = CG;
-  at[0].val.clusterDim.y = 1;
-  at[0].val.clusterDim.z = 1;
-  cfg.attrs = at;
-  cfg.numAttrs = 1;
-  cudaError_t e = cudaLaunchKernelEx(&cfg, tc3_conv_kernel<T, BN, SA, SB, ACC, CG, TPS, EPI>, P);
+  cudaError_t e = launch_pdl(tc3_conv_kernel<T, BN, SA, SB, ACC, CG, TPS, EPI>, dim3((unsigned)grid), dim3(kTc3Threads),
+                             smem, s, CG, P);
   if (e != cudaSuccess) return cuda_fail(e, "tc3_conv launch");
   return 0;
 }
 
-__global__ void __launch_bounds__(1024) tc3_stats_reduce_kernel(const float* __restrict__ ws, int rows, int BN, int N, double* __restrict__ stats) {
+__global__ void __launch_bounds__(1024) tc3_stats_reduce_kernel(const float* __restrict__ ws, int rows, int BN, int N,
+                                                                double* __restrict__ stats, int accumulate,
+                                                                const BnFinalize f) {
   __shared__ double red[32][33];
+  pdl_wait();
+  pdl_launch_dependents();
   const int lane = threadIdx.x & 31, ry = threadIdx.x >> 5;
   const int nb = blockIdx.y;
-  const int col = blockIdx.x * 32 + lane;
+  const int which = lane >> 4, c = blockIdx.x * 16 + (lane & 15);
+  const int col = which * BN + c;
   double acc = 0.0;
-  if (col < 2 * BN) {
-    const float* base = ws + (long long)nb * rows * 2 * BN + col;
-    int r = ry;
-    for (; r + 96 < rows; r += 128) {
-      const float a = base[(long long)r * 2 * BN], b = base[(long long)(r + 32) * 2 * BN],
-                  c = base[(long long)(r + 64) * 2 * BN], d = base[(long long)(r + 96) * 2 * BN];
-      acc += (double)a; acc += (double)b; acc += (double)c; acc += (double)d;
-    }
-    for (; r < rows; r += 32) acc += (double)base[(long long)r * 2 * BN];
-  }
+  const float* base = ws + (long long)nb * rows * 2 * BN + col;
+  int r = ry;
+  for (; r + 96 < rows; r += 128) {
+    const float a = base[(long long)r * 2 * BN], b = base[(long long)(r + 32) * 2 * BN],
+                c4 = base[(long long)(r + 64) * 2 * BN], d = base[(long long)(r + 96) * 2 * BN];
+    acc += (double)a; acc += (double)b; acc += (double)c4; acc += (double)d;
+  }
+  for (; r < rows; r += 32) acc += (double)base[(long long)r * 2 * BN];
   red[ry][lane] = acc;
   __syncthreads();
-  if (ry == 0 && col < 2 * BN) {
+  if (ry == 0) {
     double s = 0.0;
 #pragma unroll
     for (int i = 0; i < 32; ++i) s += red[i][lane];
-    const int which = col / BN, c = col - which * BN;
-    stats[which * N + nb * BN + c] += s;
+    double* dst = stats + which * N + nb * BN + c;
+    if (accumulate) s += *dst;
+    *dst = s;
+    if (f.C) {
+      const double sq = __shfl_down_sync(0xffffffffu, s, 16);
+      if (which == 0) bn_finalize_channel(f, nb * BN + c, s, sq);
+      if (lane == 0 && blockIdx.x == 0 && nb == 0 && f.num_batches_tracked) *f.num_batches_tracked += 1;
+    }
   }
 }
 
@@ -693,8 +695,12 @@
 
 int tc3_fprop(const unetb200_gconv_t* d, const GconvDev& g, const void* x, const void* wp, void* y, double* stats,
               float* stats_ws, cudaStream_t stream, const float* affine, const void* yprev, long long ld_yprev,
-              const float* bnc, const Tc3OutConv* oc, void* pooled, long long ld_pool) {
+              const float* bnc, const Tc3OutConv* oc, void* pooled, long long ld_pool, const BnFinalize* bnf) {
   Tc3Plan pl;
+  if (bnf && (!stats || yprev || bnf->C != d->N)) {
+    set_error("tc3_fprop: the folded BatchNorm finalize needs the forward statistics of all N channels");
+    return UNETB200_E_INVALID;
+  }
   if (pooled && (!affine || oc || d->dtype != UNETB200_BF16 || (ld_pool & 1) || (reinterpret_cast<uintptr_t>(pooled) & 3))) {
     set_error("tc3_fprop: the pooled second output needs the bf16 affine epilogue and 4-byte aligned rows");
     return UNETB200_E_INVALID;
@@ -766,10 +772,6 @@
     return pl.BN == 128 ? tc3_launch<float, 128, 2, 6, 2, 1, 1, EPI_AFFINE>(P, pl.grid, stream)
                         : tc3_launch<float, 64, 3, 6, 2, 1, 1, EPI_AFFINE>(P, pl.grid, stream);
   }
-  if (stats) {
-    cudaError_t e = cudaMemsetAsync(stats_ws, 0, sizeof(float) * (size_t)tc3_stats_workspace(d), stream);
-    if (e != cudaSuccess) return cuda_fail(e, "tc3 stats workspace memset");
-  }
   if (yprev) {
     if (pl.CG != 2 || pl.BN == 256) { set_error("tc3_fprop: BatchNorm-backward epilogue: CTA pairs, N blocks of 64 / 128"); return UNETB200_E_INVALID; }
     static const int cfg64 = getenv("UNETB200_BNBWD64_CFG") ? atoi(getenv("UNETB200_BNBWD64_CFG")) : 1;
@@ -802,8 +804,10 @@
   if (rc) return rc;
   if (stats) {
     const int rows = pl.grid * kEpi3Warps;
-    tc3_stats_reduce_kernel<<<dim3((2 * pl.BN + 31) / 32, pl.n_blocks), 1024, 0, stream>>>(stats_ws, rows, pl.BN, d->N, stats);
-    cudaError_t e = cudaGetLastError();
+    BnFinalize f = {};
+    if (bnf) f = *bnf;
+    cudaError_t e = launch_pdl(tc3_stats_reduce_kernel, dim3(pl.BN / 16, pl.n_blocks), dim3(1024), 0, stream, 1,
+                               stats_ws, rows, pl.BN, d->N, stats, yprev ? 0 : 1, f);
     if (e != cudaSuccess) return cuda_fail(e, "tc3_stats_reduce");
   }
   return 0;
@@ -853,6 +857,8 @@
     fence_barrier_init();
   }
   if (warp == 1) tmem_alloc_cg<2>(tmem_slot, 512);
+  pdl_wait();
+  pdl_launch_dependents();
   tc_fence_before();
   __syncthreads();
   cluster_sync_all();
@@ -1027,19 +1033,9 @@
   if (int rc = deep ? set_max_dynamic_smem(reinterpret_cast<const void*>(&tc3_wgrad_kernel<7>), smem, "tc3_wgrad smem attribute")
                     : set_max_dynamic_smem(reinterpret_cast<const void*>(&tc3_wgrad_kernel<5>), smem, "tc3_wgrad smem attribute"))
     return rc;
-  cudaLaunchConfig_t cfg = {};
-  cfg.gridDim = dim3((unsigned)w.mpairs * 2, (unsigned)w.ntiles, (unsigned)splits);
-  cfg.blockDim = dim3(192);
-  cfg.dynamicSmemBytes = smem;
-  cfg.stream = stream;
-  cudaLaunchAttribute at[1];
-  at[0].id = cudaLaunchAttributeClusterDimension;
-  at[0].val.clusterDim.x = 2;
-  at[0].val.clusterDim.y = 1;
-  at[0].val.clusterDim.z = 1;
-  cfg.attrs = at;
-  cfg.numAttrs = 1;
-  cudaError_t e = deep ? cudaLaunchKernelEx(&cfg, tc3_wgrad_kernel<7>, P) : cudaLaunchKernelEx(&cfg, tc3_wgrad_kernel<5>, P);
+  const dim3 grid((unsigned)w.mpairs * 2, (unsigned)w.ntiles, (unsigned)splits);
+  cudaError_t e = deep ? launch_pdl(tc3_wgrad_kernel<7>, grid, dim3(192), smem, stream, 2, P)
+                       : launch_pdl(tc3_wgrad_kernel<5>, grid, dim3(192), smem, stream, 2, P);
   if (e != cudaSuccess) return cuda_fail(e, "tc3_wgrad launch");
   return 0;
 }
diff --git a/unet-medical-image-contour-segmentation_b200/csrc/conv_tc4.cu b/unet-medical-image-contour-segmentation_b200/csrc/conv_tc4.cu
--- a/unet-medical-image-contour-segmentation_b200/csrc/conv_tc4.cu
+++ b/unet-medical-image-contour-segmentation_b200/csrc/conv_tc4.cu
@@ -46,6 +46,8 @@
     fence_barrier_init();
   }
   if (warp == 1) tmem_alloc(tmem_slot, 512);
+  pdl_wait();
+  pdl_launch_dependents();
   tc_fence_before();
   __syncthreads();
   tc_fence_after();
@@ -218,8 +220,7 @@
   static_assert(smem <= 227 * 1024, "shared memory budget");
   if (int e = set_max_dynamic_smem(reinterpret_cast<const void*>(&tc4_wgrad_kernel<ST>), smem, "tc4_wgrad")) return e;
   dim3 grid((unsigned)(w.cchunks * w.ngroups), 1, (unsigned)splits);
-  tc4_wgrad_kernel<ST><<<grid, 192, smem, stream>>>(P);
-  cudaError_t e = cudaGetLastError();
+  cudaError_t e = launch_pdl(tc4_wgrad_kernel<ST>, grid, dim3(192), smem, stream, 1, P);
   if (e != cudaSuccess) return cuda_fail(e, "tc4_wgrad launch");
   return 0;
 }
diff --git a/unet-medical-image-contour-segmentation_b200/csrc/core.cu b/unet-medical-image-contour-segmentation_b200/csrc/core.cu
--- a/unet-medical-image-contour-segmentation_b200/csrc/core.cu
+++ b/unet-medical-image-contour-segmentation_b200/csrc/core.cu
@@ -20,6 +20,11 @@
 int cuda_fail(cudaError_t e, const char* what) {
   set_error("%s: %s (%s)", what, cudaGetErrorString(e), cudaGetErrorName(e));
   return e == cudaErrorMemoryAllocation ? UNETB200_E_NOMEM : UNETB200_E_CUDA;
+}
+
+bool pdl_enabled() {
+  static const bool on = getenv("UNETB200_NO_PDL") == nullptr;
+  return on;
 }
 
 int sm_count() {
diff --git a/unet-medical-image-contour-segmentation_b200/csrc/elementwise.cu b/unet-medical-image-contour-segmentation_b200/csrc/elementwise.cu
--- a/unet-medical-image-contour-segmentation_b200/csrc/elementwise.cu
+++ b/unet-medical-image-contour-segmentation_b200/csrc/elementwise.cu
@@ -62,26 +62,11 @@
   return true;
 }
 
-__global__ void bn_finalize_kernel(const double* __restrict__ stats, double inv_count, double unbias,
-                                   const float* __restrict__ gamma, const float* __restrict__ beta,
-                                   float eps, float momentum, float* running_mean, float* running_var,
-                                   float* save_mean, float* save_invstd, float* scale, float* shift, int C,
-                                   long long* num_batches_tracked) {
+__global__ void bn_finalize_kernel(const double* __restrict__ stats, const BnFinalize f) {
   int c = blockIdx.x * blockDim.x + threadIdx.x;
-  if (c == 0 && num_batches_tracked) *num_batches_tracked += 1;
-  if (c >= C) return;
-  double mean = stats[c] * inv_count;
-  double var = stats[C + c] * inv_count - mean * mean;
-  if (var < 0) var = 0;
-  float invstd = (float)(1.0 / sqrt(var + (double)eps));
-  float g = gamma ? gamma[c] : 1.f, b = beta ? beta[c] : 0.f;
-  float sc = g * invstd;
-  save_mean[c] = (float)mean;
-  save_invstd[c] = invstd;
-  scale[c] = sc;
-  shift[c] = b - (float)mean * sc;
-  if (running_mean) running_mean[c] = (1.f - momentum) * running_mean[c] + momentum * (float)mean;
-  if (running_var) running_var[c] = (1.f - momentum) * running_var[c] + momentum * (float)(var * unbias);
+  if (c == 0 && f.num_batches_tracked) *f.num_batches_tracked += 1;
+  if (c >= f.C) return;
+  bn_finalize_channel(f, c, stats[c], stats[f.C + c]);
 }
 
 __global__ void bn_eval_coeffs_kernel(const float* __restrict__ gamma, const float* __restrict__ beta,
@@ -116,6 +101,8 @@
 bn_relu_apply_kernel(const T* __restrict__ y, int64_t ld_y, const float* __restrict__ scale,
                      const float* __restrict__ shift, T* __restrict__ z, int64_t ld_z, int64_t npix, int CV,
                      int CVB) {
+  pdl_wait();
+  pdl_launch_dependents();
   const CsThread t = cs_thread(CV, CVB);
   if (!t.active) return;
   const int c = t.cv * V;
@@ -151,6 +138,8 @@
 bn_relu_apply_pool_kernel(const T* __restrict__ y, int64_t ld_y, const float* __restrict__ scale,
                           const float* __restrict__ shift, T* __restrict__ z, int64_t ld_z, T* __restrict__ pooled,
                           int64_t ld_p, int B, int H, int W, int CV, int CVB) {
+  pdl_wait();
+  pdl_launch_dependents();
   const CsThread t = cs_thread(CV, CVB);
   if (!t.active) return;
   const int c = t.cv * V;
@@ -235,6 +224,8 @@
 template <typename T, int V, bool ACC>
 __global__ void maxpool2_bwd_kernel(const T* __restrict__ x, int64_t ld_x, const T* __restrict__ gp, int64_t ld_gp,
                                     T* __restrict__ gx, int64_t ld_gx, int B, int H, int W, int CV) {
+  pdl_wait();
+  pdl_launch_dependents();
   const int Hc = (H + 1) >> 1, Wc = (W + 1) >> 1, Hp = H >> 1, Wp = W >> 1;
   const int64_t total = (int64_t)B * Hc * Wc * CV;
   for (int64_t idx = blockIdx.x * (int64_t)blockDim.x + threadIdx.x; idx < total;
@@ -286,6 +277,8 @@
                           const float* __restrict__ scale, const float* __restrict__ shift,
                           const float* __restrict__ mean, const float* __restrict__ invstd,
                           double* __restrict__ sums, int64_t npix, int C, int CV, int CVB) {
+  pdl_wait();
+  pdl_launch_dependents();
   constexpr int RED = (V == 8) ? 512 : 256;
   __shared__ float red[2][RED];
   const CsThread t = cs_thread(CV, CVB);
@@ -363,15 +356,20 @@
   }
 }
 
+__device__ __forceinline__ void bn_bwd_coef(const double* __restrict__ sums, int C, int c, double inv_count, int training,
+                                            float* dgamma, float* dbeta, float& c0, float& c1) {
+  double sg = sums[c], sgx = sums[C + c];
+  if (dbeta) dbeta[c] = (float)sg;
+  if (dgamma) dgamma[c] = (float)sgx;
+  c0 = training ? (float)(sg * inv_count) : 0.f;
+  c1 = training ? (float)(sgx * inv_count) : 0.f;
+}
+
 __global__ void bn_bwd_finalize_kernel(const double* __restrict__ sums, double inv_count, int training,
                                        float* dgamma, float* dbeta, float* coef, int C) {
   int c = blockIdx.x * blockDim.x + threadIdx.x;
   if (c >= C) return;
-  double sg = sums[c], sgx = sums[C + c];
-  if (dbeta) dbeta[c] = (float)sg;
-  if (dgamma) dgamma[c] = (float)sgx;
-  coef[c] = training ? (float)(sg * inv_count) : 0.f;
-  coef[C + c] = training ? (float)(sgx * inv_count) : 0.f;
+  bn_bwd_coef(sums, C, c, inv_count, training, dgamma, dbeta, coef[c], coef[C + c]);
 }
 
 
@@ -382,6 +380,8 @@
                              const float* __restrict__ scale, const float* __restrict__ shift,
                              const float* __restrict__ mean, const float* __restrict__ invstd,
                              double* __restrict__ sums, int B, int H, int W, int C, int CV, int CVB) {
+  pdl_wait();
+  pdl_launch_dependents();
   constexpr int RED = (V == 8) ? 512 : 256;
   __shared__ float red[2][RED];
   const CsThread t = cs_thread(CV, CVB);
@@ -475,12 +475,15 @@
 }
 
 template <typename T, int V>
-__global__ void __launch_bounds__(256)
+__global__ void __launch_bounds__(256, sizeof(T) == 2 ? 4 : 3)
 bn_relu_bwd_apply_kernel(const T* __restrict__ gz, int64_t ld_gz, const T* __restrict__ y, int64_t ld_y,
                          const float* __restrict__ scale, const float* __restrict__ shift,
                          const float* __restrict__ mean, const float* __restrict__ invstd,
                          const float* __restrict__ coef, T* __restrict__ gy, int64_t ld_gy, int64_t npix, int C,
-                         int CV, int CVB) {
+                         int CV, int CVB, const double* __restrict__ sums, double inv_count, int training,
+                         float* dgamma, float* dbeta) {
+  pdl_wait();
+  pdl_launch_dependents();
   const CsThread t = cs_thread(CV, CVB);
   if (!t.active) return;
   const int c = t.cv * V;
@@ -491,8 +494,15 @@
     ldf<V>(shift + c, sh);
     ldf<V>(mean + c, mu);
     ldf<V>(invstd + c, is);
-    ldf<V>(coef + c, c0);
-    ldf<V>(coef + C + c, c1);
+    if (sums) {
+      const bool w = blockIdx.x == 0 && t.lane == 0;
+#pragma unroll
+      for (int k = 0; k < V; ++k)
+        bn_bwd_coef(sums, C, c + k, inv_count, training, w ? dgamma : nullptr, w ? dbeta : nullptr, c0[k], c1[k]);
+    } else {
+      ldf<V>(coef + c, c0);
+      ldf<V>(coef + C + c, c1);
+    }
 #pragma unroll
     for (int k = 0; k < V; ++k) { A[k] = -sc[k] * c1[k] * is[k]; B0[k] = -sc[k] * c0[k]; }
   }
@@ -801,10 +811,9 @@
                                float* save_invstd, float* scale, float* shift, int64_t* num_batches_tracked, int C,
                                void* stream) {
   UB_CHECK_ARG(C > 0 && count > 0, "bn_finalize: C=%d count=%lld", C, (long long)count);
-  double unbias = count > 1 ? (double)count / (double)(count - 1) : 1.0;
-  bn_finalize_kernel<<<(C + 127) / 128, 128, 0, (cudaStream_t)stream>>>(
-      stats, 1.0 / (double)count, unbias, gamma, beta, eps, momentum, running_mean, running_var, save_mean,
-      save_invstd, scale, shift, C, reinterpret_cast<long long*>(num_batches_tracked));
+  const BnFinalize f = make_bn_finalize(count, gamma, beta, eps, momentum, running_mean, running_var, save_mean,
+                                        save_invstd, scale, shift, num_batches_tracked, C);
+  bn_finalize_kernel<<<(C + 127) / 128, 128, 0, (cudaStream_t)stream>>>(stats, f);
   UB_LAUNCH_CHECK("bn_finalize");
   return 0;
 }
@@ -839,11 +848,11 @@
     int CV = C / V;                                                                                           \
     if (pooled) {                                                                                             \
       CsGeom g_ = cs_geom(CV, (int64_t)B * ((H + 1) / 2) * ((W + 1) / 2), 2);                                 \
-      bn_relu_apply_pool_kernel<T, V><<<dim3(g_.gx, g_.gy), 256, 0, s>>>(                                     \
+      (void)launch_pdl(bn_relu_apply_pool_kernel<T, V>, dim3(g_.gx, g_.gy), dim3(256), 0, s, 1, \
           (const T*)y, ld_y, scale, shift, (T*)z, ld_z, (T*)pooled, ld_p, B, H, W, CV, g_.CVB);               \
     } else {                                                                                                  \
       CsGeom g_ = cs_geom(CV, npix, 8);                                                                       \
-      bn_relu_apply_kernel<T, V><<<dim3(g_.gx, g_.gy), 256, 0, s>>>((const T*)y, ld_y, scale, shift, (T*)z,   \
+      (void)launch_pdl(bn_relu_apply_kernel<T, V>, dim3(g_.gx, g_.gy), dim3(256), 0, s, 1, (const T*)y, ld_y, scale, shift, (T*)z,   \
                                                                    ld_z, npix, CV, g_.CVB);                   \
     }                                                                                                         \
   } while (0)
@@ -889,10 +898,10 @@
     int CV = C / V;                                                                                           \
     int64_t work = (int64_t)B * ((H + 1) / 2) * ((W + 1) / 2) * CV;                                           \
     if (accumulate)                                                                                           \
-      maxpool2_bwd_kernel<T, V, true><<<grid_for(work, 256, 16), 256, 0, s>>>(                                \
+      (void)launch_pdl(maxpool2_bwd_kernel<T, V, true>, grid_for(work, 256, 16), dim3(256), 0, s, 1, \
           (const T*)x, ld_x, (const T*)gp, ld_gp, (T*)gx, ld_gx, B, H, W, CV);                                \
     else                                                                                                      \
-      maxpool2_bwd_kernel<T, V, false><<<grid_for(work, 256, 16), 256, 0, s>>>(                               \
+      (void)launch_pdl(maxpool2_bwd_kernel<T, V, false>, grid_for(work, 256, 16), dim3(256), 0, s, 1, \
           (const T*)x, ld_x, (const T*)gp, ld_gp, (T*)gx, ld_gx, B, H, W, CV);                                \
   } while (0)
   if (dtype == UNETB200_BF16) {
@@ -917,7 +926,7 @@
   do {                                                                                                        \
     const int CV = (C + V - 1) / V;                                                                           \
     CsGeom g_ = cs_geom(CV, nwin, 2, V == 8 ? 64 : 256);                                                      \
-    maxpool2_bwd_bnreduce_kernel<T, V><<<dim3(g_.gx, g_.gy), 256, 0, s>>>(                                    \
+    (void)launch_pdl(maxpool2_bwd_bnreduce_kernel<T, V>, dim3(g_.gx, g_.gy), dim3(256), 0, s, 1, \
         (const T*)x, ld_x, (const T*)gp, ld_gp, (T*)gx, ld_gx, (const T*)y, ld_y, scale, shift, mean, invstd, \
         sums, B, H, W, C, CV, g_.CVB);                                                                        \
   } while (0)
@@ -942,7 +951,7 @@
   do {                                                                                                        \
     int CV = C / V;                                                                                           \
     CsGeom g_ = cs_geom(CV, npix, 8, V == 8 ? 64 : 256);      \
-    bn_relu_bwd_reduce_kernel<T, V><<<dim3(g_.gx, g_.gy), 256, 0, s>>>(                                       \
+    (void)launch_pdl(bn_relu_bwd_reduce_kernel<T, V>, dim3(g_.gx, g_.gy), dim3(256), 0, s, 1, \
         (const T*)gz, ld_gz, (const T*)y, ld_y, scale, shift, mean, invstd, sums, npix, C, CV, g_.CVB);       \
   } while (0)
   if (dtype == UNETB200_BF16) {
@@ -964,20 +973,22 @@
   return 0;
 }
 
-int unetb200_bn_relu_bwd_apply(const void* gz, int64_t ld_gz, const void* y, int64_t ld_y, const float* scale,
-                               const float* shift, const float* mean, const float* invstd, const float* coef,
-                               void* gy, int64_t ld_gy, int dtype, int B, int H, int W, int C, void* stream) {
+static int bn_relu_bwd_apply_launch(const void* gz, int64_t ld_gz, const void* y, int64_t ld_y, const float* scale,
+                                    const float* shift, const float* mean, const float* invstd, const float* coef,
+                                    const double* sums, int training, float* dgamma, float* dbeta, void* gy,
+                                    int64_t ld_gy, int dtype, int B, int H, int W, int C, void* stream) {
   UB_DTYPE_OK(dtype);
   UB_CHECK_ARG(B > 0 && H > 0 && W > 0 && C > 0, "bn_relu_bwd_apply: bad shape");
   cudaStream_t s = (cudaStream_t)stream;
   const int64_t npix = (int64_t)B * H * W;
+  const double inv_count = 1.0 / (double)npix;
 #define GO(T, V)                                                                                             \
   do {                                                                                                       \
     int CV = C / V;                                                                                          \
     CsGeom g_ = cs_geom(CV, npix, 8);                                                                        \
-    bn_relu_bwd_apply_kernel<T, V><<<dim3(g_.gx, g_.gy), 256, 0, s>>>(                                       \
+    (void)launch_pdl(bn_relu_bwd_apply_kernel<T, V>, dim3(g_.gx, g_.gy), dim3(256), 0, s, 1, \
         (const T*)gz, ld_gz, (const T*)y, ld_y, scale, shift, mean, invstd, coef, (T*)gy, ld_gy, npix, C, CV,  \
-        g_.CVB);                                                                                             \
+        g_.CVB, sums, inv_count, training, dgamma, dbeta);                                                   \
   } while (0)
   if (dtype == UNETB200_BF16) {
     if (vec_ok<bf16>(C, {ld_gz, ld_y, ld_gy}, {gz, y, gy})) GO(bf16, 8); else GO(bf16, 1);
@@ -987,6 +998,23 @@
 #undef GO
   UB_LAUNCH_CHECK("bn_relu_bwd_apply");
   return 0;
+}
+
+int unetb200_bn_relu_bwd_apply(const void* gz, int64_t ld_gz, const void* y, int64_t ld_y, const float* scale,
+                               const float* shift, const float* mean, const float* invstd, const float* coef,
+                               void* gy, int64_t ld_gy, int dtype, int B, int H, int W, int C, void* stream) {
+  UB_CHECK_ARG(coef, "bn_relu_bwd_apply: null coefficients");
+  return bn_relu_bwd_apply_launch(gz, ld_gz, y, ld_y, scale, shift, mean, invstd, coef, nullptr, 0, nullptr, nullptr,
+                                  gy, ld_gy, dtype, B, H, W, C, stream);
+}
+
+int unetb200_bn_relu_bwd_finalize_apply(const void* gz, int64_t ld_gz, const void* y, int64_t ld_y, const float* scale,
+                                        const float* shift, const float* mean, const float* invstd, const double* sums,
+                                        int training, float* dgamma, float* dbeta, void* gy, int64_t ld_gy, int dtype,
+                                        int B, int H, int W, int C, void* stream) {
+  UB_CHECK_ARG(sums, "bn_relu_bwd_finalize_apply: null sums");
+  return bn_relu_bwd_apply_launch(gz, ld_gz, y, ld_y, scale, shift, mean, invstd, nullptr, sums, training, dgamma,
+                                  dbeta, gy, ld_gy, dtype, B, H, W, C, stream);
 }
 
 static inline float ac_scale(int in, int out) { return out > 1 ? (float)(in - 1) / (float)(out - 1) : 0.f; }
diff --git a/unet-medical-image-contour-segmentation_b200/csrc/gconv.cuh b/unet-medical-image-contour-segmentation_b200/csrc/gconv.cuh
--- a/unet-medical-image-contour-segmentation_b200/csrc/gconv.cuh
+++ b/unet-medical-image-contour-segmentation_b200/csrc/gconv.cuh
@@ -60,7 +60,7 @@
 int tc3_fprop(const unetb200_gconv_t* d, const GconvDev& g, const void* x, const void* wp, void* y, double* stats,
               float* stats_ws, cudaStream_t stream, const float* affine = nullptr, const void* yprev = nullptr,
               long long ld_yprev = 0, const float* bnc = nullptr, const Tc3OutConv* oc = nullptr, void* pooled = nullptr,
-              long long ld_pool = 0);
+              long long ld_pool = 0, const BnFinalize* bnf = nullptr);
 int tc3_bnbwd_supported(const unetb200_gconv_t* d);
 
 int tc3_wgrad_supported(const unetb200_gconv_t* d, const void* x, const void* gy);
diff --git a/unet-medical-image-contour-segmentation_b200/unetb200/_lib.py b/unet-medical-image-contour-segmentation_b200/unetb200/_lib.py
--- a/unet-medical-image-contour-segmentation_b200/unetb200/_lib.py
+++ b/unet-medical-image-contour-segmentation_b200/unetb200/_lib.py
@@ -45,6 +45,8 @@
     "unetb200_device_info": (C.c_int, [C.POINTER(C.c_int)] * 3),
     "unetb200_gconv_stats_workspace": (c_i64, [C.POINTER(GConv)]),
     "unetb200_gconv_fprop": (C.c_int, [C.POINTER(GConv), c_p, c_p, c_p, c_p, c_p, c_p, C.POINTER(C.c_int), c_p]),
+    "unetb200_gconv_fprop_bn": (C.c_int, [C.POINTER(GConv), c_p, c_p, c_p, c_p, c_p, c_i64, c_p, c_p, C.c_float, C.c_float,
+                                          c_p, c_p, c_p, c_p, c_p, c_p, c_p, C.POINTER(C.c_int), C.POINTER(C.c_int), c_p]),
     "unetb200_gconv_fprop_affine_relu_supported": (C.c_int, [C.POINTER(GConv), c_p, c_p, c_p]),
     "unetb200_gconv_fprop_affine_relu": (C.c_int, [C.POINTER(GConv), c_p, c_p, c_p, c_p, c_p]),
     "unetb200_gconv_fprop_affine_relu_pool_supported": (C.c_int, [C.POINTER(GConv), c_p, c_p, c_p, c_p, C.c_int64]),
@@ -71,6 +73,8 @@
     "unetb200_bn_relu_bwd_reduce": (C.c_int, [c_p, c_i64, c_p, c_i64, c_p, c_p, c_p, c_p, c_p, C.c_int, C.c_int, C.c_int, C.c_int, C.c_int, c_p]),
     "unetb200_bn_bwd_finalize": (C.c_int, [c_p, c_i64, C.c_int, c_p, c_p, c_p, C.c_int, c_p]),
     "unetb200_bn_relu_bwd_apply": (C.c_int, [c_p, c_i64, c_p, c_i64, c_p, c_p, c_p, c_p, c_p, c_p, c_i64, C.c_int, C.c_int, C.c_int, C.c_int, C.c_int, c_p]),
+    "unetb200_bn_relu_bwd_finalize_apply": (C.c_int, [c_p, c_i64, c_p, c_i64, c_p, c_p, c_p, c_p, c_p, C.c_int, c_p, c_p,
+                                                      c_p, c_i64, C.c_int, C.c_int, C.c_int, C.c_int, C.c_int, c_p]),
     "unetb200_bn_peer_group_create": (C.c_int, [C.c_int, C.c_int, C.c_int, c_p, c_p, C.POINTER(c_p)]),
     "unetb200_bn_peer_group_open": (C.c_int, [c_p, c_p, c_p]),
     "unetb200_bn_peer_group_destroy": (C.c_int, [c_p]),
diff --git a/unet-medical-image-contour-segmentation_b200/unetb200/functional.py b/unet-medical-image-contour-segmentation_b200/unetb200/functional.py
--- a/unet-medical-image-contour-segmentation_b200/unetb200/functional.py
+++ b/unet-medical-image-contour-segmentation_b200/unetb200/functional.py
@@ -345,7 +345,7 @@
     y = ops.empty_nhwc(B, Cout, H, W, cd, dev)
     use_batch = training or bn.running_mean is None
     stats = zeros_f64(2 * Cout, dev) if use_batch else None
-    ops.gconv_fprop(_gconv3x3(x, Cout, y, cd), x, wp, None, y, stats)
+    d = _gconv3x3(x, Cout, y, cd)
     gamma = _f32c(bn.weight) if bn.weight is not None else None
     beta = _f32c(bn.bias) if bn.bias is not None else None
     if use_batch:
@@ -356,12 +356,14 @@
                 bn.running_mean if update else None, bn.running_var if update else None, Cout)
         nbt = bn.num_batches_tracked if update else None
         if peer is None:
-            coefs = ops.bn_finalize(*args, num_batches_tracked=nbt)
+            coefs = ops.gconv_fprop_bn(d, x, wp, y, *args, num_batches_tracked=nbt)
         else:
+            ops.gconv_fprop(d, x, wp, None, y, stats)
             coefs = ops.bn_sync_finalize(peer, *args, num_batches_tracked=nbt)
         if update:
             torch._C._increment_version([bn.running_mean, bn.running_var])
     else:
+        ops.gconv_fprop(d, x, wp, None, y, stats)
         coefs = ops.bn_eval_coeffs(gamma, beta, bn.running_mean, bn.running_var, bn.eps, Cout)
     z = out if out is not None else ops.empty_nhwc(B, Cout, H, W, cd, dev)
     pooled = ops.empty_nhwc(B, Cout, H // 2, W // 2, cd, dev) if want_pool else None
diff --git a/unet-medical-image-contour-segmentation_b200/unetb200/ops.py b/unet-medical-image-contour-segmentation_b200/unetb200/ops.py
--- a/unet-medical-image-contour-segmentation_b200/unetb200/ops.py
+++ b/unet-medical-image-contour-segmentation_b200/unetb200/ops.py
@@ -344,6 +344,38 @@
     return used.value
 
 
+BNSTATS_FOLD = _os.environ.get("UNETB200_NO_BNSTATS_FOLD") is None
+
+
+def gconv_fprop_bn(d, x, wp, y, stats, count, gamma, beta, eps, momentum, running_mean, running_var, Cc,
+                   num_batches_tracked=None):
+    if not BNSTATS_FOLD or x3_active(d):
+        gconv_fprop(d, x, wp, None, y, stats)
+        return bn_finalize(stats, count, gamma, beta, eps, momentum, running_mean, running_var, Cc,
+                           num_batches_tracked=num_batches_tracked)
+    coefs = torch.empty((4, Cc), dtype=torch.float32, device=stats.device)
+    nbt = num_batches_tracked
+    if nbt is not None and not (nbt.dtype == torch.int64 and nbt.is_cuda and nbt.numel() == 1):
+        nbt.add_(1)
+        nbt = None
+    n = lib().unetb200_gconv_stats_workspace(C.byref(d))
+    if n < 0:
+        _lib.check(-1, "gconv_stats_workspace")
+    ws = torch.empty(n, dtype=torch.float32, device=x.device)
+    used, folded = C.c_int(0), C.c_int(0)
+    _run("conv_fprop", lib().unetb200_gconv_fprop_bn, C.byref(d), _p(x), _p(wp), _p(y), _p(stats), _p(ws), count,
+         _p(gamma), _p(beta), eps, momentum, _p(running_mean), _p(running_var), _prow(coefs, 0), _prow(coefs, 1),
+         _prow(coefs, 2), _prow(coefs, 3), _p(nbt), C.byref(used), C.byref(folded), _stream(), kernels=3,
+         flops=gconv_flops(d), nbytes=gconv_bytes(d, 2 if d.dtype == BF16 else 4))
+    global LAUNCHES
+    LAUNCHES -= folded.value
+    if _PROFILE is not None:
+        _PROFILE[-1][0] = f"conv_fprop_{_ALGO_NAME.get(used.value, '?')}" + _shape_tag(d)
+    if nbt is not None:
+        torch._C._increment_version([nbt])
+    return coefs
+
+
 def gconv_fprop_affine_relu_supported(d, x, wp, z):
     if x3_active(d):
         d = _x3_desc(d, ld_in=3 * d.Cin)
@@ -397,7 +429,7 @@
 def gconv_dgrad_bnbwd(d, g, wp, gx, yprev, coefs_prev):
     flops, nbytes = gconv_flops(d), gconv_bytes(d, 2 if d.dtype == BF16 else 4)
     tag = _shape_tag(d)
-    sums = torch.zeros((2, d.N), dtype=torch.float64, device=g.device)
+    sums = torch.empty((2, d.N), dtype=torch.float64, device=g.device)
     n = lib().unetb200_gconv_stats_workspace(C.byref(d))
     if n < 0:
         _lib.check(-1, "gconv_stats_workspace")
@@ -612,13 +644,18 @@
         dgamma = torch.empty(Cc, dtype=torch.float32, device=dev)
     if dbeta is None:
         dbeta = torch.empty(Cc, dtype=torch.float32, device=dev)
+    gy = empty_nhwc(B, Cc, H, W, y.dtype, dev)
+    if peer is None and BNSTATS_FOLD:
+        _run("bn_relu_bwd_apply", L.unetb200_bn_relu_bwd_finalize_apply, _p(gz), nhwc_ld(gz), _p(y), nhwc_ld(y),
+             _prow(coefs, 2), _prow(coefs, 3), _prow(coefs, 0), _prow(coefs, 1), _p(sums), 1 if training else 0,
+             _p(dgamma), _p(dbeta), _p(gy), nhwc_ld(gy), dt(y), B, H, W, Cc, _stream(), nbytes=3.0 * y.numel() * es)
+        return gy, dgamma, dbeta
     coef = torch.empty((2, Cc), dtype=torch.float32, device=dev)
     if peer is not None:
         bn_sync_bwd_finalize(peer, sums, B * H * W, dgamma, dbeta, coef)
     else:
         _run("bn_bwd_finalize", L.unetb200_bn_bwd_finalize, _p(sums), B * H * W, 1 if training else 0, _p(dgamma),
              _p(dbeta), _p(coef), Cc, _stream())
-    gy = empty_nhwc(B, Cc, H, W, y.dtype, dev)
     _run("bn_relu_bwd_apply", L.unetb200_bn_relu_bwd_apply, _p(gz), nhwc_ld(gz), _p(y), nhwc_ld(y), _prow(coefs, 2),
          _prow(coefs, 3), _prow(coefs, 0), _prow(coefs, 1), _p(coef), _p(gy), nhwc_ld(gy), dt(y), B, H, W, Cc, _stream(),
          nbytes=3.0 * y.numel() * es)
```

After: 705.4, median of 6. About the same (-0.3%).
